# acproject/wsi-segmentation-pipeline

Measured on AMD Instinct MI355X. Metric: patches/sec (256×256×3) whole-slide inference, 1/2/4/8 MI355X + CPU ref, higher is better.
Workload: dtype fp16 + MX-fp6 cross terms (fp32 accumulate); 1 GPU; cfg3: ONE 40000x40000 synthetic slide, tile 256 stride 256 -> 24648 tiles sharded over 1 rank(s) (each holds only its own slide regions: 4.80 GB on rank 0), ResNet-18 trunk + Classifier, fused read+normalise+conv HIP path, 1 all-gather, float64 stitch + softmax; tiles_total=24648, batch=6200, mode=mx, parallelism=tile-shard x1 + 1 all-gather, batches_in_flight=2

## Files before the change

include/wsi_hip.h:

```cpp
#ifndef WSI_HIP_H
#define WSI_HIP_H
#include <stddef.h>
#include <stdint.h>

#ifdef __cplusplus
extern "C" {
#endif

#define WSI_HIP_ABI_VERSION 8
int wsi_hip_abi_version(void);

size_t wsi_pf_bytes(int n, int h, int w, int c, int planes);
long long wsi_pf_pixel_index(int n, int y, int x, int h, int w);

size_t wsi_prepack_conv_bytes(int cout, int cin, int k, int planes);
int wsi_prepack_conv(const float* w, const float* bn_weight, const float* bn_bias, const float* bn_mean,
                     const float* bn_var, float eps, int cout, int cin, int k, int planes, void* wpk_out,
                     float* bias_out);
size_t wsi_prepack_stem_bytes(int planes);
int wsi_prepack_stem(const float* w, const float* bn_weight, const float* bn_bias, const float* bn_mean,
                     const float* bn_var, float eps, int planes, void* wpk_out, float* bias_out);
int wsi_prepack_stem_u8(const float* w, const float* bn_weight, const float* bn_bias, const float* bn_mean,
                        const float* bn_var, float eps, const float mean[3], const float std_[3], int planes,
                        void* wpk_out, float* bias_out);
int wsi_normalize_u8_lut(const float mean[3], const float std_[3], float* lut_out );

int wsi_stem_conv7x7_bn_relu_maxpool(const float* in_f32, const uint8_t* slide, long long slide_pitch_bytes,
                                     int slide_h, int slide_w, const int* tile_xy, const float* lut,
                                     const void* stem_wpk, const float* stem_bias,
                                     const void* stem_wpk_u8 ,
                                     const float* stem_bias_u8, const float* norm_mean_std ,
                                     int n, int h, int w, float* scratch, void* out_pf, int planes, void* stream);

enum {
    WSI_STEM_MODE_UNFUSED = 0,
    WSI_STEM_MODE_FUSED = 1,
    WSI_STEM_MODE_FUSED_LUT = 2,
    WSI_STEM_MODE_FUSED_ONE_STRIP = 3
};
int wsi_stem_set_mode(int fused, int rows_per_seg);

int wsi_conv3x3_bn_act(const void* in_pf, void* out_pf, const void* resid_pf, const void* wpk, const float* bias,
                       int n, int h_in, int w_in, int cin, int cout, int stride, int relu, int planes,
                       void* stream);
int wsi_conv1x1_bn(const void* in_pf, void* out_pf, const void* wpk, const float* bias, int n, int h_in, int w_in,
                   int cin, int cout, int stride, int planes, void* stream);
int wsi_conv3x3_up_concat_bn_act(const void* up_pf, const void* skip_pf, void* out_pf, const void* wpk, const float* bias, int n, int h, int w,
                                 int c_up, int c_skip, int cout, int relu, int planes, void* stream);
int wsi_conv3x3s2_ds_fused(const void* in_pf, void* out_conv_pf, void* out_ds_pf, const void* wpk3, const float* bias3,
                           const void* wpk1, const float* bias1, int n, int h_in, int w_in, int cin, int cout, int planes,
                           void* stream);
int wsi_s2_slab_images(int n, int h_in, int w_in, int cin, int planes);
size_t wsi_pf_split_bytes(int n, int h, int w, int c, int planes);
int wsi_conv3x3_bn_act_split(const void* in_pf, void* out_split, const void* resid_pf, const void* wpk, const float* bias,
                             int n, int h, int w, int cin, int cout, int relu, int planes, void* stream);
int wsi_conv3x3s2_ds_fused_split(const void* in_split, void* out_conv_pf, void* out_ds_pf, const void* wpk3,
                                 const float* bias3, const void* wpk1, const float* bias1, int n, int h_in, int w_in,
                                 int cin, int cout, int planes, void* stream);
enum {
    WSI_CONV_MODE_S2_GATHER = 0,
    WSI_CONV_MODE_S2_SLAB = 1,
    WSI_CONV_MODE_S2_SLAB_128 = 3,
    WSI_CONV_MODE_XCD_ORDER = 8,
    WSI_CONV_MODE_WIDE_FROM_256 = 16,
    WSI_CONV_MODE_WIDE_NEVER = 32,
    WSI_CONV_MODE_S2_ABLATE = 64,
    WSI_CONV_MODE_NO_S2_SPLIT = 128,
    WSI_CONV_MODE_XCD_RANGES_OFF = 256,
    WSI_CONV_MODE_XCD_RANGES_L1 = 512,
    WSI_CONV_MODE_L1_SLAB3 = 1024,
    WSI_CONV_MODE_NO_DS_FOLD = 2048,
    WSI_CONV_MODE_NO_SLAB_PAIR = 4096,
    WSI_CONV_MODE_L1_LINES128 = 16384,
    WSI_CONV_MODE_S2_NT2 = 32768,
    WSI_CONV_MODE_UNET_CONCAT_PASS = 65536,
    WSI_CONV_MODE_WIDE_NO_D8 = 131072,
    WSI_CONV_MODE_L1_PERSISTENT = 1048576,
    WSI_CONV_MODE_UNET_NO_TAIL = 2097152,
    WSI_CONV_MODE_UNET_TAIL_FORM1 = 4194304,
    WSI_CONV_MODE_UNET_X0_UNFUSED = 8388608
};
int wsi_conv_set_mode(int mode);
int wsi_conv3x3_bn_act_cfg(const void* in_pf, void* out_pf, const void* resid_pf, const void* wpk, const float* bias,
                           int n, int h_in, int w_in, int cin, int cout, int stride, int relu, int planes, int cfg,
                           void* stream);

int wsi_avgpool_fc(const void* in_pf, int n, int h, int w, int c, const float* fc_w, const float* fc_b, int k,
                   float* feat_out, float* logits_out, int planes, void* stream);
int wsi_linear(const float* x, const float* w, const float* bias, float* y, int b, int k, int j, int relu,
               void* stream);

int wsi_pf_pack(const float* in_nchw, void* out_pf, int n, int c, int h, int w, int planes, void* stream);
int wsi_pf_unpack(const void* in_pf, float* out_nchw, int n, int c, int h, int w, int planes, void* stream);

typedef struct {
    const void* stem_w;   const float* stem_b;
    const void* stem_w_u8; const float* stem_b_u8;
    float norm[6];
    const void* conv_w[16]; const float* conv_b[16];
    const void* down_w[3];  const float* down_b[3];
    const float* head_w;  const float* head_b;  int head_k;
    int planes;
} wsi_trunk_weights;

size_t wsi_trunk_workspace_bytes(int n, int h, int w, int planes);
int wsi_trunk_workspace_init(void* workspace, int n, int h, int w, int planes, void* stream);
int wsi_trunk_workspace_release(void* workspace);
int wsi_trunk_forward(const wsi_trunk_weights* wt, const float* in_f32, const uint8_t* slide,
                      long long slide_pitch_bytes, int slide_h, int slide_w, const int* tile_xy, const float* lut,
                      int n, int h, int w, void* workspace, int workspace_n, float* feat_out ,
                      float* logits_out , float* fmap_out ,
                      void* stream);
int wsi_trunk_set_chunks(int stem_chunk, int layer1_chunk);
int wsi_trunk_forward_tap(const wsi_trunk_weights* wt, const float* in_f32, const uint8_t* slide,
                          long long slide_pitch_bytes, int slide_h, int slide_w, const int* tile_xy, const float* lut,
                          int n, int h, int w, void* workspace, int workspace_n, int stop_after, float* tap_out_nchw,
                          void* stream);

int wsi_prof_begin(int max_records);
int wsi_prof_end(float* ms_out, int* kind_out, double* flops_out, int cap);

int wsi_tile_gather(const uint8_t* slide, long long slide_pitch_bytes, int slide_h, int slide_w, const int* tile_xy,
                    const float* lut, float* out_nchw, int n, int ph, int pw, void* stream);
int wsi_stitch_add(const float* tile_logits, const int* map_xy, int t, int c, int dy, int dx, double* pred, int map_h,
                   int map_w, void* stream);
int wsi_stitch_add_dense(const float* tile_pred, const int* map_xy, int t, int c, int ph, int pw, double* pred, int map_h,
                         int map_w, void* stream);
int wsi_softmax_threshold_argmax(const double* pred, int c, long long hw, const double* class_thresh, double* probs,
                                 uint8_t* classes, const uint8_t* mask, int heat_mode, uint8_t* heat, void* stream);
typedef struct wsi_ring wsi_ring;
typedef struct wsi_resample_plan wsi_resample_plan;
int wsi_ring_create(wsi_ring** out, int slots, size_t slot_bytes);
void* wsi_ring_host_slot(wsi_ring* ring, int slot);
int wsi_ring_wait_slot(wsi_ring* ring, int slot);
int wsi_ring_submit(wsi_ring* ring, int slot, int rows, int width, int channels, long long src_pitch, uint8_t* level_rows, long long level_pitch);
int wsi_ring_acquire(wsi_ring* ring, void* compute_stream);
int wsi_ring_fence(wsi_ring* ring, void* compute_stream);
int wsi_ring_device(const wsi_ring* ring);
int wsi_ring_drain(wsi_ring* ring);
void wsi_ring_destroy(wsi_ring* ring);
int wsi_resample_plan_create(wsi_resample_plan** out, int in_h, int in_w, int out_h, int out_w);
void wsi_resample_plan_destroy(wsi_resample_plan* plan);
size_t wsi_resample_scratch_bytes(const wsi_resample_plan* plan, int n);
int wsi_resample_tiles(const wsi_resample_plan* plan, const uint8_t* slide, long long pitch, int sh, int sw, const int* tile_xy, int n,
                       uint8_t* out, void* scratch, void* stream);
int wsi_find_nuclei_hsv(const uint8_t* rgb, long long npix, int pixel_stride, double mu_percent, uint8_t* mask_out, void* stream);
size_t wsi_connected_components_scratch_bytes(int h, int w);
int wsi_connected_components(const uint8_t* mask, int h, int w, int* labels_out, int* count_out, void* scratch, void* stream);
int wsi_kmeans_points(const int* points_xy, int n, double* centres_xy, int k, int max_iters, int* labels_out, void* scratch, void* stream);
int wsi_kmeans_seed_farthest(const int* points_xy, int n, int k, double* centres_xy_out, void* scratch, void* stream);
int wsi_find_nuclei_lab(const uint8_t* rgb, long long npix, int pixel_stride, double mu_percent, uint8_t* mask_out, void* scratch, void* stream);
size_t wsi_fill_holes_scratch_bytes(int h, int w);
int wsi_fill_holes(const uint8_t* mask, int h, int w, uint8_t* out, void* scratch, void* stream);
size_t wsi_slic_scratch_bytes(int h, int w, int k);
int wsi_slic(const uint8_t* rgb, int h, int w, const double* gauss_weights, int radius, double* segments, int k, int step_y, int step_x,
             double step, double compactness, int iters, int* labels_out, void* scratch, void* stream);
long long wsi_tile_grid_candidates(int iw, int ih, int ph, int pw, int sh, int sw);
size_t wsi_tile_grid_scratch_bytes(long long candidates);
int wsi_tile_grid(int iw, int ih, int ph, int pw, int sh, int sw, const uint8_t* mask, int mask_h, int mask_w, double m, double thresh,
                  int* tile_xy_out, int* count_out, void* scratch, void* stream);
int wsi_exponent_span(const float* values, long long n, int* out2, void* stream);
int wsi_paint_regions(const long long* pixel_idx, const int* region_of, long long n, const uint8_t* region_class, int* winner_scratch,
                      long long* label, long long npix, void* stream);

int wsi_resize_bilinear_f64(const double* src, int c, int hs, int ws, double* dst, int hd, int wd, void* stream);
int wsi_argmax_classes(const double* pred, int c, long long hw, uint8_t* classes, void* stream);
int wsi_morph_rect(const uint8_t* src, uint8_t* dst, uint8_t* tmp, int h, int w, int k, int op, void* stream);
int wsi_bwperim(const uint8_t* src, uint8_t* dst, int h, int w, void* stream);
size_t wsi_tumor_bed_workspace_bytes(int h, int w);
int wsi_convex_hull_image(const uint8_t* src, uint8_t* dst, int h, int w, void* workspace, void* stream);
int wsi_tumor_bed(const uint8_t* codes, int h, int w, int min_code, int open_k, int dilate_k, uint8_t* opened_out,
                  uint8_t* tb_pred_out, uint8_t* outline_out, void* workspace, void* stream);
int wsi_hull_polygon(void* workspace, int h, int w, double* out_xy, int cap, int* count_out, void* stream);
int wsi_mask_iou_counts(const uint8_t* a, const uint8_t* b, long long n, unsigned long long* out2, void* stream);
int wsi_score_counts(const uint8_t* p, const uint8_t* gt, const uint8_t* mask, long long n, unsigned long long* out6,
                     void* stream);
int wsi_esp(const double* pts_xy, int n, int num_pts, double* out_xy, double* scratch, void* stream);

typedef struct {
    const void* conv_w[10]; const float* conv_b[10];
    int cin[10], cout[10];
    const float* head_w; const float* head_b;
    int head_cin, classes;
    const void* tail_w;
} wsi_unet_decoder_weights;
size_t wsi_unet_tail_prepack_bytes(void);
int wsi_unet_tail_prepack(const float* w1, const float* bn1_weight, const float* bn1_bias, const float* bn1_mean, const float* bn1_var,
                          const float* w2, const float* bn2_weight, const float* bn2_bias, const float* bn2_mean, const float* bn2_var,
                          float eps, const float* head_w, const float* head_b, int cin, int cmid, int classes, void* out);
int wsi_unet_tail_bands(int n, int h, int cus);
int wsi_unet_tail_timeouts(unsigned long long* out, int reset);
size_t wsi_unet_workspace_bytes(const wsi_unet_decoder_weights* dw, int n, int h, int w, int planes);
int wsi_unet_workspace_init(const wsi_unet_decoder_weights* dw, void* workspace, int n, int h, int w, int planes, void* stream);
int wsi_unet_forward(const wsi_trunk_weights* wt, const wsi_unet_decoder_weights* dw, const float* in_f32, const uint8_t* slide,
                     long long slide_pitch_bytes, int slide_h, int slide_w, const int* tile_xy, const float* lut, int n, int h,
                     int w, void* workspace, int workspace_n, float* logits_out, float* enc_out[5], void* stream);
int wsi_unet_decoder(const wsi_unet_decoder_weights* dw, const float* const enc_nchw[5], int n, int h, int w, int planes,
                     void* workspace, int workspace_n, float* logits_out, void* stream);
int wsi_resize_nearest_f32(const float* src, long long planes_n, int hs, int ws, float* dst, int hd, int wd, void* stream);

#ifdef __cplusplus
}
#endif
#endif
```

wsi_segmentation_pipeline_amd/csrc/capi.hip:

```cpp
#include "common.h"
#include <mutex>
#include <unordered_map>
#include <vector>
#include <cmath>
#include "../../include/wsi_hip.h"
#include <math.h>
#include <string.h>

int wsi_conv_dispatch(const ConvArgs& a, int planes, int cfg, hipStream_t st);
int wsi_s2_dispatch(const ConvArgs& a, int planes, hipStream_t st);
int wsi_stem_dispatch(const StemArgs& a, int planes, hipStream_t st);
int wsi_maxpool_dispatch(const float* in, void* out, int N, int Hc, int Wc, int planes, hipStream_t st);
int wsi_stem_pool_dispatch(const StemArgs& a, void* out_pf, int planes, int rows_per_seg, hipStream_t st, int out96 = 0, long long plane96 = 0, void* x0_pf = nullptr);
int wsi_avgpool_fc_dispatch(const void* in, const PFGeom& g, const float* w, const float* b, int K, float* feat,
                            float* logits, int planes, hipStream_t st);
int wsi_linear_dispatch(const float* x, const float* w, const float* bias, float* y, int B, int K, int J, int relu,
                        hipStream_t st);
int wsi_pf_pack_dispatch(const float* in, void* out, const PFGeom& g, int planes, hipStream_t st);
int wsi_pf_unpack_dispatch(const void* in, float* out, const PFGeom& g, int planes, hipStream_t st);
int wsi_tile_gather_dispatch(const uint8_t* slide, long long pitch, int SH, int SW, const int* origins, const float* lut,
                             float* out, int N, int ph, int pw, hipStream_t st);
int wsi_stitch_add_dispatch(const float* logits, const int* txy, int T, int C, int dy, int dx, double* pred, int MH, int MW,
                            hipStream_t st);
int wsi_stitch_add_dense_dispatch(const float* tiles, const int* txy, int T, int C, int ph, int pw, double* pred, int MH,
// ... 359 lines not shown
    const int DIG = 3;
    int8_t* o = (int8_t*)wpk_out;
    float* scale_out = (float*)((char*)wpk_out + 2 * 7 * 3 * 1024);
    memset(wpk_out, 0, (size_t)2 * 7 * 3 * 1024 + 64 * sizeof(float));
    const double qmax = DIG == 3 ? 127.0 * 65536.0 : 127.0 * 256.0;
    for (int co = 0; co < 64; ++co) {
        double sc, sh;
        bn_fold(bn_weight, bn_bias, bn_mean, bn_var, eps, co, sc, sh);
        bias_out[co] = (float)sh;
        double val[7][8][4];
        double amax = 0.0;
        for (int kh = 0; kh < 7; ++kh)
            for (int kw = 0; kw < 8; ++kw) {
                double kap = 0.0;
                for (int c = 0; c < 3; ++c) {
                    const double wd = kw < 7 ? (double)w[(((size_t)co * 3 + c) * 7 + kh) * 7 + kw] * sc / (255.0 * (double)std_[c]) : 0.0;
                    val[kh][kw][c] = wd;
                    kap += wd * (128.0 - 255.0 * (double)mean[c]);
                    amax = fmax(amax, fabs(wd));
                }
                val[kh][kw][3] = kap / 127.0;
                amax = fmax(amax, fabs(val[kh][kw][3]));
            }
        const double scale = amax > 0.0 ? amax / qmax : 1.0;
        scale_out[co] = (float)scale;
        const double fscale = (double)scale_out[co];
        const int nt = co >> 5, l31 = co & 31;
        for (int kh = 0; kh < 7; ++kh)
            for (int kw = 0; kw < 8; ++kw)
                for (int c = 0; c < 4; ++c) {
                    long long q = llround(val[kh][kw][c] / fscale);
                    const int h = kw >> 2, j = (kw & 3) * 4 + c, lane = h * 32 + l31;
                    for (int d = 0; d < DIG; ++d) {
                        const long long dig = ((q + 128) & 255) - 128;
                        q = (q - dig) / 256;
                        o[(((size_t)(nt * 7 + kh) * DIG + d) * 64 + lane) * 16 + j] = (int8_t)dig;
                    }
                }
    }
    return WSI_OK;
}

int wsi_normalize_u8_lut(const float mean[3], const float std_[3], float* lut_out) {
    if (!mean || !std_ || !lut_out) return WSI_EINVAL;
    for (int c = 0; c < 3; ++c)
        for (int v = 0; v < 256; ++v) {
            volatile float t = (float)v / 255.0f;
            volatile float d = t - mean[c];
            lut_out[c * 256 + v] = d / std_[c];
        }
    return WSI_OK;
}

int wsi_stem_set_mode(int fused, int rows_per_seg) {
    if (rows_per_seg <= 0) return WSI_EINVAL;
    g_routes.stem_fused = fused != WSI_STEM_MODE_UNFUSED; g_routes.stem_rows = rows_per_seg;
    g_routes.stem_u8x = fused != WSI_STEM_MODE_FUSED_LUT;
    g_routes.stem_shared_weights = fused != WSI_STEM_MODE_FUSED_ONE_STRIP;
    return WSI_OK;
}

struct TileSource {
    const float* in_f32;
    const uint8_t* slide;
    long long pitch; int SH, SW;
    const int* tile_xy;
    const float* lut;
    bool valid() const { return in_f32 || (slide && tile_xy && lut); }
    TileSource from_image(int n0, int h, int w) const {
        return {in_f32 ? in_f32 + (size_t)n0 * 3 * h * w : nullptr, slide, pitch, SH, SW, tile_xy ? tile_xy + 2 * n0 : nullptr, lut};
    }
};
static StemArgs stem_args(const TileSource& src, const void* wpk, const float* bias, float* scratch, int n, int h, int w) {
    StemArgs a;
    a.mode = src.in_f32 ? 0 : 1;
    a.in_f32 = src.in_f32; a.slide = src.slide; a.slide_pitch = src.pitch; a.SH = src.SH; a.SW = src.SW;
    a.origins = src.tile_xy; a.lut = src.lut; a.wpk = wpk; a.bias = bias; a.out = scratch;
    a.N = n; a.H = h; a.W = w; a.wpk_u8 = nullptr; a.bias_u8 = nullptr;
    return a;
}

static int stem_run(const TileSource& src, const void* stem_wpk, const float* stem_bias, const void* stem_wpk_u8,
                    const float* stem_bias_u8, const float* norm_mean_std, int n, int h, int w,
                    float* scratch, void* out_pf, int planes, void* stream, int out96, long long plane96 = 0, void* x0_pf = nullptr) {
    if (!stem_wpk || !stem_bias || !scratch || !out_pf || n <= 0 || h % 16 || w % 4) return WSI_EINVAL;
    if (!src.valid()) return WSI_EINVAL;
    StemArgs a = stem_args(src, stem_wpk, stem_bias, scratch, n, h, w);
    if (stem_wpk_u8 && stem_bias_u8 && norm_mean_std && !src.in_f32 && g_routes.stem_u8x) { a.wpk_u8 = stem_wpk_u8; a.bias_u8 = stem_bias_u8; }
    if (out96 && planes != 3) return WSI_EINVAL;
    if (x0_pf && !(a.wpk_u8 && g_routes.stem_fused && planes == 2)) return WSI_EINVAL;
    if (g_routes.stem_fused || planes == 3) return wsi_stem_pool_dispatch(a, out_pf, planes, g_routes.stem_rows, (hipStream_t)stream, out96, plane96, x0_pf);
    int rc = wsi_stem_dispatch(a, planes, (hipStream_t)stream);
    if (rc) return rc;
    return wsi_maxpool_dispatch(scratch, out_pf, n, h / 2, w / 2, planes, (hipStream_t)stream);
}

int wsi_stem_conv7x7_bn_relu_maxpool(const float* in_f32, const uint8_t* slide, long long slide_pitch_bytes,
                                     int slide_h, int slide_w, const int* tile_xy, const float* lut,
                                     const void* stem_wpk, const float* stem_bias, const void* stem_wpk_u8,
                                     const float* stem_bias_u8, const float* norm_mean_std, int n, int h, int w,
                                     float* scratch, void* out_pf, int planes, void* stream) {
    return stem_run({in_f32, slide, slide_pitch_bytes, slide_h, slide_w, tile_xy, lut}, stem_wpk, stem_bias, stem_wpk_u8, stem_bias_u8,
                    norm_mean_std, n, h, w, scratch, out_pf, planes, stream, 0);
}

#ifdef WSI_STUDY
static void* g_study_debug = nullptr;
extern "C" int wsi_study_set_debug(void* dev_buf) { g_study_debug = dev_buf; return WSI_OK; }
#endif

struct ConvCall {
    const void* in;
    void* out;
    const void* resid = nullptr;
    const void* wpk; const float* bias;
    int n, h, w, cin, cout, stride, ksize, relu, planes;
    void* stream;
    int cfg = -1;
    int split_out = 0; long long split_pixels = 0;
    const void* in2 = nullptr; int in2_c = 0; const void* wpk2 = nullptr; const float* bias2 = nullptr;
    int line_flags = 0;
    const void* in_up = nullptr; int up_c = 0;
    long long plane96 = 0;
};

static ConvArgs conv_args(const ConvCall& c) {
    ConvArgs a;
    a.in = c.in; a.out = c.out; a.resid = c.resid; a.wpk = c.wpk; a.bias = c.bias;
    a.gi = pf_geom_fd(c.n, c.h, c.w, c.cin);
    a.go = pf_geom_fd(c.n, c.h / c.stride, c.w / c.stride, c.cout);
    a.stride = c.stride; a.ksize = c.ksize; a.relu = c.relu & 1; a.flags = 0;
    a.out2 = nullptr; a.wpk2 = nullptr; a.bias2 = nullptr;
    a.in_split_pixels = 0; a.out_split_pixels = 0;
    return a;
}

static int conv_common(const ConvCall& c) {
    const hipStream_t st = (hipStream_t)c.stream;
    int cfg = c.cfg;
    if ((!c.in && !(c.in_up && c.up_c == c.cin)) || !c.out || !c.wpk || !c.bias || c.in == c.out || c.in_up == c.out || c.n <= 0) return WSI_EINVAL;
    if (c.line_flags && (c.planes != 3 || c.stride != 1 || c.ksize != 3 || c.cin != 64 || c.cout != 64 || (c.split_out && (c.line_flags & CONV_OUT96)) ||
                         (c.line_flags & ~(CONV_IN96 | CONV_OUT96 | CONV_RESID96)) || ((c.line_flags & CONV_RESID96) && !c.resid)))
        return WSI_EINVAL;
    if ((c.stride != 1 && c.stride != 2) || c.h % c.stride || c.w % c.stride) return WSI_EINVAL;
    ConvArgs a = conv_args(c);
    a.plane96 = c.line_flags ? (c.plane96 > 0 ? c.plane96 : (long long)pf_alloc_pixels(c.n, c.h, c.w) * 96) : 0;
#ifdef WSI_STUDY
    if (c.relu & 2) a.flags |= CONV_ABL_NO_STORE;
    if (c.relu & 64) a.flags |= CONV_ABL_DISPATCH_ONLY;
    if (c.relu & 128) a.flags |= CONV_ABL_NO_MAINLOOP;
    if (c.relu & 256) a.flags |= CONV_NONTEMPORAL;
    if (c.relu & 512) a.flags |= CONV_XCD_ORDER;
    if (c.relu & 16384) a.flags |= CONV_XCD_RANGES;
    if (c.relu & 65536) a.flags |= CONV_RESID_DIRECT;
    a.flags |= ((c.relu >> 10) & 15) << CONV_WCOPIES_SHIFT;
#else
    if (c.relu & ~1) return WSI_EINVAL;
#endif
    a.flags |= c.line_flags;
    if (c.in_up) {
        if (c.stride != 1 || c.ksize != 3 || c.h % 2 || c.w % 2 || c.up_c <= 0 || c.up_c > c.cin || c.resid || c.in2 || c.line_flags || c.split_out) return WSI_EINVAL;
        a.in_up = c.in_up; a.up_c = c.up_c; a.gup = pf_geom_fd(c.n, c.h / 2, c.w / 2, c.up_c);
    }
    if (c.in2) {
        if (c.planes != 3 || c.stride != 1 || c.ksize != 3 || c.resid || !c.wpk2 || !c.bias2 || c.in2_c <= 0 || c.in2_c % 32 || c.cout % 128 || cfg >= 0) return WSI_EINVAL;
        a.in2 = c.in2; a.in2_c = c.in2_c; a.wpk2 = c.wpk2; a.bias2 = c.bias2;
        cfg = 60;
    }
#ifdef WSI_STUDY
    if (cfg == 75 || cfg == 76) a.out2 = g_study_debug;
#endif
    a.out_split_pixels = c.split_out ? (c.split_pixels ? c.split_pixels : pf_alloc_pixels(c.n, c.h / 2, c.w / 2)) : 0;
    if (c.split_out && (c.stride != 1 || c.ksize != 3 || c.h % 2 || c.w % 2 || c.planes < 2)) return WSI_EINVAL;
    if (c.ksize == 3 && c.stride == 2 && c.cout % 128 == 0 && cfg != 0 && g_routes.s2_slab) {
        const int rc = wsi_s2_dispatch(a, c.planes, st);
        if (rc != WSI_EINVAL) return rc;
    }
    return wsi_conv_dispatch(a, c.planes, cfg, st);
}

int wsi_conv3x3_bn_act(const void* in_pf, void* out_pf, const void* resid_pf, const void* wpk, const float* bias,
                       int n, int h_in, int w_in, int cin, int cout, int stride, int relu, int planes,
                       void* stream) {
    return conv_common({.in = in_pf, .out = out_pf, .resid = resid_pf, .wpk = wpk, .bias = bias, .n = n, .h = h_in, .w = w_in, .cin = cin,
                        .cout = cout, .stride = stride, .ksize = 3, .relu = relu, .planes = planes, .stream = stream});
}

size_t wsi_pf_split_bytes(int n, int h, int w, int c, int planes) {
    if (h % 2 || w % 2) return 0;
    return 4 * wsi_pf_bytes(n, h / 2, w / 2, c, planes);
}

int wsi_conv3x3_bn_act_split(const void* in_pf, void* out_split, const void* resid_pf, const void* wpk, const float* bias,
                             int n, int h, int w, int cin, int cout, int relu, int planes, void* stream) {
    return conv_common({.in = in_pf, .out = out_split, .resid = resid_pf, .wpk = wpk, .bias = bias, .n = n, .h = h, .w = w, .cin = cin,
                        .cout = cout, .stride = 1, .ksize = 3, .relu = relu, .planes = planes, .stream = stream, .split_out = 1});
}

static ConvArgs s2_ds_args(const void* in, void* out_conv_pf, void* out_ds_pf, const void* wpk3, const float* bias3, const void* wpk1,
                           const float* bias1, int n, int h_in, int w_in, int cin, int cout) {
    ConvArgs a = conv_args({.in = in, .out = out_conv_pf, .wpk = wpk3, .bias = bias3, .n = n, .h = h_in, .w = w_in, .cin = cin, .cout = cout,
                            .stride = 2, .ksize = 3, .relu = 1});
    a.out2 = out_ds_pf; a.wpk2 = out_ds_pf ? wpk1 : nullptr; a.bias2 = out_ds_pf ? bias1 : nullptr;
    return a;
}

static int s2_split_common(const void* in_split, void* out_conv_pf, void* out_ds_pf, const void* wpk3,
                           const float* bias3, const void* wpk1, const float* bias1, int n, int h_in, int w_in,
                           int cin, int cout, int planes, void* stream, long long split_pixels) {
    if (!in_split || !out_conv_pf || !wpk3 || !bias3 || (out_ds_pf && (!wpk1 || !bias1)) || n <= 0 || h_in % 2 || w_in % 2)
        return WSI_EINVAL;
    if (in_split == out_conv_pf || in_split == out_ds_pf || out_conv_pf == out_ds_pf) return WSI_EINVAL;
    ConvArgs a = s2_ds_args(in_split, out_conv_pf, out_ds_pf, wpk3, bias3, wpk1, bias1, n, h_in, w_in, cin, cout);
    a.in_split_pixels = split_pixels ? split_pixels : pf_alloc_pixels(n, h_in / 2, w_in / 2);
    return wsi_s2_dispatch(a, planes, (hipStream_t)stream);
}

int wsi_conv3x3s2_ds_fused_split(const void* in_split, void* out_conv_pf, void* out_ds_pf, const void* wpk3,
                                 const float* bias3, const void* wpk1, const float* bias1, int n, int h_in, int w_in,
                                 int cin, int cout, int planes, void* stream) {
    return s2_split_common(in_split, out_conv_pf, out_ds_pf, wpk3, bias3, wpk1, bias1, n, h_in, w_in, cin, cout, planes, stream, 0);
}

int wsi_conv3x3_bn_act_cfg(const void* in_pf, void* out_pf, const void* resid_pf, const void* wpk, const float* bias,
                           int n, int h_in, int w_in, int cin, int cout, int stride, int relu, int planes, int cfg,
                           void* stream) {
    return conv_common({.in = in_pf, .out = out_pf, .resid = resid_pf, .wpk = wpk, .bias = bias, .n = n, .h = h_in, .w = w_in, .cin = cin,
                        .cout = cout, .stride = stride, .ksize = 3, .relu = relu, .planes = planes, .stream = stream, .cfg = cfg});
}

int wsi_conv3x3_up_concat_bn_act(const void* up_pf, const void* skip_pf, void* out_pf, const void* wpk, const float* bias, int n, int h, int w,
                                 int c_up, int c_skip, int cout, int relu, int planes, void* stream) {
    if (!up_pf || c_up <= 0 || c_skip < 0 || (c_skip > 0 && !skip_pf)) return WSI_EINVAL;
    return conv_common({.in = c_skip ? skip_pf : nullptr, .out = out_pf, .wpk = wpk, .bias = bias, .n = n, .h = h, .w = w, .cin = c_up + c_skip,
                        .cout = cout, .stride = 1, .ksize = 3, .relu = relu, .planes = planes, .stream = stream, .in_up = up_pf, .up_c = c_up});
}

int wsi_s2_slab_images(int n, int h_in, int w_in, int cin, int planes) {
    if (n <= 0 || h_in <= 0 || w_in <= 0 || cin <= 0 || planes < 1 || planes > 3) return WSI_EINVAL;
    const unsigned long long pix = (unsigned long long)cin * (planes == 1 ? PFmt<1>::BPC : PFmt<2>::BPC);
    auto fits = [&](int m) { return (unsigned long long)pf_alloc_pixels(m, h_in, w_in) * pix < 0xffffffffull; };
    if (fits(n)) return n;
    if (!fits(1)) return 0;
    int lo = 1, hi = n;
    while (hi - lo > 1) {
        const int mid = lo + (hi - lo) / 2;
        (fits(mid) ? lo : hi) = mid;
    }
    return lo;
}

int wsi_conv3x3s2_ds_fused(const void* in_pf, void* out_conv_pf, void* out_ds_pf, const void* wpk3, const float* bias3,
                           const void* wpk1, const float* bias1, int n, int h_in, int w_in, int cin, int cout, int planes,
                           void* stream) {
    if (!in_pf || !out_conv_pf || !out_ds_pf || !wpk3 || !bias3 || !wpk1 || !bias1 || n <= 0 || h_in % 2 || w_in % 2)
        return WSI_EINVAL;
    if (in_pf == out_conv_pf || in_pf == out_ds_pf || out_conv_pf == out_ds_pf) return WSI_EINVAL;
    ConvArgs a = s2_ds_args(in_pf, out_conv_pf, out_ds_pf, wpk3, bias3, wpk1, bias1, n, h_in, w_in, cin, cout);
    const int per = wsi_s2_slab_images(n, h_in, w_in, cin, planes);
    const size_t bpc = planes == 1 ? PFmt<1>::BPC : PFmt<2>::BPC;
    const size_t in_img = (size_t)(h_in + 1) * (w_in + 1) * cin * bpc, out_img = (size_t)(h_in / 2 + 1) * (w_in / 2 + 1) * cout * bpc;
    int rc = WSI_EINVAL;
    for (int n0 = 0; per > 0 && n0 < n; n0 += per) {
        const int nn = n - n0 < per ? n - n0 : per;
        a.in = (const char*)in_pf + n0 * in_img;
        a.out = (char*)out_conv_pf + n0 * out_img;
        a.out2 = (char*)out_ds_pf + n0 * out_img;
        a.gi = pf_geom_fd(nn, h_in, w_in, cin);
        a.go = pf_geom_fd(nn, h_in / 2, w_in / 2, cout);
        rc = wsi_s2_dispatch(a, planes, (hipStream_t)stream);
        if (rc) break;
    }
    if (rc == WSI_EINVAL) {
        ConvCall c = {.in = in_pf, .out = out_conv_pf, .wpk = wpk3, .bias = bias3, .n = n, .h = h_in, .w = w_in, .cin = cin, .cout = cout,
                      .stride = 2, .ksize = 3, .relu = 1, .planes = planes, .stream = stream, .cfg = 0};
        rc = conv_common(c);
        c.out = out_ds_pf; c.wpk = wpk1; c.bias = bias1; c.ksize = 1; c.relu = 0;
        if (!rc) rc = conv_common(c);
    }
    return rc;
}

int wsi_conv_set_mode(int mode) {
    ConvRoutes& r = g_routes;
    const int base = mode & 7;
    r.s2_slab = base != WSI_CONV_MODE_S2_GATHER;
    r.s2_small_tiles = base != WSI_CONV_MODE_S2_SLAB_128;
    r.xcd_order = (mode & WSI_CONV_MODE_XCD_ORDER) ? 1 : 0;
    r.wide_min_c = (mode & WSI_CONV_MODE_WIDE_FROM_256) ? 256 : (mode & WSI_CONV_MODE_WIDE_NEVER) ? (1 << 30) : 128;
    r.s2_ablate = (mode & WSI_CONV_MODE_S2_ABLATE) ? 1 : 0;
    r.s2_split = (mode & WSI_CONV_MODE_NO_S2_SPLIT) ? 0 : 1;
    r.xcd_ranges = (mode & WSI_CONV_MODE_XCD_RANGES_OFF) ? 0 : (mode & WSI_CONV_MODE_XCD_RANGES_L1) ? 1 : 2;
    r.l1_rows = (mode & WSI_CONV_MODE_L1_SLAB3) ? 0 : 1;
    r.ds_fold = (mode & WSI_CONV_MODE_NO_DS_FOLD) ? 0 : 1;
    r.slab_pair = (mode & WSI_CONV_MODE_NO_SLAB_PAIR) ? 0 : 1;
    r.l1_lines96 = (mode & WSI_CONV_MODE_L1_LINES128) ? 0 : 1;
    r.s2_nt4 = (mode & WSI_CONV_MODE_S2_NT2) ? 0 : 1;
    r.unet_fuse_up = (mode & WSI_CONV_MODE_UNET_CONCAT_PASS) ? 0 : 1;
    r.wide_d8 = (mode & WSI_CONV_MODE_WIDE_NO_D8) ? 0 : 1;
    r.l1p = (mode & WSI_CONV_MODE_L1_PERSISTENT) ? 1 : 0;
    r.unet_tail = (mode & WSI_CONV_MODE_UNET_NO_TAIL) ? 0 : 1;
    r.unet_tail_form = (mode & WSI_CONV_MODE_UNET_TAIL_FORM1) ? 1 : 2;
    r.unet_x0_fused = (mode & WSI_CONV_MODE_UNET_X0_UNFUSED) ? 0 : 1;
    return WSI_OK;
}

int wsi_conv1x1_bn(const void* in_pf, void* out_pf, const void* wpk, const float* bias, int n, int h_in, int w_in,
                   int cin, int cout, int stride, int planes, void* stream) {
    return conv_common({.in = in_pf, .out = out_pf, .wpk = wpk, .bias = bias, .n = n, .h = h_in, .w = w_in, .cin = cin, .cout = cout,
                        .stride = stride, .ksize = 1, .relu = 0, .planes = planes, .stream = stream});
}

int wsi_avgpool_fc(const void* in_pf, int n, int h, int w, int c, const float* fc_w, const float* fc_b, int k,
                   float* feat_out, float* logits_out, int planes, void* stream) {
    if (!in_pf || n <= 0 || (logits_out && (!fc_w || !fc_b || k <= 0))) return WSI_EINVAL;
    return wsi_avgpool_fc_dispatch(in_pf, pf_geom(n, h, w, c), fc_w, fc_b, k, feat_out, logits_out, planes,
                                   (hipStream_t)stream);
}

int wsi_linear(const float* x, const float* w, const float* bias, float* y, int b, int k, int j, int relu,
               void* stream) {
    if (!x || !w || !y) return WSI_EINVAL;
    return wsi_linear_dispatch(x, w, bias, y, b, k, j, relu, (hipStream_t)stream);
}

int wsi_pf_pack(const float* in_nchw, void* out_pf, int n, int c, int h, int w, int planes, void* stream) {
    if (!in_nchw || !out_pf || n <= 0 || planes < 1 || planes > 3 || c % (planes == 1 ? 64 : 32)) return WSI_EINVAL;
    return wsi_pf_pack_dispatch(in_nchw, out_pf, pf_geom(n, h, w, c), planes, (hipStream_t)stream);
}

int wsi_pf_unpack(const void* in_pf, float* out_nchw, int n, int c, int h, int w, int planes, void* stream) {
    if (!in_pf || !out_nchw || n <= 0 || planes < 1 || planes > 3 || c % (planes == 1 ? 64 : 32)) return WSI_EINVAL;
    return wsi_pf_unpack_dispatch(in_pf, out_nchw, pf_geom(n, h, w, c), planes, (hipStream_t)stream);
}

int wsi_tile_gather(const uint8_t* slide, long long slide_pitch_bytes, int slide_h, int slide_w, const int* tile_xy,
                    const float* lut, float* out_nchw, int n, int ph, int pw, void* stream) {
    if (!slide || !tile_xy || !lut || !out_nchw) return WSI_EINVAL;
    return wsi_tile_gather_dispatch(slide, slide_pitch_bytes, slide_h, slide_w, tile_xy, lut, out_nchw, n, ph, pw,
                                    (hipStream_t)stream);
}

int wsi_stitch_add(const float* tile_logits, const int* map_xy, int t, int c, int dy, int dx, double* pred, int map_h,
                   int map_w, void* stream) {
    if (!tile_logits || !map_xy || !pred || map_h <= 0 || map_w <= 0) return WSI_EINVAL;
    return wsi_stitch_add_dispatch(tile_logits, map_xy, t, c, dy, dx, pred, map_h, map_w, (hipStream_t)stream);
}

int wsi_stitch_add_dense(const float* tile_pred, const int* map_xy, int t, int c, int ph, int pw, double* pred, int map_h,
                         int map_w, void* stream) {
    if (!tile_pred || !map_xy || !pred || map_h <= 0 || map_w <= 0) return WSI_EINVAL;
    return wsi_stitch_add_dense_dispatch(tile_pred, map_xy, t, c, ph, pw, pred, map_h, map_w, (hipStream_t)stream);
}

int wsi_softmax_threshold_argmax(const double* pred, int c, long long hw, const double* class_thresh, double* probs,
                                 uint8_t* classes, const uint8_t* mask, int heat_mode, uint8_t* heat, void* stream) {
    if (!pred || !class_thresh) return WSI_EINVAL;
    return wsi_softmax_dispatch(pred, c, hw, class_thresh, probs, classes, mask, heat_mode, heat, (hipStream_t)stream);
}

int wsi_ring_create(wsi_ring** out, int slots, size_t slot_bytes) { return wsi_ring_create_impl(out, slots, slot_bytes); }
void* wsi_ring_host_slot(wsi_ring* r, int slot) { return wsi_ring_host_slot_impl(r, slot); }
int wsi_ring_wait_slot(wsi_ring* r, int slot) { return wsi_ring_wait_slot_impl(r, slot); }
int wsi_ring_submit(wsi_ring* r, int slot, int rows, int width, int channels, long long src_pitch, uint8_t* level_rows, long long level_pitch) {
    return wsi_ring_submit_impl(r, slot, rows, width, channels, src_pitch, level_rows, level_pitch);
}
int wsi_ring_fence(wsi_ring* r, void* compute_stream) { return wsi_ring_fence_impl(r, (hipStream_t)compute_stream); }
int wsi_ring_acquire(wsi_ring* r, void* compute_stream) { return wsi_ring_acquire_impl(r, (hipStream_t)compute_stream); }
int wsi_ring_device(const wsi_ring* r) { return wsi_ring_device_impl(r); }
int wsi_ring_drain(wsi_ring* r) { return wsi_ring_drain_impl(r); }
void wsi_ring_destroy(wsi_ring* r) { wsi_ring_destroy_impl(r); }
int wsi_resample_plan_create(wsi_resample_plan** out, int in_h, int in_w, int out_h, int out_w) {
    return wsi_resample_plan_create_impl(out, in_h, in_w, out_h, out_w);
}
void wsi_resample_plan_destroy(wsi_resample_plan* p) { wsi_resample_plan_destroy_impl(p); }
size_t wsi_resample_scratch_bytes(const wsi_resample_plan* p, int n) { return wsi_resample_scratch_bytes_impl(p, n); }
int wsi_resample_tiles(const wsi_resample_plan* p, const uint8_t* slide, long long pitch, int sh, int sw, const int* tile_xy, int n,
                       uint8_t* out, void* scratch, void* stream) {
    return wsi_resample_tiles_impl(p, slide, pitch, sh, sw, tile_xy, n, out, scratch, (hipStream_t)stream);
}

int wsi_find_nuclei_hsv(const uint8_t* rgb, long long npix, int pixel_stride, double mu_percent, uint8_t* mask_out, void* stream) {
    if (!rgb || !mask_out) return WSI_EINVAL;
    return wsi_hsv_mask_dispatch(rgb, npix, pixel_stride, mu_percent, mask_out, (hipStream_t)stream);
}
size_t wsi_connected_components_scratch_bytes(int h, int w) { return (h <= 0 || w <= 0) ? 0 : wsi_cc_scratch_bytes(h, w); }
int wsi_connected_components(const uint8_t* mask, int h, int w, int* labels_out, int* count_out, void* scratch, void* stream) {
    if (!mask || !labels_out || !scratch) return WSI_EINVAL;
    return wsi_cc_dispatch(mask, h, w, labels_out, count_out, scratch, (hipStream_t)stream);
}
int wsi_find_nuclei_lab(const uint8_t* rgb, long long npix, int pixel_stride, double mu_percent, uint8_t* mask_out, void* scratch, void* stream) {
    return wsi_lab_mask_dispatch(rgb, npix, pixel_stride, mu_percent, mask_out, scratch, (hipStream_t)stream);
}
size_t wsi_fill_holes_scratch_bytes(int h, int w) { return (h <= 0 || w <= 0) ? 0 : wsi_fill_holes_scratch_bytes_impl(h, w); }
int wsi_fill_holes(const uint8_t* mask, int h, int w, uint8_t* out, void* scratch, void* stream) {
    return wsi_fill_holes_dispatch(mask, h, w, out, scratch, (hipStream_t)stream);
}
size_t wsi_slic_scratch_bytes(int h, int w, int k) { return wsi_slic_scratch_bytes_impl(h, w, k); }
int wsi_slic(const uint8_t* rgb, int h, int w, const double* gauss_weights, int radius, double* segments, int k, int step_y, int step_x,
             double step, double compactness, int iters, int* labels_out, void* scratch, void* stream) {
    return wsi_slic_dispatch(rgb, h, w, gauss_weights, radius, segments, k, step_y, step_x, step, compactness, iters, labels_out, scratch,
                             (hipStream_t)stream);
}
int wsi_kmeans_points(const int* points_xy, int n, double* centres_xy, int k, int max_iters, int* labels_out, void* scratch, void* stream) {
    if (!points_xy || !centres_xy || !labels_out || !scratch) return WSI_EINVAL;
    return wsi_kmeans_dispatch(points_xy, n, centres_xy, k, max_iters, labels_out, scratch, (hipStream_t)stream);
}

int wsi_kmeans_seed_farthest(const int* points_xy, int n, int k, double* centres_xy_out, void* scratch, void* stream) {
    if (!points_xy || !centres_xy_out || !scratch) return WSI_EINVAL;
    return wsi_kmeans_seed_farthest_dispatch(points_xy, n, k, centres_xy_out, scratch, (hipStream_t)stream);
}

long long wsi_tile_grid_candidates(int iw, int ih, int ph, int pw, int sh, int sw) { return wsi_tile_grid_candidates_impl(iw, ih, ph, pw, sh, sw); }
size_t wsi_tile_grid_scratch_bytes(long long candidates) { return candidates < 0 ? 0 : wsi_tile_grid_scratch_bytes_impl(candidates); }
int wsi_tile_grid(int iw, int ih, int ph, int pw, int sh, int sw, const uint8_t* mask, int mask_h, int mask_w, double m, double thresh,
                  int* tile_xy_out, int* count_out, void* scratch, void* stream) {
    if (!tile_xy_out || !count_out || !scratch) return WSI_EINVAL;
    return wsi_tile_grid_dispatch(iw, ih, ph, pw, sh, sw, mask, mask_h, mask_w, m, thresh, tile_xy_out, count_out, scratch, (hipStream_t)stream);
}

int wsi_exponent_span(const float* values, long long n, int* out2, void* stream) {
    if (!values || !out2) return WSI_EINVAL;
    return wsi_exponent_span_dispatch(values, n, out2, (hipStream_t)stream);
}

int wsi_paint_regions(const long long* pixel_idx, const int* region_of, long long n, const uint8_t* region_class, int* winner_scratch,
                      long long* label, long long npix, void* stream) {
    if (!region_class || !winner_scratch || !label || (n && (!pixel_idx || !region_of))) return WSI_EINVAL;
    return wsi_paint_dispatch(pixel_idx, region_of, n, region_class, winner_scratch, label, npix, (hipStream_t)stream);
}

int wsi_resize_bilinear_f64(const double* src, int c, int hs, int ws, double* dst, int hd, int wd, void* stream) {
    if (!src || !dst || src == dst) return WSI_EINVAL;
    return wsi_resize_dispatch(src, c, hs, ws, dst, hd, wd, (hipStream_t)stream);
}
int wsi_argmax_classes(const double* pred, int c, long long hw, uint8_t* classes, void* stream) {
    if (!pred || !classes) return WSI_EINVAL;
    return wsi_argmax_dispatch(pred, c, hw, classes, (hipStream_t)stream);
}
int wsi_morph_rect(const uint8_t* src, uint8_t* dst, uint8_t* tmp, int h, int w, int k, int op, void* stream) {
    if (!src || !dst || !tmp) return WSI_EINVAL;
    return wsi_morph_dispatch(src, dst, tmp, h, w, k, op, (hipStream_t)stream);
}
int wsi_bwperim(const uint8_t* src, uint8_t* dst, int h, int w, void* stream) {
    if (!src || !dst) return WSI_EINVAL;
    return wsi_bwperim_dispatch(src, dst, h, w, (hipStream_t)stream);
}
size_t wsi_tumor_bed_workspace_bytes(int h, int w) {
    if (h <= 0 || w <= 0) return 0;
    return 3 * align_up((size_t)h * w, 256) + align_up(wsi_hull_ws_bytes(h), 256);
}
int wsi_convex_hull_image(const uint8_t* src, uint8_t* dst, int h, int w, void* workspace, void* stream) {
    if (!src || !dst || !workspace || src == dst) return WSI_EINVAL;
    return wsi_hull_dispatch(src, dst, h, w, (char*)workspace + 3 * align_up((size_t)h * w, 256), (hipStream_t)stream);
}
int wsi_tumor_bed(const uint8_t* codes, int h, int w, int min_code, int open_k, int dilate_k, uint8_t* opened_out,
                  uint8_t* tb_pred_out, uint8_t* outline_out, void* workspace, void* stream) {
    if (!codes || !tb_pred_out || !outline_out || !workspace || h <= 0 || w <= 0 || open_k <= 0 || dilate_k <= 0 ||
        tb_pred_out == outline_out)
        return WSI_EINVAL;
    hipStream_t st = (hipStream_t)stream;
    const size_t plane = align_up((size_t)h * w, 256);
    uint8_t *A = (uint8_t*)workspace, *B = A + plane, *Cc = B + plane;
    void* hws = Cc + plane;
    int rc = wsi_threshold_dispatch(codes, (long long)h * w, min_code, A, st);
    if (!rc) rc = wsi_morph_dispatch(A, B, Cc, h, w, open_k, 2, st);
    if (!rc && opened_out && hipMemcpyAsync(opened_out, B, (size_t)h * w, hipMemcpyDeviceToDevice, st) != hipSuccess) rc = WSI_EFAULT;
    if (!rc) rc = wsi_hull_dispatch(B, tb_pred_out, h, w, hws, st);
    if (!rc) rc = wsi_bwperim_dispatch(tb_pred_out, A, h, w, st);
    if (!rc) rc = wsi_morph_dispatch(A, outline_out, Cc, h, w, dilate_k, 1, st);
    return rc;
}
int wsi_hull_polygon(void* workspace, int h, int w, double* out_xy, int cap, int* count_out, void* stream) {
    if (!workspace || !out_xy || !count_out || h <= 0 || w <= 0 || cap <= 0) return WSI_EINVAL;
    char* hws = (char*)workspace + 3 * align_up((size_t)h * w, 256);
    int rc = wsi_hull_polygon_dispatch(hws, h, out_xy, cap, (hipStream_t)stream);
    if (rc) return rc;
    const int* counts = (const int*)hws + 2 * (2 * (size_t)h + 1);
    return hipMemcpyAsync(count_out, counts + 2, sizeof(int), hipMemcpyDeviceToDevice, (hipStream_t)stream) == hipSuccess ? WSI_OK : WSI_EFAULT;
}
int wsi_mask_iou_counts(const uint8_t* a, const uint8_t* b, long long n, unsigned long long* out2, void* stream) {
    if (!a || !b || !out2) return WSI_EINVAL;
    return wsi_iou_counts_dispatch(a, b, n, out2, (hipStream_t)stream);
}
int wsi_score_counts(const uint8_t* p, const uint8_t* gt, const uint8_t* mask, long long n, unsigned long long* out6, void* stream) {
    if (!p || !gt || !out6) return WSI_EINVAL;
    return wsi_score_counts_dispatch(p, gt, mask, n, out6, (hipStream_t)stream);
}
int wsi_esp(const double* pts_xy, int n, int num_pts, double* out_xy, double* scratch, void* stream) {
    if (!pts_xy || !out_xy || !scratch) return WSI_EINVAL;
    return wsi_esp_dispatch(pts_xy, n, num_pts, out_xy, scratch, (hipStream_t)stream);
}

#define WSI_PROF_MAX 16384
static struct {
    int enabled, count, cap;
    hipEvent_t ev[2 * WSI_PROF_MAX];
    int kind[WSI_PROF_MAX];
    double flops[WSI_PROF_MAX];
    int created;
} g_prof;

int wsi_prof_begin(int max_records) {
    if (max_records <= 0 || max_records > WSI_PROF_MAX) return WSI_EINVAL;
    for (; g_prof.created < 2 * max_records; ++g_prof.created)
        if (hipEventCreate(&g_prof.ev[g_prof.created]) != hipSuccess) return WSI_ENOMEM;
    g_prof.cap = max_records; g_prof.count = 0; g_prof.enabled = 1;
    return WSI_OK;
}

int wsi_prof_end(float* ms_out, int* kind_out, double* flops_out, int cap) {
    g_prof.enabled = 0;
    int n = g_prof.count < cap ? g_prof.count : cap;
    for (int i = 0; i < n; ++i) {
        if (hipEventSynchronize(g_prof.ev[2 * i + 1]) != hipSuccess) return WSI_EFAULT;
        float ms = 0.f;
        if (hipEventElapsedTime(&ms, g_prof.ev[2 * i], g_prof.ev[2 * i + 1]) != hipSuccess) return WSI_EFAULT;
        ms_out[i] = ms; kind_out[i] = g_prof.kind[i]; flops_out[i] = g_prof.flops[i];
    }
    g_prof.count = 0;
    return n;
}

struct ProfScope {
    const hipStream_t st;
    int i = -1;
    ProfScope(hipStream_t st, int kind, double flops) : st(st) {
        if (!g_prof.enabled || g_prof.count >= g_prof.cap) return;
        i = g_prof.count++;
        g_prof.kind[i] = kind; g_prof.flops[i] = flops;
        (void)hipEventRecord(g_prof.ev[2 * i], st);
    }
    ~ProfScope() { if (i >= 0) (void)hipEventRecord(g_prof.ev[2 * i + 1], st); }
    void relabel(int kind) { if (i >= 0) g_prof.kind[i] = kind; }
};
static inline double conv_flops(int n, int ho, int wo, int ci, int co, int taps) { return 2.0 * n * ho * wo * (double)co * ci * taps; }

static std::mutex g_ws_mutex;
struct WsTag { int layout; size_t bytes; };
static std::unordered_map<const void*, WsTag> g_ws_layout;
static int ws_layout_switch(const void* ws, int want, size_t need) {
    std::lock_guard<std::mutex> lk(g_ws_mutex);
    auto it = g_ws_layout.find(ws);
    const int have = it == g_ws_layout.end() ? -2 : it->second.layout;
    const size_t bytes = it == g_ws_layout.end() ? 0 : it->second.bytes;
    if (bytes && need > bytes) return -1;
    g_ws_layout[ws] = WsTag{want, bytes};
    if (have == want || have == -1) return 0;
    return (have >= 0 && have / 2 != want / 2) ? 2 : 1;
}
int wsi_trunk_workspace_release(void* workspace) {
    std::lock_guard<std::mutex> lk(g_ws_mutex);
    g_ws_layout.erase(workspace);
    return WSI_OK;
}

int wsi_trunk_set_chunks(int stem_chunk, int layer1_chunk) {
    if (stem_chunk < 0 || layer1_chunk < 0) return WSI_EINVAL;
    if (stem_chunk && layer1_chunk && layer1_chunk % stem_chunk) return WSI_EINVAL;
    g_routes.chunk_stem = stem_chunk; g_routes.chunk_l1 = layer1_chunk;
    return WSI_OK;
}
struct TrunkPlan {
    size_t stem_scratch;
    size_t buf[4][4];
    size_t total;
    int sh[4], sw[4], sc[4];
};

static int trunk_plan(int n, int h, int w, int planes, TrunkPlan& p) {
    if (n <= 0 || h <= 0 || w <= 0 || h % 32 || w % 32 || planes < 1 || planes > 3) return WSI_EINVAL;
    size_t off = 0;
    p.stem_scratch = off;
    off += align_up((size_t)n * (h / 2) * (w / 2) * 64 * sizeof(float), 256);
    for (int s = 0; s < 4; ++s) {
        p.sh[s] = h >> (2 + s); p.sw[s] = w >> (2 + s); p.sc[s] = 64 << s;
        for (int b = 0; b < 3; ++b) {
            p.buf[s][b] = off;
            off += align_up(wsi_pf_bytes(n, p.sh[s], p.sw[s], p.sc[s], planes), 256);
        }
        p.buf[s][3] = off;
        if (s < 3 && planes >= 2) off += align_up(wsi_pf_split_bytes(n, p.sh[s], p.sw[s], p.sc[s], planes), 256);
    }
    p.total = off;
    return WSI_OK;
}

size_t wsi_trunk_workspace_bytes(int n, int h, int w, int planes) {
    TrunkPlan p;
    return trunk_plan(n, h, w, planes, p) ? 0 : p.total;
}

int wsi_trunk_workspace_init(void* workspace, int n, int h, int w, int planes, void* stream) {
    TrunkPlan p;
    if (!workspace || trunk_plan(n, h, w, planes, p)) return WSI_EINVAL;
    {
        std::lock_guard<std::mutex> lk(g_ws_mutex);
        g_ws_layout[workspace] = WsTag{-1, p.total};
    }
    return hipMemsetAsync((char*)workspace + p.buf[0][0], 0, p.total - p.buf[0][0], (hipStream_t)stream) == hipSuccess
               ? WSI_OK
               : WSI_EFAULT;
}

static int trunk_run(const wsi_trunk_weights* wt, const TileSource& src, int n, int cap, int h, int w, void* workspace,
// ... 318 lines not shown
```

wsi_segmentation_pipeline_amd/csrc/common.h:

```cpp
#pragma once
#include <hip/hip_runtime.h>
#include <stdint.h>

typedef __attribute__((ext_vector_type(8))) __bf16 bf16x8;
typedef __attribute__((ext_vector_type(4))) __bf16 bf16x4;
typedef __attribute__((ext_vector_type(16))) float f32x16;
typedef __attribute__((ext_vector_type(4))) float f32x4;

#define WSI_OK 0
#define WSI_EINVAL (-22)
#define WSI_ENOMEM (-12)
#define WSI_EFAULT (-14)

struct FastDiv { unsigned m; int s; };
static inline FastDiv fastdiv_make(int d) {
    FastDiv f;
    if (d <= 1) { f.m = 0u; f.s = -1; return f; }
    int l = 0;
    while ((1ll << l) < d) ++l;
    f.m = (unsigned)(((1ull << (31 + l)) / (unsigned long long)d) + 1ull);
    f.s = l - 1;
    return f;
}
#ifdef __HIPCC__
static inline __device__ int fd_div(int i, const FastDiv& f) { return f.s < 0 ? i : (int)(__umulhi((unsigned)i, f.m) >> f.s); }
#endif

struct PFGeom {
    int N, H, W, C;
    int P, S, G;
    int NS;
    FastDiv dHW, dW, dS, dP;
};

static inline __host__ __device__ PFGeom pf_geom(int n, int h, int w, int c) {
    PFGeom g;
    g.N = n; g.H = h; g.W = w; g.C = c;
    g.P = w + 1; g.S = (h + 1) * (w + 1); g.G = w + 2; g.NS = n * g.S;
    g.dHW.m = g.dW.m = g.dS.m = g.dP.m = 0u; g.dHW.s = g.dW.s = g.dS.s = g.dP.s = 0;
    return g;
}
static inline PFGeom pf_geom_fd(int n, int h, int w, int c) {
    PFGeom g = pf_geom(n, h, w, c);
    g.dHW = fastdiv_make(h * w); g.dW = fastdiv_make(w); g.dS = fastdiv_make(g.S); g.dP = fastdiv_make(g.P);
    return g;
}
static inline __device__ int pf_pos_of_index(const PFGeom& g, int i) {
    const int n = fd_div(i, g.dHW), rem = i - n * (g.H * g.W);
    const int y = fd_div(rem, g.dW), x = rem - y * g.W;
    return g.G + n * g.S + y * g.P + x;
}

#define PF_TILE_ROUND 512

static inline __host__ __device__ long long pf_alloc_pixels(int n, int h, int w) {
    long long P = w + 1, S = (long long)(h + 1) * P, G = P + 1;
    long long body = ((long long)n * S + PF_TILE_ROUND - 1) / PF_TILE_ROUND * PF_TILE_ROUND;
    return 2 * G + body + PF_TILE_ROUND;
}

static inline __device__ bool pf_is_pixel(const PFGeom& g, int q) {
    int r = q - g.G;
    if (r < 0 || r >= g.NS) return false;
    int x = r % g.P;
    int y = (r / g.P) % (g.H + 1);
    return x != g.W && y != g.H;
}

template <int PLANES> struct PFmt {
    static constexpr int BPC = PLANES == 1 ? 2 : 4;
    static constexpr int CPL = PLANES == 1 ? 64 : 32;
};
typedef __attribute__((ext_vector_type(8))) _Float16 f16x8;
typedef __attribute__((ext_vector_type(4))) _Float16 f16x4;
typedef __attribute__((ext_vector_type(8))) int i32x8;
typedef __attribute__((ext_vector_type(4))) unsigned int u32x4;
typedef __attribute__((ext_vector_type(2))) float f32x2;
typedef __attribute__((ext_vector_type(2))) _Float16 f16x2;
typedef __attribute__((ext_vector_type(4))) int i32x4;

struct ConvArgs {
    const void* in;
    void* out;
    const void* resid;
    const void* wpk;
    const float* bias;
    PFGeom gi, go;
    int stride;
    int ksize;
    int relu;
    int flags;
    void* out2;
    const void* wpk2;
    const float* bias2;
    long long out_split_pixels, in_split_pixels;
    int mtiles = 0;
    const void* in2 = nullptr;
    int in2_c = 0;
    const void* in_up = nullptr;
    int up_c = 0;
    PFGeom gup = {};
    long long plane96 = 0;
};

enum : int {
    CONV_XCD_ORDER = 1,
    CONV_XCD_RANGES = 2,
    CONV_RESID_DIRECT = 4,
    CONV_IN96 = 16, CONV_OUT96 = 32, CONV_RESID96 = 64,
    CONV_ABL_NO_STORE = 1 << 8, CONV_ABL_DISPATCH_ONLY = 1 << 9, CONV_ABL_NO_MAINLOOP = 1 << 10, CONV_NONTEMPORAL = 1 << 11,
    CONV_WCOPIES_SHIFT = 16,
};
#ifdef WSI_STUDY
#define CONV_STUDY(a, bits) ((a).flags & (bits))
#else
#define CONV_STUDY(a, bits) 0
#endif

static inline __device__ size_t pf_out_offset(const PFGeom& g, long long split_pixels, int q, size_t pixstride) {
    if (!split_pixels) return (size_t)q * pixstride;
    int r = q - g.G;
    const int n = fd_div(r, g.dS);
    r -= n * g.S;
    const int y = fd_div(r, g.dP), x = r - y * g.P;
    const int P2 = g.W / 2 + 1, S2 = (g.H / 2 + 1) * P2;
    const long long q2 = (long long)(P2 + 1) + (long long)n * S2 + (y >> 1) * P2 + (x >> 1);
    return (size_t)(((y & 1) * 2 + (x & 1)) * split_pixels + q2) * pixstride;
}

static inline __device__ f32x16 mfma_bf16(bf16x8 a, bf16x8 b, f32x16 c) {
    return __builtin_amdgcn_mfma_f32_32x32x16_bf16(a, b, c, 0, 0, 0);
}
template <int PLANES> struct PairElem { typedef __bf16 T; };
template <> struct PairElem<2> { typedef _Float16 T; };
template <int PLANES>
static inline __device__ f32x16 mfma16(bf16x8 a, bf16x8 b, f32x16 c) {
    typedef __attribute__((ext_vector_type(8))) _Float16 h8;
    if constexpr (PLANES == 2) return __builtin_amdgcn_mfma_f32_32x32x16_f16(__builtin_bit_cast(h8, a), __builtin_bit_cast(h8, b), c, 0, 0, 0);
    else return __builtin_amdgcn_mfma_f32_32x32x16_bf16(a, b, c, 0, 0, 0);
}

typedef __attribute__((ext_vector_type(6))) unsigned u32x6;
typedef __attribute__((ext_vector_type(16))) unsigned u32x16;
typedef __attribute__((ext_vector_type(32))) float f32x32;
static inline __host__ __device__ int mx6_scale_byte(float amax) {
    union { float f; unsigned u; } c;
    c.f = amax;
    const unsigned u = c.u & 0x7fffffffu;
    if (u == 0u) return 0;
    const int e = (int)(u >> 23) - 2 + ((u & 0x7fffffu) > 0x780000u ? 1 : 0);
    return e < 1 ? 1 : (e > 254 ? 254 : e);
}
static inline __host__ __device__ float mx_scale_value(int s) {
    union { float f; unsigned u; } c;
    c.u = (unsigned)s << 23;
    return c.f;
}
static inline __host__ __device__ int mx_line_pos(int c) { return 16 * ((c >> 2) & 1) + 4 * (c >> 3) + (c & 3); }
static inline __host__ __device__ int mx_line_chan(int p) { return 8 * ((p & 15) >> 2) + 4 * (p >> 4) + (p & 3); }
static inline __host__ __device__ int mx6_field_of_pos(int p) { return 2 * (p & 15) + (p >> 4); }
static inline __host__ __device__ int mx6_field_chan(int f) { return mx_line_chan(16 * (f & 1) + (f >> 1)); }
#define MX6_PLANE_LO(q) (64 + 16 * (q))
#define MX6_PLANE_HI(q) (96 + 16 * (q))
#define MX6_SCALE(q) (104 + 16 * (q))

static inline __host__ __device__ float fp6_value(unsigned c) {
    const int e = (c >> 3) & 3, m = c & 7;
    const float v = e ? (float)(8 + m) * (e == 1 ? 0.125f : e == 2 ? 0.25f : 0.5f) : (float)m * 0.125f;
    return (c & 32) ? -v : v;
}
static inline __host__ __device__ unsigned fp6_encode(float y) {
    union { float f; unsigned u; } c;
    c.f = y;
    const unsigned sign = (c.u >> 31) ? 32u : 0u;
    c.u &= 0x7fffffffu;
    const float a = c.f;
    if (!(a < 7.5f)) return sign | 31u;
    const float step = a < 2.f ? 0.125f : a < 4.f ? 0.25f : 0.5f;
    const float t = a / step;
    float r = (float)(int)t;
    const float frac = t - r;
    if (frac > 0.5f || (frac == 0.5f && ((int)r & 1))) r += 1.f;
    const float q = r * step;
    unsigned code;
    if (q < 1.f) code = (unsigned)(q * 8.f);
    else if (q < 2.f) code = 8u + (unsigned)((q - 1.f) * 8.f);
    else if (q < 4.f) code = 16u + (unsigned)((q - 2.f) * 4.f);
    else code = 24u + (unsigned)((q - 4.f) * 2.f);
    return sign | code;
}
static inline __host__ __device__ unsigned mx6_get_field(const unsigned* w, int f) {
    const int bit = 6 * f, d = bit >> 5, s = bit & 31;
    unsigned v = w[d] >> s;
    if (s > 26) v |= w[d + 1] << (32 - s);
    return v & 63u;
}
static inline __host__ __device__ void mx6_set_field(unsigned* w, int f, unsigned code) {
    const int bit = 6 * f, d = bit >> 5, s = bit & 31;
    w[d] |= code << s;
    if (s > 26) w[d + 1] |= code >> (32 - s);
}

#ifdef __HIPCC__
static __device__ __forceinline__ u32x6 mx6_pack32(f32x16 a, f32x16 b, float scale) {
    u32x6 r;
    asm volatile("v_cvt_scalef32_2xpk16_fp6_f32 %0, %1, %2, %3" : "=&v"(r) : "v"(a), "v"(b), "v"(scale));
    return r;
}
static __device__ __forceinline__ f32x32 mx6_unpack32(u32x6 q, float scale) {
    f32x32 r;
    asm volatile("v_cvt_scalef32_pk32_f32_fp6 %0, %1, %2" : "=&v"(r) : "v"(q), "v"(scale));
    return r;
}
static __device__ __forceinline__ void swap32_halves(f32x16& a, f32x16& b) {
#pragma unroll
    for (int k = 0; k < 16; k += 8) {
        float a0 = a[k], a1 = a[k + 1], a2 = a[k + 2], a3 = a[k + 3], a4 = a[k + 4], a5 = a[k + 5], a6 = a[k + 6], a7 = a[k + 7];
        float b0 = b[k], b1 = b[k + 1], b2 = b[k + 2], b3 = b[k + 3], b4 = b[k + 4], b5 = b[k + 5], b6 = b[k + 6], b7 = b[k + 7];
        asm volatile("s_nop 1\n\tv_permlane32_swap_b32 %0, %8\n\tv_permlane32_swap_b32 %1, %9\n\tv_permlane32_swap_b32 %2, %10\n\t"
                     "v_permlane32_swap_b32 %3, %11\n\tv_permlane32_swap_b32 %4, %12\n\tv_permlane32_swap_b32 %5, %13\n\t"
                     "v_permlane32_swap_b32 %6, %14\n\tv_permlane32_swap_b32 %7, %15\n\ts_nop 1"
                     : "+v"(a0), "+v"(a1), "+v"(a2), "+v"(a3), "+v"(a4), "+v"(a5), "+v"(a6), "+v"(a7),
                       "+v"(b0), "+v"(b1), "+v"(b2), "+v"(b3), "+v"(b4), "+v"(b5), "+v"(b6), "+v"(b7));
        a[k] = a0; a[k + 1] = a1; a[k + 2] = a2; a[k + 3] = a3; a[k + 4] = a4; a[k + 5] = a5; a[k + 6] = a6; a[k + 7] = a7;
        b[k] = b0; b[k + 1] = b1; b[k + 2] = b2; b[k + 3] = b3; b[k + 4] = b4; b[k + 5] = b5; b[k + 6] = b6; b[k + 7] = b7;
    }
}
static __device__ __forceinline__ void pair_max2(float& x, float& y) {
    float x2 = x, y2 = y;
    asm volatile("s_nop 1\n\tv_permlane32_swap_b32 %0, %1\n\tv_permlane32_swap_b32 %2, %3\n\ts_nop 1" : "+v"(x), "+v"(x2), "+v"(y), "+v"(y2));
    x = fmaxf(x, x2);
    y = fmaxf(y, y2);
}

#endif

static inline __device__ void split_f16(float x, _Float16& hi, _Float16& lo) {
    x = __builtin_amdgcn_fmed3f(x, -65504.f, 65504.f);
    hi = (_Float16)x;
    lo = (_Float16)(x - (float)hi);
}
static inline __device__ void split_f16x4(const float* v, f16x4& hi, f16x4& lo) {
#pragma unroll
    for (int i = 0; i < 4; ++i) {
        _Float16 a, b;
        split_f16(v[i], a, b);
        hi[i] = a;
        lo[i] = b;
    }
}
static inline __device__ const float* conv_wscale_inv(const void* wpk, int cout, int cin, int ksize) {
    return (const float*)((const char*)wpk + (size_t)(cout / 32) * (cin / 32) * ksize * ksize * 4096);
}

struct StemArgs {
    int mode;
    const float* in_f32;
    const uint8_t* slide;
    long long slide_pitch;
    int SH, SW;
    const int* origins;
    const float* lut;
    const void* wpk;
    const float* bias;
    float* out;
    int N, H, W;
    const void* wpk_u8;
    const float* bias_u8;
    void* out_pf = nullptr;
    int out_planes = 0;
};

struct ConvRoutes {
    int stem_fused = 1;
    int stem_rows = 64;
    int stem_u8x = 1;
    int stem_shared_weights = 1;
    int chunk_stem = 0;
    int chunk_l1 = 0;
    int s2_slab = 1;
    int s2_small_tiles = 1;
    int xcd_order = 0;
    int wide_min_c = 128;
    int s2_ablate = 0;
    int s2_split = 1;
    int xcd_ranges = 2;
    int l1_rows = 1;
    int ds_fold = 1;
    int slab_pair = 1;
    int l1_lines96 = 1;
    int s2_nt4 = 1;
    int unet_fuse_up = 1;
    int wide_d8 = 1;
    int l1p = 0;
    int unet_tail = 1;
    int unet_tail_form = 2;
    int unet_x0_fused = 1;
};
extern ConvRoutes g_routes;
```

wsi_segmentation_pipeline_amd/csrc/conv.hip:

```cpp
#include "conv_dev.h"

template <int MT, int WM, int WN, int PLANES>
__global__ __launch_bounds__(WM* WN * 64) void conv_gather_kernel(ConvArgs a) {
    extern __shared__ __attribute__((aligned(16))) char smem[];
    constexpr int BM = WM * MT * 32;
    constexpr int NTHREADS = WM * WN * 64;
    constexpr int PPT = BM * 8 / NTHREADS;
    constexpr int PIX_STEP = NTHREADS / 8;
    const int tid = threadIdx.x, lane = tid & 63, wave = tid >> 6;
    const int wm = wave / WN, wn = wave % WN;
    const int l31 = lane & 31, h = lane >> 5;
    const int nblocks = a.go.C / (WN * 32);
    const int nb = blockIdx.x % nblocks;
    const int mtile = blockIdx.x / nblocks;
    const int q0 = a.go.G + mtile * BM;
    const int ntile = nb * WN + wn;
    const int NC = a.gi.C / PFmt<PLANES>::CPL;
    const int KS = a.ksize, NT = KS * KS, pad = KS / 2;
    const size_t in_pixstride = (size_t)a.gi.C * PFmt<PLANES>::BPC;
    const bf16x8* wbase = (const bf16x8*)a.wpk + (size_t)ntile * NC * NT * 4 * 64 + lane;

    int inq[PPT];
    const int sp = tid & 7;
#pragma unroll
// ... 16 lines not shown
#pragma unroll
    for (int mt = 0; mt < MT; ++mt)
#pragma unroll
        for (int r = 0; r < 16; ++r) acc[mt][r] = 0.f;
    int xbase[MT];
#pragma unroll
    for (int mt = 0; mt < MT; ++mt) xbase[mt] = lds_xbase(wm * MT * 32 + mt * 32 + l31, h);

    for (int c = 0; c < NC; ++c) {
        for (int t = 0; t < NT; ++t) {
            const int toff = (t / KS) * a.gi.P + (t % KS);
            __syncthreads();
#pragma unroll
            for (int k = 0; k < PPT; ++k) {
                const int m = (tid >> 3) + k * PIX_STEP;
                const int s = sp ^ ((m >> 1) & 7);
                const int src = inq[k] < 0 ? 0 : inq[k] + toff;
                *(uint4*)(smem + (size_t)(m * 8 + sp) * 16) =
                    *(const uint4*)((const char*)a.in + (size_t)src * in_pixstride + c * 128 + s * 16);
            }
            bf16x8 wf[4];
#pragma unroll
            for (int f = 0; f < 4; ++f) wf[f] = wbase[((size_t)(c * NT + t) * 4 + f) * 64];
            __syncthreads();
            mfma_line<MT, PLANES>(acc, wf, smem, xbase);
        }
    }
    conv_epilogue<MT, PLANES>(a, acc, q0 + wm * MT * 32, ntile, lane);
}

#ifdef WSI_STUDY
__device__ unsigned long long g_wide_stamps[8];
#define WSTAMP(...) __VA_ARGS__
extern "C" int wsi_study_wide_stamps(unsigned long long* out8, int reset) {
    if (out8 && hipMemcpyFromSymbol(out8, HIP_SYMBOL(g_wide_stamps), sizeof(g_wide_stamps)) != hipSuccess) return WSI_EFAULT;
    if (reset) {
        unsigned long long z[8] = {0};
        if (hipMemcpyToSymbol(HIP_SYMBOL(g_wide_stamps), z, sizeof(z)) != hipSuccess) return WSI_EFAULT;
    }
    return WSI_OK;
}
#else
#define WSTAMP(...)
#endif


template <int MT, int WM, int WN, int PLANES, int MINW, bool DENSE, int ABL = 0, bool PAIR = false>
__global__ __launch_bounds__(WM* WN * 64, MINW) void conv3x3s1_slab3_kernel(ConvArgs a) {
    extern __shared__ __attribute__((aligned(16))) char smem[];
    constexpr int BM = WM * MT * 32;
    constexpr int NTHREADS = WM * WN * 64;
    constexpr int RESID_NBUF = MT < 2 ? MT : 2;
    constexpr bool SCHED = MINW < 3;
    const int tid = threadIdx.x, lane = tid & 63;
    if (CONV_STUDY(a, CONV_ABL_DISPATCH_ONLY)) return;
    WSTAMP(const unsigned long long st_begin = __builtin_readcyclecounter(); unsigned long long st_pro = 0, st_line = 0, st_tap = 0, st_a = 0;)
    const int wave = __builtin_amdgcn_readfirstlane(tid >> 6);
    const int wm = wave / WN, wn = wave % WN;
    const int l31 = lane & 31, h = lane >> 5;
    const int nblocks = a.go.C / (WN * 32);
    int nb = blockIdx.x % nblocks, mtile = blockIdx.x / nblocks;
    if (a.flags & CONV_XCD_ORDER) {
        const int per = 8 * nblocks, r = blockIdx.x % per;
        nb = r >> 3;
        mtile = (blockIdx.x / per) * 8 + (r & 7);
        const int mtiles = DENSE ? (a.gi.N * a.gi.H * a.gi.W + BM - 1) / BM : (a.gi.NS + BM - 1) / BM;
        if (mtile >= mtiles) return;
    } else if (a.flags & CONV_XCD_RANGES) {
        const int chunk = gridDim.x >> 3, lin = (blockIdx.x & 7) * chunk + (blockIdx.x >> 3);
        nb = lin % nblocks;
        mtile = lin / nblocks;
        const int mtiles = DENSE ? (a.gi.N * a.gi.H * a.gi.W + BM - 1) / BM : (a.gi.NS + BM - 1) / BM;
        if (mtile >= mtiles) return;
    }
    const int P = a.gi.P;
    const int ntile = nb * WN + wn;
    const int NC = CONV_STUDY(a, CONV_ABL_NO_MAINLOOP) ? 0 : a.gi.C / PFmt<PLANES>::CPL;
    const bool in96 = PLANES == 3 && (a.flags & CONV_IN96);
    const int ncup = a.in_up ? a.up_c / PFmt<PLANES>::CPL : 0;
    const size_t in_pixstride = in96 ? (size_t)96 : (size_t)(a.gi.C - (a.in_up ? a.up_c : 0)) * PFmt<PLANES>::BPC;
    const int in_line = in96 ? 0 : 128;
    int xoff[MT], qs[MT];
    bool valid[MT];
    int slab0, npieces;
    if constexpr (DENSE) {
        const int HW = a.gi.H * a.gi.W, R = a.gi.N * HW;
        auto pos = [&](int i) { return pf_pos_of_index(a.gi, i); };
        const int i0 = mtile * BM, i1 = min(i0 + BM, R) - 1;
        slab0 = pos(i0) - P - 1;
        npieces = (pos(i1) + P + 1 - slab0 + 1) * 8;
#pragma unroll
        for (int mt = 0; mt < MT; ++mt) {
            const int i = i0 + wm * MT * 32 + mt * 32 + (a.gi.W < 32 ? dense_lane_pixel(l31) : l31);
            valid[mt] = i < R;
            qs[mt] = pos(valid[mt] ? i : i1);
            xoff[mt] = qs[mt] - slab0 - (P + 1);
        }
    } else {
        const int q0 = a.gi.G + mtile * BM;
        slab0 = q0 - P - 1;
        npieces = (BM + 2 * P + 2) * 8;
#pragma unroll
        for (int mt = 0; mt < MT; ++mt) {
            xoff[mt] = wm * MT * 32 + mt * 32 + l31;
            qs[mt] = q0 + xoff[mt];
            valid[mt] = pf_is_pixel(a.go, qs[mt]);
        }
    }
    static_assert((NTHREADS / 8) % 16 == 0, "whole swizzle periods per DMA round");
    const size_t slab_byte0 = (size_t)slab0 * in_pixstride;
    const size_t in_bytes = (size_t)pf_alloc_pixels(a.gi.N, a.gi.H, a.gi.W) * in_pixstride;
    const __amdgpu_buffer_rsrc_t xrs = __builtin_amdgcn_make_buffer_rsrc(
        (void*)((const char*)a.in + slab_byte0), 0, a.in ? (int)min(in_bytes - slab_byte0, (size_t)0x7fffffff) : 0, 0x00020000);
    int xvoff, upl, usl;
    bool xact = true;
    {
        const int i = wave * 64 + lane, Pl = i >> 3, sl = (i & 7) ^ ((Pl >> 1) & 7);
        xvoff = Pl * (int)in_pixstride + (in96 ? mx96_piece(sl) : sl) * 16;
        if (in96) xact = mx96_stored(sl);
        upl = Pl; usl = sl;
    }
    const int up_pixstride = a.up_c * PFmt<PLANES>::BPC;
    const __amdgpu_buffer_rsrc_t urs = __builtin_amdgcn_make_buffer_rsrc(
        (void*)a.in_up, 0, a.in_up ? (int)((size_t)pf_alloc_pixels(a.gup.N, a.gup.H, a.gup.W) * up_pixstride) : 0, 0x00020000);
    const size_t wcopy = (size_t)(mtile % ((CONV_STUDY(a, 15 << CONV_WCOPIES_SHIFT) >> CONV_WCOPIES_SHIFT) + 1)) * (size_t)(a.go.C / 32) * NC * 9 * 4096;
    const __amdgpu_buffer_rsrc_t wrs = __builtin_amdgcn_make_buffer_rsrc(
        (void*)((const char*)a.wpk + wcopy + (size_t)ntile * NC * 9 * 4096), 0, NC * 9 * 4096, 0x00020000);
    const int wvoff = lane * 16;

    f32x16 acc[1][MT];
    if constexpr (PLANES == 3) acc_init_bias<MT>(acc[0], a.bias, ntile, lane);
    else {
#pragma unroll
        for (int mt = 0; mt < MT; ++mt)
#pragma unroll
            for (int r = 0; r < 16; ++r) acc[0][mt][r] = 0.f;
    }
    auto wload = [&](bf16x8(&w)[4], int soff) {
#pragma unroll
        for (int f = 0; f < 4; ++f)
            w[f] = __builtin_bit_cast(bf16x8, __builtin_amdgcn_raw_buffer_load_b128(wrs, wvoff + f * 1024, soff, 0));
    };
    int xa[4];
    auto xload_m = [&](bf16x8(&x)[4], int Pl, int m) {
        if (PAIR && (m & 1)) {
#pragma unroll
            for (int f = 0; f < 4; ++f) x[f] = *(const bf16x8*)(smem + xa[f] + 4096);
            return;
        }
        const int base = lds_xbase(Pl, h);
#pragma unroll
        for (int f = 0; f < 4; ++f) {
            xa[f] = base ^ (f << 5);
            x[f] = *(const bf16x8*)(smem + xa[f]);
        }
    };

    WSTAMP(const unsigned long long st_setup = __builtin_readcyclecounter();)
    for (int c = 0; c < NC; ++c) {
        WSTAMP(st_a = __builtin_readcyclecounter();)
        const int sline = c * 9 * 4096;
        int Pc = P;
        asm volatile("" : "+s"(Pc));
        bf16x8 wbuf[3][4], xf[2][4];
        wload(wbuf[0], sline);
        if (c) __syncthreads();
        if (c < ncup) {
            for (int i0 = wave * 64, r = 0; i0 < npieces; i0 += NTHREADS, ++r) {
                const int rel = slab0 + upl + r * (NTHREADS / 8) - a.gi.G;
                int src = 0;
                if (rel >= 0 && rel < a.gi.NS) {
                    const int n = fd_div(rel, a.gi.dS), rem = rel - n * a.gi.S;
                    const int y = fd_div(rem, a.gi.dP), x = rem - y * P;
                    if (x != a.gi.W && y != a.gi.H) src = a.gup.G + n * a.gup.S + (y >> 1) * a.gup.P + (x >> 1);
                }
                dma16_buf(urs, smem + (size_t)i0 * 16, src * up_pixstride + usl * 16, c * 128);
            }
        } else {
            const __amdgpu_buffer_rsrc_t xr = in96 ? __builtin_amdgcn_make_buffer_rsrc((void*)((const char*)a.in + (size_t)c * (size_t)a.plane96 + slab_byte0), 0,
                                                                                        (int)min(in_bytes - slab_byte0, (size_t)0x7fffffff), 0x00020000)
                                                   : xrs;
            for (int i0 = wave * 64, r = 0; i0 < npieces; i0 += NTHREADS, ++r)
                if (xact) dma16_buf(xr, smem + (size_t)i0 * 16, xvoff, (c - ncup) * in_line + r * (NTHREADS / 8) * (int)in_pixstride);
        }
        asm volatile("s_waitcnt vmcnt(0)" ::: "memory");
        __syncthreads();
        WSTAMP(if (c) st_line += __builtin_readcyclecounter() - st_a; else st_pro = __builtin_readcyclecounter() - st_a; st_a = __builtin_readcyclecounter();)
        if (in96) {
            mx96_rebuild_hi6(smem, npieces >> 3, tid, NTHREADS);
            __syncthreads();
        }
        WSTAMP(st_tap += __builtin_readcyclecounter() - st_a;)
        xload_m(xf[0], xoff[0], 0);
#pragma unroll
        for (int t = 0; t < 9; ++t) {
            asm volatile("" ::: "memory");
            if (t < 8 && !(ABL & 16)) wload(wbuf[(t + 1) % 3], sline + (t + 1) * 4096);
            asm volatile("" ::: "memory");
            const int toff = (t / 3) * Pc + (t % 3);
            const int toff_next = ((t + 1) / 3) * Pc + ((t + 1) % 3);
#pragma unroll
            for (int mt = 0; mt < MT; ++mt) {
                const int k = t * MT + mt;
                if constexpr (!(ABL & 32)) {
                    if (mt + 1 < MT) xload_m(xf[(k + 1) & 1], xoff[mt + 1] + toff, mt + 1);
                    else if (t < 8) xload_m(xf[(k + 1) & 1], xoff[0] + toff_next, 0);
                }
                if constexpr (SCHED) __builtin_amdgcn_sched_barrier(0);
                const bf16x8(&w)[4] = wbuf[t % 3];
                const bf16x8(&x)[4] = xf[k & 1];
                if constexpr (ABL & 8) {
#pragma unroll
                    for (int f = 0; f < 4; ++f) acc[0][mt][f] += (float)w[f][0] * (float)x[f][0];
                } else if constexpr (PLANES == 3) {
                    acc[0][mt] = mfma_mx6(acc[0][mt], w, x);
                } else if constexpr (PLANES == 2) {
                    mfma_step<2>(acc[0][mt], w, x);
                } else {
#pragma unroll
                    for (int f = 0; f < 4; ++f) acc[0][mt] = mfma_bf16(w[f], x[f], acc[0][mt]);
                }
                if constexpr (SCHED) __builtin_amdgcn_sched_barrier(0);
            }
        }
    }
    WSTAMP(const unsigned long long st_loop_end = __builtin_readcyclecounter();)
    if constexpr (PLANES == 3) {
        if (a.resid) __syncthreads();
        conv_tail_mx<1, MT, RESID_NBUF>(a, acc, qs, valid, ntile, lane, smem + wave * (RESID_NBUF * 4096), slab0);
    } else {
        char* scratch = nullptr;
        if (PLANES == 2 && a.resid && !(a.flags & CONV_RESID_DIRECT)) {
            __syncthreads();
            scratch = smem + wave * 8192;
        }
        conv_epilogue_q<MT, PLANES>(a, acc[0], qs, valid, ntile, lane, scratch);
    }
#ifdef WSI_STUDY
    asm volatile("s_waitcnt vmcnt(0)" ::: "memory");
    if (lane == 0 && (blockIdx.x & 63) == 0) {
        const unsigned long long st_end = __builtin_readcyclecounter();
        atomicAdd(&g_wide_stamps[0], 1ull);
        atomicAdd(&g_wide_stamps[1], st_end - st_begin);
        atomicAdd(&g_wide_stamps[2], st_setup - st_begin);
        atomicAdd(&g_wide_stamps[3], st_pro);
        atomicAdd(&g_wide_stamps[4], st_line);
        atomicAdd(&g_wide_stamps[5], st_tap);
        atomicAdd(&g_wide_stamps[6], st_end - st_loop_end);
    }
#endif
}

long long dense_max_slab_pixels(const ConvArgs& a, int BM) {
    const long long R = (long long)a.gi.N * a.gi.H * a.gi.W;
    const int mtiles = (int)((R + BM - 1) / BM);
    const int HW = a.gi.H * a.gi.W;
    auto pos = [&](long long i) { const long long n = i / HW, rem = i - n * HW; return (long long)a.gi.G + n * a.gi.S + (rem / a.gi.W) * a.gi.P + rem % a.gi.W; };
    auto span = [&](int m) { const long long i0 = (long long)m * BM, i1 = (i0 + BM < R ? i0 + BM : R) - 1; return pos(i1) + a.gi.P + 1 - (pos(i0) - a.gi.P - 1) + 1; };
    long long maxpix = span(mtiles - 1);
    int g = BM, r = HW;
    while (r) { const int t = g % r; g = r; r = t; }
    const int period = HW / g + 1;
    const int scan = mtiles < period ? mtiles : period;
    for (int m = 0; m < scan; ++m) { const long long px = span(m); if (px > maxpix) maxpix = px; }
    return maxpix;
}

template <int MT, int WM, int WN, int PLANES, int MINW, bool DENSE, int ABL = 0, bool PAIR = false>
static int launch_slab3(const ConvArgs& a, hipStream_t st) {
    constexpr int BM = WM * MT * 32, NTHREADS = WM * WN * 64;
    if (a.go.C % (WN * 32)) return WSI_EINVAL;
    const int nblocks = a.go.C / (WN * 32);
    int mtiles, maxpix;
    if (DENSE) {
        const long long R = (long long)a.gi.N * a.gi.H * a.gi.W;
        mtiles = (int)((R + BM - 1) / BM);
        maxpix = (int)dense_max_slab_pixels(a, BM);
    } else {
        mtiles = (a.gi.NS + BM - 1) / BM;
        maxpix = BM + 2 * a.gi.P + 2;
    }
    size_t lds = (size_t)((maxpix * 8 + NTHREADS - 1) / NTHREADS * NTHREADS) * 16;
    if (lds < (size_t)WM * WN * 8192) lds = (size_t)WM * WN * 8192;
    if (lds > 160 * 1024) return WSI_EINVAL;
    if (PAIR && (!DENSE || MT % 2 || a.gi.W % 64 || ((long long)a.gi.N * a.gi.H * a.gi.W) % BM)) return WSI_EINVAL;
    if (a.in_up) {
        constexpr int CPL = PFmt<PLANES>::CPL;
        if (a.up_c <= 0 || a.up_c % CPL || a.up_c > a.gi.C || (a.up_c < a.gi.C && !a.in) || a.gup.H * 2 != a.gi.H || a.gup.W * 2 != a.gi.W ||
            a.gup.N != a.gi.N || (a.flags & (CONV_IN96 | CONV_RESID96)) || a.in2 ||
            (size_t)pf_alloc_pixels(a.gup.N, a.gup.H, a.gup.W) * a.up_c * PFmt<PLANES>::BPC > (size_t)0x7fffffff)
            return WSI_EINVAL;
    }
    auto k = conv3x3s1_slab3_kernel<MT, WM, WN, PLANES, MINW, DENSE, ABL, PAIR>;
    if (lds > 64 * 1024) {
        if (hipFuncSetAttribute((const void*)k, hipFuncAttributeMaxDynamicSharedMemorySize, (int)lds) != hipSuccess)
            return WSI_EINVAL;
    }
    const int grid = (a.flags & CONV_XCD_ORDER) ? (mtiles + 7) / 8 * 8 * nblocks : (a.flags & CONV_XCD_RANGES) ? (mtiles * nblocks + 7) / 8 * 8 : mtiles * nblocks;
    hipLaunchKernelGGL(k, dim3(grid), dim3(NTHREADS), lds, st, a);
    return hipGetLastError() == hipSuccess ? WSI_OK : WSI_EFAULT;
}


template <int MINW, int NCT = 0, bool IN96 = true>
__global__ __launch_bounds__(256, MINW) void conv3x3s1_rows_kernel(ConvArgs a) {
    extern __shared__ __attribute__((aligned(16))) char smem[];
    constexpr int MT = 4, WN = 2, BM = 256, NTHREADS = 256, RESID_NBUF = 2;
    const int tid = threadIdx.x, lane = tid & 63;
    WSTAMP(const unsigned long long st_begin = __builtin_readcyclecounter(); unsigned long long st_pro = 0, st_line = 0, st_tap = 0, st_a = 0;)
    const int wave = __builtin_amdgcn_readfirstlane(tid >> 6);
    const int wm = wave / WN, wn = wave % WN;
    const int l31 = lane & 31, h = lane >> 5;
    const int nblocks = a.go.C / (WN * 32);
    int nb = blockIdx.x % nblocks, mtile = blockIdx.x / nblocks;
    if (a.flags & CONV_XCD_RANGES) {
        const int chunk = gridDim.x >> 3, lin = (blockIdx.x & 7) * chunk + (blockIdx.x >> 3);
        nb = lin % nblocks;
        mtile = lin / nblocks;
        if (mtile >= (a.gi.N * a.gi.H * a.gi.W) / BM) return;
    }
    const int P = a.gi.P;
    const int ntile = nb * WN + wn;
    const int NC = NCT ? NCT : a.gi.C / 32;
    constexpr bool in96 = IN96;
    const size_t in_pixstride = in96 ? (size_t)96 : (size_t)a.gi.C * 4;
    const int in_line = in96 ? 0 : 128;
    const int p0 = pf_pos_of_index(a.gi, mtile * BM);
    const int slab0 = p0 - P - 1;
    const int npieces = (5 * P + 66) * 8;
    const int xoff0 = wm * 32 + l31;
    const size_t slab_byte0 = (size_t)slab0 * in_pixstride;
    const size_t in_bytes = (size_t)pf_alloc_pixels(a.gi.N, a.gi.H, a.gi.W) * in_pixstride;
    const __amdgpu_buffer_rsrc_t xrs = __builtin_amdgcn_make_buffer_rsrc(
        (void*)((const char*)a.in + slab_byte0), 0, (int)min(in_bytes - slab_byte0, (size_t)0x7fffffff), 0x00020000);
    int xvoff;
    bool xact = true;
    {
        const int i = wave * 64 + lane, Pl = i >> 3, sl = (i & 7) ^ ((Pl >> 1) & 7);
        xvoff = Pl * (int)in_pixstride + (in96 ? mx96_piece(sl) : sl) * 16;
        if (in96) xact = mx96_stored(sl);
    }
    const __amdgpu_buffer_rsrc_t wrs = __builtin_amdgcn_make_buffer_rsrc(
        (void*)((const char*)a.wpk + (size_t)ntile * NC * 9 * 4096), 0, NC * 9 * 4096, 0x00020000);
    const int wvoff = lane * 16;

    f32x16 acc[1][MT];
    auto wload = [&](bf16x8(&w)[4], int soff) {
#pragma unroll
        for (int f = 0; f < 4; ++f)
            w[f] = __builtin_bit_cast(bf16x8, __builtin_amdgcn_raw_buffer_load_b128(wrs, wvoff, soff + f * 1024, 0));
    };
    auto xload = [&](bf16x8(&x)[4], int Pl) {
        asm volatile("" : "+v"(Pl));
        const int base = lds_xbase(Pl, h);
#pragma unroll
        for (int f = 0; f < 4; ++f) x[f] = *(const bf16x8*)(smem + (base ^ (f << 5)));
    };

    bf16x8 wbuf[3][4], xf[2][4];
    constexpr bool XLINE = !IN96 && NCT > 0;
    if constexpr (XLINE) {
#pragma unroll
        for (int dy = 0; dy < 3; ++dy) wload(wbuf[dy], (dy * 3) * 4096);
    }
    WSTAMP(const unsigned long long st_setup = __builtin_readcyclecounter();)
#pragma unroll NCT ? NCT : 1
    for (int c = 0; c < (NCT ? NCT : NC); ++c) {
        WSTAMP(st_a = __builtin_readcyclecounter();)
        if (c) __syncthreads();
        {
            const __amdgpu_buffer_rsrc_t xr = in96 ? __builtin_amdgcn_make_buffer_rsrc((void*)((const char*)a.in + (size_t)c * (size_t)a.plane96 + slab_byte0), 0,
                                                                                        (int)min(in_bytes - slab_byte0, (size_t)0x7fffffff), 0x00020000)
                                                   : xrs;
            for (int i0 = wave * 64, r = 0; i0 < npieces; i0 += NTHREADS, ++r)
                if (xact) dma16_buf(xr, smem + (size_t)i0 * 16, xvoff, c * in_line + r * (NTHREADS / 8) * (int)in_pixstride);
        }
        asm volatile("s_waitcnt vmcnt(0)" ::: "memory");
        __syncthreads();
        WSTAMP(if (c) st_line += __builtin_readcyclecounter() - st_a; else st_pro = __builtin_readcyclecounter() - st_a; st_a = __builtin_readcyclecounter();)
        if (in96) {
            mx96_rebuild_hi6(smem, npieces >> 3, tid, NTHREADS);
            __syncthreads();
        }
        WSTAMP(st_tap += __builtin_readcyclecounter() - st_a;)
        int Pc = P;
        asm volatile("" : "+s"(Pc));
        const int sline = c * 9 * 4096;
        if constexpr (!XLINE) {
#pragma unroll
            for (int dy = 0; dy < 3; ++dy) wload(wbuf[dy], sline + (dy * 3) * 4096);
        }
        if (c == 0) acc_init_bias<MT>(acc[0], a.bias, ntile, lane);
        xload(xf[0], xoff0);
#pragma unroll
        for (int dx = 0; dx < 3; ++dx) {
#pragma unroll
            for (int j = 0; j < 6; ++j) {
                const int k = dx * 6 + j;
                if (j < 5) xload(xf[(k + 1) & 1], xoff0 + (j + 1) * Pc + dx);
                else if (dx < 2) xload(xf[(k + 1) & 1], xoff0 + dx + 1);
                __builtin_amdgcn_sched_barrier(0);
#pragma unroll
                for (int mt = 0; mt < MT; ++mt) {
                    const int dy = j - mt;
                    if (dy >= 0 && dy < 3) acc[0][mt] = mfma_mx6(acc[0][mt], wbuf[dy], xf[k & 1]);
                }
                __builtin_amdgcn_sched_barrier(0);
                if (j >= 3 && (dx < 2 || (XLINE && c + 1 < NC))) {
                    wload(wbuf[j - 3], dx < 2 ? sline + ((j - 3) * 3 + dx + 1) * 4096 : sline + (9 + (j - 3) * 3) * 4096);
                    __builtin_amdgcn_sched_barrier(0);
                }
            }
        }
    }
    WSTAMP(const unsigned long long st_loop_end = __builtin_readcyclecounter();)
    int qs[MT];
    bool valid[MT];
#pragma unroll
    for (int mt = 0; mt < MT; ++mt) {
        qs[mt] = p0 + mt * P + wm * 32 + l31;
        valid[mt] = true;
    }
    if (a.resid) __syncthreads();
    conv_tail_mx<1, MT, RESID_NBUF>(a, acc, qs, valid, ntile, lane, smem + wave * (RESID_NBUF * 4096), slab0);
#ifdef WSI_STUDY
    asm volatile("s_waitcnt vmcnt(0)" ::: "memory");
    if (lane == 0 && (blockIdx.x & 63) == 0) {
        const unsigned long long st_end = __builtin_readcyclecounter();
        atomicAdd(&g_wide_stamps[0], 1ull);
        atomicAdd(&g_wide_stamps[1], st_end - st_begin);
        atomicAdd(&g_wide_stamps[2], st_setup - st_begin);
        atomicAdd(&g_wide_stamps[3], st_pro);
        atomicAdd(&g_wide_stamps[4], st_line);
        atomicAdd(&g_wide_stamps[5], st_tap);
        atomicAdd(&g_wide_stamps[6], st_end - st_loop_end);
    }
#endif
}

template <int MINW>
static int launch_rows(const ConvArgs& a, hipStream_t st) {
    const bool nc2 = a.gi.C == 64;
    constexpr int BM = 256, NTHREADS = 256;
    if (a.go.C % 64 || a.gi.C % 32 || a.gi.W != 64 || a.gi.H % 4 || a.in2) return WSI_EINVAL;
    const int nblocks = a.go.C / 64;
    const long long R = (long long)a.gi.N * a.gi.H * a.gi.W;
    const int mtiles = (int)(R / BM);
    const int npix = 5 * a.gi.P + 66;
    size_t lds = (size_t)((npix * 8 + NTHREADS - 1) / NTHREADS * NTHREADS) * 16;
    if (lds < (size_t)4 * 8192) lds = (size_t)4 * 8192;
    const bool i96 = a.flags & CONV_IN96;
    auto k = nc2 ? (i96 ? conv3x3s1_rows_kernel<MINW, 2, true> : conv3x3s1_rows_kernel<MINW, 2, false>)
                 : (i96 ? conv3x3s1_rows_kernel<MINW, 0, true> : conv3x3s1_rows_kernel<MINW, 0, false>);
    if (lds > 64 * 1024 && hipFuncSetAttribute((const void*)k, hipFuncAttributeMaxDynamicSharedMemorySize, (int)lds) != hipSuccess)
        return WSI_EINVAL;
    const int grid = (a.flags & CONV_XCD_RANGES) ? (mtiles * nblocks + 7) / 8 * 8 : mtiles * nblocks;
    hipLaunchKernelGGL(k, dim3(grid), dim3(NTHREADS), lds, st, a);
    return hipGetLastError() == hipSuccess ? WSI_OK : WSI_EFAULT;
}


constexpr int L1P_SLAB_PIX = 392;
constexpr int L1P_SLAB = L1P_SLAB_PIX * 128;
constexpr int L1P_STAGE = 16 * 3072;
constexpr int L1P_LDS = 2 * L1P_SLAB + L1P_STAGE;
template <int NCT>
__global__ __launch_bounds__(320, 1) void conv3x3s1_l1p_kernel(ConvArgs a) {
    static_assert(NCT >= 2 && NCT % 2 == 0, "the slab buffer of a unit is its line's parity; the staging area needs two lines per tile");
    extern __shared__ __attribute__((aligned(16))) char smem[];
    constexpr int MT = 4, P = 65, NPIX = 391;
    char* const stage = smem + 2 * L1P_SLAB;
    const int tid = threadIdx.x, lane = tid & 63;
    const int wave = __builtin_amdgcn_readfirstlane(tid >> 6);
    const bool producer = wave == 4;
    const int wm = (wave >> 1) & 1, wn = wave & 1;
    const int l31 = lane & 31, h = lane >> 5;
    constexpr int NC = NCT;
    const int in_pixstride = 96;
    const int mtiles = (a.gi.N * a.gi.H * a.gi.W) >> 8;
    const int xcd = blockIdx.x & 7, slot = blockIdx.x >> 3, per = gridDim.x >> 3;
    const int chunk = (mtiles + 7) >> 3;
    const int t_lo = xcd * chunk, t_hi = min(t_lo + chunk, mtiles);
    const int ntl = t_hi - t_lo > slot ? (t_hi - t_lo - slot + per - 1) / per : 0;
    const int nunits = ntl * NC;
    if (nunits == 0) return;
    auto tile_p0 = [&](int k) { return pf_pos_of_index(a.gi, (t_lo + slot + k * per) << 8); };

    int sv[2];
    bool sact[2];
#pragma unroll
    for (int par = 0; par < 2; ++par) {
        const int Pl = 8 * par + (lane >> 3), sl = (lane & 7) ^ ((Pl >> 1) & 7);
        sv[par] = (lane >> 3) * in_pixstride + mx96_piece(sl) * 16;
        sact[par] = mx96_stored(sl);
    }
    const int r_pixstride = 96;
    int rv[3];
#pragma unroll
    for (int k = 0; k < 3; ++k) {
        const int g = 64 * k + lane;
        rv[k] = (g / 6) * r_pixstride + (g % 6) * 16;
    }
    auto dma_slab = [&](int u) {
        const int k = u / NC, c = u - k * NC;
        const size_t byte0 = (size_t)(tile_p0(k) - P - 1) * in_pixstride;
        const size_t in_bytes = (size_t)pf_alloc_pixels(a.gi.N, a.gi.H, a.gi.W) * in_pixstride;
        const __amdgpu_buffer_rsrc_t rs = __builtin_amdgcn_make_buffer_rsrc((void*)((const char*)a.in + (size_t)c * (size_t)a.plane96 + byte0), 0,
                                                                             (int)min(in_bytes - byte0, (size_t)0x7fffffff), 0x00020000);
        const unsigned dst = lds_addr_of(smem + (u & 1) * L1P_SLAB);
        for (int r = 0; r < (NPIX * 8 + 63) / 64; ++r) {
            const bool on = sact[r & 1] && (r * 64 + lane) < NPIX * 8;
            if (on) dma16_buf_asm(rs, dst + r * 1024, sv[r & 1], r * 8 * in_pixstride);
        }
    };
    auto dma_resid = [&](int k) {
        const int p0 = tile_p0(k);
        const size_t byte0 = (size_t)p0 * r_pixstride;
        const size_t r_bytes = (size_t)pf_alloc_pixels(a.go.N, a.go.H, a.go.W) * r_pixstride;
        for (int w = 0; w < 4; ++w) {
            const __amdgpu_buffer_rsrc_t rs = __builtin_amdgcn_make_buffer_rsrc((void*)((const char*)a.resid + (size_t)(w & 1) * (size_t)a.plane96 + byte0), 0,
                                                                                 (int)min(r_bytes - byte0, (size_t)0x7fffffff), 0x00020000);
            for (int mt = 0; mt < MT; ++mt) {
                const int soff = (mt * P + (w >> 1) * 32) * r_pixstride;
                const unsigned dst = lds_addr_of(stage + (w * MT + mt) * 3072);
#pragma unroll
                for (int k3 = 0; k3 < 3; ++k3) dma16_buf_asm(rs, dst + k3 * 1024, rv[k3], soff);
            }
        }
    };
    auto barrier = [&]() {
        asm volatile("s_waitcnt lgkmcnt(0)" ::: "memory");
        __builtin_amdgcn_s_barrier();
        asm volatile("" ::: "memory");
    };

    const int ntile = wn;
    const __amdgpu_buffer_rsrc_t wrs = __builtin_amdgcn_make_buffer_rsrc(
        (void*)((const char*)a.wpk + (size_t)ntile * NC * 9 * 4096), 0, NC * 9 * 4096, 0x00020000);
    const int wvoff = lane * 16;
    f32x16 acc[1][MT];
    bf16x8 wbuf[3][4], xf[2][4];
    auto wload = [&](bf16x8(&w)[4], int soff) {
#pragma unroll
        for (int f = 0; f < 4; ++f)
            w[f] = __builtin_bit_cast(bf16x8, __builtin_amdgcn_raw_buffer_load_b128(wrs, wvoff, soff + f * 1024, 0));
    };
    const int xoff0 = wm * 32 + l31;

    if (producer) {
        dma_slab(0);
        asm volatile("s_waitcnt vmcnt(0)" ::: "memory");
    }
    barrier();
    if (producer && nunits > 1) dma_slab(1);
    mx96_rebuild_hi6(smem, NPIX, tid, 320);
    barrier();

    for (int k = 0; k < ntl; ++k) {
#pragma unroll
    for (int c = 0; c < NC; ++c) {
        const int u = k * NC + c;
        const bool last_line = c == NC - 1;
        if (producer) {
            asm volatile("s_waitcnt vmcnt(0)" ::: "memory");
        } else {
            const char* const xl = smem + (c & 1) * L1P_SLAB;
            auto xload = [&](bf16x8(&x)[4], int Pl) {
                asm volatile("" : "+v"(Pl));
                const int base = lds_xbase(Pl, h);
#pragma unroll
                for (int f = 0; f < 4; ++f) x[f] = *(const bf16x8*)(xl + (base ^ (f << 5)));
            };
            if (c == 0) acc_init_bias<MT>(acc[0], a.bias, ntile, lane);
#pragma unroll
            for (int dy = 0; dy < 3; ++dy) wload(wbuf[dy], (c * 9 + dy * 3) * 4096);
            int Pc = P;
            asm volatile("" : "+s"(Pc));
            const int sline = c * 9 * 4096;
            xload(xf[0], xoff0);
#pragma unroll
            for (int dx = 0; dx < 3; ++dx) {
#pragma unroll
                for (int j = 0; j < 6; ++j) {
                    const int kk = dx * 6 + j;
                    if (j < 5) xload(xf[(kk + 1) & 1], xoff0 + (j + 1) * Pc + dx);
                    else if (dx < 2) xload(xf[(kk + 1) & 1], xoff0 + dx + 1);
                    __builtin_amdgcn_sched_barrier(0);
#pragma unroll
                    for (int mt = 0; mt < MT; ++mt) {
                        const int dy = j - mt;
                        if (dy >= 0 && dy < 3) acc[0][mt] = mfma_mx6(acc[0][mt], wbuf[dy], xf[kk & 1]);
                    }
                    __builtin_amdgcn_sched_barrier(0);
                    if (j >= 3 && dx < 2) {
                        wload(wbuf[j - 3], sline + ((j - 3) * 3 + dx + 1) * 4096);
                        __builtin_amdgcn_sched_barrier(0);
                    }
                }
            }
        }
        barrier();
        if (producer) {
            if (u + 2 < nunits) dma_slab(u + 2);
            if (a.resid && u + 1 < nunits && (u + 1) % NC == NC - 1) dma_resid((u + 1) / NC);
        }
        if (u + 1 < nunits) mx96_rebuild_hi6(smem + ((c + 1) & 1) * L1P_SLAB, NPIX, tid, 320);
        barrier();
        if (!producer && last_line) {
            const int p0 = tile_p0(k);
            int qs[MT];
            bool valid[MT];
#pragma unroll
            for (int mt = 0; mt < MT; ++mt) {
                qs[mt] = p0 + mt * P + wm * 32 + l31;
                valid[mt] = true;
            }
            if (a.resid) {
                bf16x8 iw[4];
                {
                    int lo = l31;
                    asm volatile("" : "+v"(lo));
                    const int pp = mx_line_pos(lo), f0 = mx6_field_of_pos(pp);
                    f16x8 k0, k1;
#pragma unroll
                    for (int jj = 0; jj < 8; ++jj) {
                        k0[jj] = (pp == 8 * h + jj) ? (_Float16)1.0f : (_Float16)0.0f;
                        k1[jj] = (pp == 16 + 8 * h + jj) ? (_Float16)1.0f : (_Float16)0.0f;
                    }
                    unsigned q[6];
#pragma unroll
                    for (int d = 0; d < 6; ++d) {
                        const int bit = 6 * f0 + 3 - 32 * d;
                        q[d] = (h == 0 && bit >= 0 && bit < 32) ? (1u << (bit & 31)) : 0u;
                    }
                    iw[0] = __builtin_bit_cast(bf16x8, k0);
                    iw[1] = __builtin_bit_cast(bf16x8, k1);
                    iw[2] = __builtin_bit_cast(bf16x8, u32x4{q[0], q[1], q[2], q[3]});
                    iw[3] = __builtin_bit_cast(bf16x8, u32x4{q[4], q[5], 127u, 0u});
                }
#pragma unroll
                for (int mt = 0; mt < MT; ++mt) {
                    const char* t = stage + (wave * MT + mt) * 3072 + l31 * 96;
                    bf16x8 x[4];
                    x[0] = *(const bf16x8*)(t + h * 16);
                    x[1] = *(const bf16x8*)(t + (2 + h) * 16);
                    if (h == 0) {
                        x[2] = *(const bf16x8*)(t + 4 * 16);
                        x[3] = *(const bf16x8*)(t + 5 * 16);
                    } else {
                        x[2] = __builtin_bit_cast(bf16x8, u32x4{0u, 0u, 0u, 0u});
                        x[3] = x[2];
                    }
                    acc[0][mt] = mfma_mx6(acc[0][mt], iw, x);
                }
            }
            conv_epilogue_mx<MT>(a, acc[0], qs, valid, ntile, lane);
        }
    }
    }
}

static int g_l1p_grid = 0;
static int launch_l1p(const ConvArgs& a, hipStream_t st) {
    if (a.go.C != 64 || a.gi.C % 32 || a.gi.C < 64 || a.gi.W != 64 || a.gi.H % 4 || a.in2 || a.in_up || !(a.flags & CONV_IN96) ||
        (a.resid && !(a.flags & CONV_RESID96)))
        return WSI_EINVAL;
    if (!g_l1p_grid) {
        int dev = 0, cus = 0;
        if (hipGetDevice(&dev) != hipSuccess || hipDeviceGetAttribute(&cus, hipDeviceAttributeMultiprocessorCount, dev) != hipSuccess || cus < 8)
            return WSI_EFAULT;
        g_l1p_grid = cus / 8 * 8;
    }
    const long long mtiles = (long long)a.gi.N * a.gi.H * a.gi.W / 256;
    int grid = g_l1p_grid;
    if (mtiles < grid) grid = (int)((mtiles + 7) / 8 * 8);
    if (a.gi.C != 64) return WSI_EINVAL;
    auto k = conv3x3s1_l1p_kernel<2>;
    if (hipFuncSetAttribute((const void*)k, hipFuncAttributeMaxDynamicSharedMemorySize, L1P_LDS) != hipSuccess) return WSI_EINVAL;
    hipLaunchKernelGGL(k, dim3(grid), dim3(320), L1P_LDS, st, a);
    return hipGetLastError() == hipSuccess ? WSI_OK : WSI_EFAULT;
}


template <int PLANES, int MINW, int ABL = 0, int WM = 2, int WN = 2, int NT = 2, bool D8 = false>
__global__ __launch_bounds__(WM* WN * 64, MINW) void conv3x3s1_wide_kernel(ConvArgs a) {
    extern __shared__ __attribute__((aligned(16))) char smem[];
    constexpr int MT = 4, BM = WM * 128, NTHREADS = WM * WN * 64, NTILES = WN * NT, WB = NTILES * 4096;
    constexpr int D8_ZB = 304;
    static_assert(!D8 || (BM == 256 && NTHREADS == 256), "D8: four whole 8 x 8 images per tile, 32 slab pixels per DMA round");
    constexpr int RESID_NBUF = 4;
    char* const wl = smem;
    char* const xl = smem + 2 * WB;
    const int tid = threadIdx.x, lane = tid & 63;
    WSTAMP(const unsigned long long st_begin = __builtin_readcyclecounter(); unsigned long long st_pro = 0, st_line = 0, st_tap = 0, st_a = 0;)
    const int wave = __builtin_amdgcn_readfirstlane(tid >> 6);
    const int wm = wave / WN, wn = wave % WN;
    const int l31 = lane & 31, h = lane >> 5;
    const int nblocks = a.go.C / (NTILES * 32);
    int nb = blockIdx.x % nblocks, mtile = blockIdx.x / nblocks;
    if (a.flags & CONV_XCD_RANGES) {
        const int chunk = gridDim.x >> 3, lin = (blockIdx.x & 7) * chunk + (blockIdx.x >> 3);
        nb = lin % nblocks;
        mtile = lin / nblocks;
        if (mtile >= (a.gi.N * a.gi.H * a.gi.W + BM - 1) / BM) return;
    }
    const int P = a.gi.P;
    const int NC = a.gi.C / PFmt<PLANES>::CPL;
    const size_t in_pixstride = (size_t)a.gi.C * PFmt<PLANES>::BPC;
    int xoff[MT];
    bool valid[MT];
    int slab0, npieces;
    const int lpix = a.gi.W < 32 ? dense_lane_pixel(l31) : l31;
    const int Rtot = a.gi.N * a.gi.H * a.gi.W;
    if constexpr (D8) {
        const int i0 = mtile * BM, i1 = min(i0 + BM, Rtot) - 1, n0 = i0 >> 6;
        slab0 = a.gi.G + n0 * a.gi.S - P;
        npieces = (1 + 9 * ((i1 >> 6) - n0 + 1)) * 64;
#pragma unroll
        for (int mt = 0; mt < MT; ++mt) {
            const int i = i0 + wm * MT * 32 + mt * 32 + lpix;
            valid[mt] = i < Rtot;
            const int ii = valid[mt] ? i : i1;
            xoff[mt] = 8 * (9 * ((ii >> 6) - n0) + ((ii >> 3) & 7)) + (ii & 7) - 1;
        }
    } else {
        auto pos = [&](int i) { return pf_pos_of_index(a.gi, i); };
        const int i0 = mtile * BM, i1 = min(i0 + BM, Rtot) - 1;
        slab0 = pos(i0) - P - 1;
        npieces = (pos(i1) + P + 1 - slab0 + 1) * 8;
#pragma unroll
        for (int mt = 0; mt < MT; ++mt) {
            const int i = i0 + wm * MT * 32 + mt * 32 + lpix;
            valid[mt] = i < Rtot;
            xoff[mt] = pos(valid[mt] ? i : i1) - slab0 - (P + 1);
        }
    }
    const bool d8_left = D8 && (lpix & 7) == 0, d8_right = D8 && (lpix & 7) == 7;
    constexpr int RPIX = D8 ? 36 : NTHREADS / 8;
    static_assert((NTHREADS / 8) % 16 == 0, "whole swizzle periods per DMA round");
    const size_t slab_byte0 = (size_t)slab0 * in_pixstride;
    const size_t in_bytes = (size_t)pf_alloc_pixels(a.gi.N, a.gi.H, a.gi.W) * in_pixstride;
    const __amdgpu_buffer_rsrc_t xrs = __builtin_amdgcn_make_buffer_rsrc(
        (void*)((const char*)a.in + slab_byte0), 0, (int)min(in_bytes - slab_byte0, (size_t)0x7fffffff), 0x00020000);
    int xvoff;
    {
        const int i = wave * 64 + lane, Pl = i >> 3, sl = (i & 7) ^ ((Pl >> 1) & 7);
        xvoff = (D8 ? (Pl >> 3) * 9 + (Pl & 7) : Pl) * (int)in_pixstride + sl * 16;
    }
    if constexpr (D8) {
        if (tid < 128) *(u32x4*)(xl + D8_ZB * 128 + tid * 16) = u32x4{0u, 0u, 0u, 0u};
    }
    const __amdgpu_buffer_rsrc_t wrs = __builtin_amdgcn_make_buffer_rsrc(
        (void*)((const char*)a.wpk + (size_t)(nb * NTILES) * NC * 9 * 4096), 0, NTILES * NC * 9 * 4096, 0x00020000);
    const int wvoff = (tid & 255) * 16;
    const unsigned wl_addr = lds_addr_of(wl), xl_addr = lds_addr_of(xl);
    auto wdma = [&](int c, int t, int wboff) {
#pragma unroll
        for (int p0 = 0; p0 < NTILES * 256; p0 += NTHREADS) {
            static_assert((NTILES * 256) % NTHREADS == 0, "whole DMA rounds");
            const int pw = p0 + wave * 64;
            dma16_buf_asm(wrs, wl_addr + wboff + pw * 16, wvoff, (((pw >> 8) * NC + c) * 9 + t) * 4096);
        }
    };

    f32x16 acc[NT][MT];
#pragma unroll
    for (int nt = 0; nt < NT; ++nt) {
        if constexpr (PLANES == 3) acc_init_bias<MT>(acc[nt], a.bias, nb * NTILES + wn * NT + nt, lane);
        else {
#pragma unroll
            for (int mt = 0; mt < MT; ++mt)
#pragma unroll
                for (int r = 0; r < 16; ++r) acc[nt][mt][r] = 0.f;
        }
    }

    auto xload = [&](bf16x8(&x)[4], int Pl, int tx = 1) {
        asm volatile("" : "+v"(Pl));
        if constexpr (D8) {
            if (tx == 0) Pl = d8_left ? D8_ZB + (Pl & 15) : Pl;
            if (tx == 2) Pl = d8_right ? D8_ZB + (Pl & 15) : Pl;
        }
        const int base = lds_xbase(Pl, h);
#pragma unroll
        for (int f = 0; f < 4; ++f) x[f] = *(const bf16x8*)(xl + (base ^ (f << 5)));
    };
    auto wread = [&](bf16x8(&w)[4], const char* wb, int nt) {
        const char* src = wb + (wn * NT + nt) * 4096 + lane * 16;
#pragma unroll
        for (int f = 0; f < 4; ++f) w[f] = *(const bf16x8*)(src + f * 1024);
    };

    int kpar = 0;
    WSTAMP(const unsigned long long st_setup = __builtin_readcyclecounter();)
    for (int c = 0; c < NC; ++c) {
        WSTAMP(st_a = __builtin_readcyclecounter();)
        if (c) __syncthreads();
        for (int i0 = wave * 64, r = 0; i0 < npieces; i0 += NTHREADS, ++r)
            dma16_buf_asm(xrs, xl_addr + i0 * 16, xvoff, c * 128 + r * RPIX * (int)in_pixstride);
        wdma(c, 0, kpar * WB);
        asm volatile("s_waitcnt vmcnt(0)" ::: "memory");
        __syncthreads();
        WSTAMP(if (c) st_line += __builtin_readcyclecounter() - st_a; else st_pro = __builtin_readcyclecounter() - st_a;)
        int Pc = D8 ? 8 : P;
        asm volatile("" : "+s"(Pc));
        bf16x8 xf[2][4], wf[NT][4];
        xload(xf[0], xoff[0], 0);
#pragma unroll
        for (int t = 0; t < 9; ++t) {
            const char* wb = wl + kpar * WB;
            if (t < 8) wdma(c, t + 1, (kpar ^ 1) * WB);
#pragma unroll
            for (int nt = 0; nt < NT; ++nt) wread(wf[nt], wb, nt);
            const int toff = (t / 3) * Pc + (t % 3);
            const int toff_next = ((t + 1) / 3) * Pc + ((t + 1) % 3);
#pragma unroll
            for (int mt = 0; mt < MT; ++mt) {
                const int k = t * MT + mt;
                if constexpr (!(ABL & 32)) {
                    if (mt + 1 < MT) xload(xf[(k + 1) & 1], xoff[mt + 1] + toff, t % 3);
                    else if (t < 8) xload(xf[(k + 1) & 1], xoff[0] + toff_next, (t + 1) % 3);
                }
                __builtin_amdgcn_sched_barrier(0);
                const bf16x8(&x)[4] = xf[k & 1];
#pragma unroll
                for (int nt = 0; nt < NT; ++nt) {
                    mfma_step<PLANES>(acc[nt][mt], wf[nt], x);
                }
            }
            if (t < 8) {
                WSTAMP(st_a = __builtin_readcyclecounter();)
                asm volatile("s_waitcnt vmcnt(0)" ::: "memory");
                __syncthreads();
                WSTAMP(st_tap += __builtin_readcyclecounter() - st_a;)
            }
            kpar ^= 1;
        }
    }
    WSTAMP(const unsigned long long st_loop_end = __builtin_readcyclecounter();)
    int qs[MT];
#pragma unroll
    for (int mt = 0; mt < MT; ++mt) {
        if constexpr (D8) {
            const int i = mtile * BM + wm * MT * 32 + mt * 32 + lpix;
            qs[mt] = pf_pos_of_index(a.gi, valid[mt] ? i : min(mtile * BM + BM, Rtot) - 1);
        } else {
            qs[mt] = xoff[mt] + slab0 + (P + 1);
        }
    }
    if constexpr (PLANES == 3) {
        if (a.in2) {
            const int NC2 = a.in2_c / 32;
            const size_t ps2 = (size_t)a.in2_c * 4, sb2 = (size_t)slab0 * ps2;
            const size_t bytes2 = (size_t)pf_alloc_pixels(a.gi.N, a.gi.H, a.gi.W) * ps2;
            const __amdgpu_buffer_rsrc_t xrs2 = __builtin_amdgcn_make_buffer_rsrc(
                (void*)((const char*)a.in2 + sb2), 0, (int)min(bytes2 - sb2, (size_t)0x7fffffff), 0x00020000);
            int xvoff2;
            {
                const int i = wave * 64 + lane, Pl = i >> 3, sl = (i & 7) ^ ((Pl >> 1) & 7);
                xvoff2 = (D8 ? (Pl >> 3) * 9 + (Pl & 7) : Pl) * (int)ps2 + sl * 16;
            }
            const char* wsrc2 = (const char*)a.wpk2 + (size_t)(nb * NTILES) * NC2 * 4096 + (size_t)(tid & 255) * 16;
#pragma unroll
            for (int nt = 0; nt < NT; ++nt) {
                f32x16 b2[1];
                acc_init_bias<1>(b2, a.bias2, nb * NTILES + wn * NT + nt, lane);
#pragma unroll
                for (int mt = 0; mt < MT; ++mt)
#pragma unroll
                    for (int r = 0; r < 16; ++r) acc[nt][mt][r] += b2[0][r];
            }
            for (int c = 0; c < NC2; ++c) {
                __syncthreads();
                for (int i0 = wave * 64, r = 0; i0 < npieces; i0 += NTHREADS, ++r)
                    dma16_buf(xrs2, xl + (size_t)i0 * 16, xvoff2, c * 128 + r * RPIX * (int)ps2);
#pragma unroll
                for (int p0 = 0; p0 < NTILES * 256; p0 += NTHREADS) {
                    const int pw = p0 + wave * 64;
                    dma16(wsrc2 + (size_t)((pw >> 8) * NC2 + c) * 4096, wl + pw * 16);
                }
                asm volatile("s_waitcnt vmcnt(0)" ::: "memory");
                __syncthreads();
                bf16x8 wf2[NT][4];
#pragma unroll
                for (int nt = 0; nt < NT; ++nt) wread(wf2[nt], wl, nt);
#pragma unroll
                for (int mt = 0; mt < MT; ++mt) {
                    bf16x8 x2[4];
                    xload(x2, xoff[mt] + (D8 ? 8 : P) + 1);
#pragma unroll
                    for (int nt = 0; nt < NT; ++nt) mfma_step<PLANES>(acc[nt][mt], wf2[nt], x2);
                }
            }
        }
        if (a.resid) __syncthreads();
        conv_tail_mx<NT, MT, RESID_NBUF>(a, acc, qs, valid, nb * NTILES + wn * NT, lane, smem + wave * (RESID_NBUF * 4096), slab0);
    } else {
        char* scratch = nullptr;
        if (PLANES == 2 && a.resid && !(a.flags & CONV_RESID_DIRECT)) {
            __syncthreads();
            scratch = xl + wave * 8192;
        }
#pragma unroll
        for (int nt = 0; nt < NT; ++nt) conv_epilogue_q<MT, PLANES>(a, acc[nt], qs, valid, nb * NTILES + wn * NT + nt, lane, scratch);
    }
#ifdef WSI_STUDY
    asm volatile("s_waitcnt vmcnt(0)" ::: "memory");
    if (lane == 0 && (blockIdx.x & 63) == 0) {
        const unsigned long long st_end = __builtin_readcyclecounter();
        atomicAdd(&g_wide_stamps[0], 1ull);
        atomicAdd(&g_wide_stamps[1], st_end - st_begin);
        atomicAdd(&g_wide_stamps[2], st_setup - st_begin);
        atomicAdd(&g_wide_stamps[3], st_pro);
        atomicAdd(&g_wide_stamps[4], st_line);
        atomicAdd(&g_wide_stamps[5], st_tap);
        atomicAdd(&g_wide_stamps[6], st_end - st_loop_end);
    }
#endif
}


template <int PLANES, int MINW, int ABL = 0, int WM = 2, int WN = 2, int NT = 2, bool D8 = false>
static int launch_wide(const ConvArgs& a, hipStream_t st) {
    constexpr int BM = WM * 128, NTHREADS = WM * WN * 64, BN = WN * NT * 32;
    if (a.go.C % BN) return WSI_EINVAL;
    if constexpr (!D8 && ABL == 0 && WM == 2 && WN == 2 && NT == 2) {
        if (g_routes.wide_d8 && a.gi.W == 8 && a.gi.H == 8) return launch_wide<PLANES, MINW, 0, 2, 2, 2, true>(a, st);
    }
    const int nblocks = a.go.C / BN;
    const long long R = (long long)a.gi.N * a.gi.H * a.gi.W;
    const int mtiles = (int)((R + BM - 1) / BM);
    size_t xbytes = D8 ? (size_t)(304 + 16) * 128
                       : (size_t)((dense_max_slab_pixels(a, BM) * 8 + NTHREADS - 1) / NTHREADS * NTHREADS) * 16;
    if (xbytes < (size_t)WM * WN * 8192) xbytes = (size_t)WM * WN * 8192;
    size_t lds = 2 * (BN / 32) * 4096 + xbytes;
    if (PLANES == 3 && lds < (size_t)WM * WN * 4 * 4096) lds = (size_t)WM * WN * 4 * 4096;
    if (lds > 160 * 1024) return WSI_EINVAL;
    auto k = conv3x3s1_wide_kernel<PLANES, MINW, ABL, WM, WN, NT, D8>;
    if (lds > 64 * 1024 && hipFuncSetAttribute((const void*)k, hipFuncAttributeMaxDynamicSharedMemorySize, (int)lds) != hipSuccess)
        return WSI_EINVAL;
    const int grid = (a.flags & CONV_XCD_RANGES) ? (mtiles * nblocks + 7) / 8 * 8 : mtiles * nblocks;
    hipLaunchKernelGGL(k, dim3(grid), dim3(NTHREADS), lds, st, a);
    return hipGetLastError() == hipSuccess ? WSI_OK : WSI_EFAULT;
}


template <int MT, int WM, int WN, int PLANES, int MINW, bool FUSE, int PMAX = 34, int ABL = 0>
__global__ __launch_bounds__(WM* WN * 64, MINW) void conv3x3s2_slab_kernel(ConvArgs a) {
    extern __shared__ __attribute__((aligned(16))) char smem[];
    constexpr int BM = WM * MT * 32;
    constexpr int NTHREADS = WM * WN * 64;
    constexpr int KMAX = ((4 * BM + 2 * PMAX + 2) * 8 + NTHREADS - 1) / NTHREADS;
    constexpr int NT = FUSE ? 10 : 9;
    constexpr int RING = FUSE ? 2 : 3;
    const int tid = threadIdx.x, lane = tid & 63;
    const int wave = __builtin_amdgcn_readfirstlane(tid >> 6);
    const int wm = wave / WN, wn = wave % WN;
    const int l31 = lane & 31, h = lane >> 5;
    const int nblocks = a.go.C / (WN * 32);
    int nb = blockIdx.x % nblocks, mtile = blockIdx.x / nblocks;
    if (a.flags & CONV_XCD_ORDER) {
        const int per = 8 * nblocks, r = blockIdx.x % per;
        nb = r >> 3;
        mtile = (blockIdx.x / per) * 8 + (r & 7);
        if (mtile >= (a.go.NS + BM - 1) / BM) return;
    }
    const int P = a.go.P;
    const int q0 = a.go.G + mtile * BM;
    const int R01 = BM, R10 = 2 * BM + 1, R11 = 3 * BM + 1 + P;
    const int npix = 4 * BM + 2 * P + 2;
    const int npieces = npix * 8;
    const int ntile = nb * WN + wn;
    const int NC = a.gi.C / PFmt<PLANES>::CPL;
    const size_t in_pixstride = (size_t)a.gi.C * PFmt<PLANES>::BPC;
    const __amdgpu_buffer_rsrc_t wrs = __builtin_amdgcn_make_buffer_rsrc(
        (void*)((const char*)a.wpk + (size_t)ntile * NC * 9 * 4096), 0, NC * 9 * 4096, 0x00020000);
    const __amdgpu_buffer_rsrc_t wrd = __builtin_amdgcn_make_buffer_rsrc(
        (void*)((const char*)(FUSE ? a.wpk2 : a.wpk) + (size_t)ntile * NC * 4096), 0, NC * 4096, 0x00020000);
    const int wvoff = lane * 16;

    int srcpix[KMAX];
#pragma unroll
    for (int k = 0; k < KMAX; ++k) {
        const int i = wave * 64 + k * NTHREADS + lane;
        const int Pl = i >> 3;
        int reg = 0, j = Pl;
        if (Pl >= R11) { reg = 3; j = Pl - R11; }
        else if (Pl >= R10) { reg = 2; j = Pl - R10; }
        else if (Pl >= R01) { reg = 1; j = Pl - R01; }
        const int py = reg >> 1, px = reg & 1;
        const int v = q0 - (py ? P : 0) - px + j;
        int src = 0;
        int r = v - a.go.G;
        if (Pl < npix && r >= 0 && r < a.go.NS) {
            const int n = r / a.go.S;
            r -= n * a.go.S;
            const int y = r / P, x = r - y * P;
            if (x != a.go.W && y != a.go.H) src = a.gi.G + n * a.gi.S + (2 * y + py) * a.gi.P + 2 * x + px;
        }
        const int sl = (i & 7) ^ ((Pl >> 1) & 7);
        srcpix[k] = (int)((unsigned)src * (unsigned)in_pixstride + (unsigned)sl * 16u);
    }
    const __amdgpu_buffer_rsrc_t irs = __builtin_amdgcn_make_buffer_rsrc((void*)a.in, 0, 0xffffffff, 0x00020000);

    f32x16 acc[MT], accd[FUSE ? MT : 1];
    if constexpr (PLANES == 3) {
        acc_init_bias<MT>(acc, a.bias, ntile, lane);
        if constexpr (FUSE) acc_init_bias<MT>(accd, a.bias2, ntile, lane);
    } else {
#pragma unroll
        for (int mt = 0; mt < MT; ++mt)
#pragma unroll
            for (int r = 0; r < 16; ++r) acc[mt][r] = 0.f;
        if constexpr (FUSE) {
#pragma unroll
            for (int mt = 0; mt < MT; ++mt)
#pragma unroll
                for (int r = 0; r < 16; ++r) accd[mt][r] = 0.f;
        }
    }
    int xoff[MT];
#pragma unroll
    for (int mt = 0; mt < MT; ++mt) xoff[mt] = wm * MT * 32 + mt * 32 + l31;

    auto wload = [&](bf16x8(&w)[4], int c, int t) {
#pragma unroll
        for (int f = 0; f < 4; ++f) {
            const u32x4 v = (t < 9) ? __builtin_amdgcn_raw_buffer_load_b128(wrs, wvoff + f * 1024, (c * 9 + t) * 4096, 0)
                                    : __builtin_amdgcn_raw_buffer_load_b128(wrd, wvoff + f * 1024, c * 4096, 0);
            w[f] = __builtin_bit_cast(bf16x8, v);
        }
    };
    auto xload = [&](bf16x8(&x)[4], int Pl) {
        const int base = lds_xbase(Pl, h);
#pragma unroll
        for (int f = 0; f < 4; ++f) x[f] = *(const bf16x8*)(smem + (base ^ (f << 5)));
    };
    auto tap_off = [&](int t, int Pc) {
        if (t == 9) return 0;
        const int kh = t / 3, kw = t % 3;
        const int py = kh != 1, px = kw != 1;
        const int base = py ? (px ? 3 * BM + 1 + Pc : 2 * BM + 1) : (px ? BM : 0);
        const int back = (py ? Pc : 0) + px;
        return base + back + (kh == 0 ? -Pc : 0) + (kw == 0 ? -1 : 0);
    };

    bf16x8 wbuf[RING][4], xf[2][4];
    wload(wbuf[0], 0, 0);
    for (int c = 0; c < NC; ++c) {
        int Pc = P;
        asm volatile("" : "+s"(Pc));
        if (c) __syncthreads();
#pragma unroll
        for (int k = 0; k < KMAX; ++k) {
            const int i0 = wave * 64 + k * NTHREADS;
            if (i0 < npieces)
                dma16_buf(irs, smem + (size_t)i0 * 16, srcpix[k], c * 128);
        }
        asm volatile("s_waitcnt vmcnt(0)" ::: "memory");
        __syncthreads();
        xload(xf[0], xoff[0] + tap_off(0, Pc));
#pragma unroll
        for (int t = 0; t < NT; ++t) {
            asm volatile("" ::: "memory");
            if constexpr (!(ABL & 16)) {
                if (t + 1 < NT) wload(wbuf[(t + 1) % RING], c, t + 1);
                else if (c + 1 < NC) wload(wbuf[0], c + 1, 0);
            }
            asm volatile("" ::: "memory");
            const int toff = tap_off(t, Pc);
            const int toff_next = t + 1 < NT ? tap_off(t + 1, Pc) : 0;
#pragma unroll
            for (int mt = 0; mt < MT; ++mt) {
                const int k = t * MT + mt;
                if (mt + 1 < MT) xload(xf[(k + 1) & 1], xoff[mt + 1] + toff);
                else if (t + 1 < NT) xload(xf[(k + 1) & 1], xoff[0] + toff_next);
                const bf16x8(&w)[4] = wbuf[t % RING];
                const bf16x8(&x)[4] = xf[k & 1];
                f32x16& d = (FUSE && t == 9) ? accd[FUSE ? mt : 0] : acc[mt];
                if constexpr (PLANES == 3) {
                    d = mfma_mx6(d, w, x);
                } else if constexpr (PLANES == 2) {
                    mfma_step<2>(d, w, x);
                } else {
#pragma unroll
                    for (int f = 0; f < 4; ++f) d = mfma_bf16(w[f], x[f], d);
                }
            }
        }
    }
    conv_epilogue_any<MT, PLANES>(a, acc, q0 + wm * MT * 32, ntile, lane);
    if constexpr (FUSE) {
        ConvArgs a2 = a;
        a2.out = a.out2; a2.bias = a.bias2; a2.resid = nullptr; a2.relu = 0;
        a2.wpk = a.wpk2; a2.ksize = 1;
        conv_epilogue_any<MT, PLANES>(a2, accd, q0 + wm * MT * 32, ntile, lane);
    }
}

template <int MT, int WM, int WN, int PLANES, int MINW, bool FUSE, int PMAX = 34, int ABL = 0>
static int launch_s2slab(const ConvArgs& a, hipStream_t st) {
    constexpr int BM = WM * MT * 32, NTHREADS = WM * WN * 64;
    if (a.go.C % (WN * 32) || a.go.P > PMAX) return WSI_EINVAL;
    if ((unsigned long long)pf_alloc_pixels(a.gi.N, a.gi.H, a.gi.W) * a.gi.C * PFmt<PLANES>::BPC >= 0xffffffffull) return WSI_EINVAL;
    const int mtiles = (a.go.NS + BM - 1) / BM;
    const int nblocks = a.go.C / (WN * 32);
    const int npieces = (4 * BM + 2 * a.go.P + 2) * 8;
    const size_t lds = (size_t)((npieces + NTHREADS - 1) / NTHREADS * NTHREADS) * 16;
    if (lds > 160 * 1024) return WSI_EINVAL;
    auto k = conv3x3s2_slab_kernel<MT, WM, WN, PLANES, MINW, FUSE, PMAX, ABL>;
    if (lds > 64 * 1024) {
        if (hipFuncSetAttribute((const void*)k, hipFuncAttributeMaxDynamicSharedMemorySize, (int)lds) != hipSuccess)
            return WSI_EINVAL;
    }
    const int grid = (a.flags & CONV_XCD_ORDER) ? (mtiles + 7) / 8 * 8 * nblocks : mtiles * nblocks;
    hipLaunchKernelGGL(k, dim3(grid), dim3(NTHREADS), lds, st, a);
    return hipGetLastError() == hipSuccess ? WSI_OK : WSI_EFAULT;
}

template <int PLANES, bool DENSE, bool DS, int NT = 2>
__global__ __launch_bounds__(512, 1) void conv3x3s2_wide_kernel(ConvArgs a) {
    extern __shared__ __attribute__((aligned(16))) char smem[];
    static_assert(NT == 2 || (NT == 4 && !DS), "four channel tiles per wave: no second accumulator set");
    constexpr int MT = 2, BM = 256, NTILES = 2 * NT, ULEN = NT == 2 ? 2 : 1;
    constexpr int WBUF = NTILES * 4096, XB = 45056;
    constexpr int NWB = 2 * ULEN;
    char* const wl = smem;
    char* const xl0 = smem + NWB * WBUF;
    const int tid = threadIdx.x, lane = tid & 63;
    const int wave = __builtin_amdgcn_readfirstlane(tid >> 6);
    const int wm = wave >> 1, wn = wave & 1;
    const int l31 = lane & 31, h = lane >> 5;
    const int nblocks = a.go.C / (NTILES * 32);
    const int chunk = gridDim.x >> 3, lin = (blockIdx.x & 7) * chunk + (blockIdx.x >> 3);
    const int nb = lin % nblocks, mtile = lin / nblocks;
    if (mtile >= a.mtiles) return;
    const int P = a.go.P;
    int q0, qlast, qs[MT];
    bool valid[MT];
    if constexpr (!DENSE) {
        q0 = a.go.G + mtile * BM;
        qlast = q0 + BM - 1;
#pragma unroll
        for (int mt = 0; mt < MT; ++mt) {
            qs[mt] = q0 + wm * MT * 32 + mt * 32 + l31;
            valid[mt] = pf_is_pixel(a.go, qs[mt]);
        }
    } else {
        const int HW = a.go.H * a.go.W, R = a.go.N * HW;
        auto pos = [&](int i) { return pf_pos_of_index(a.go, i); };
        const int i0 = mtile * BM, i1 = min(i0 + BM, R) - 1;
        q0 = pos(i0);
        qlast = pos(i1);
#pragma unroll
        for (int mt = 0; mt < MT; ++mt) {
            const int i = i0 + wm * MT * 32 + mt * 32 + (a.go.W < 32 ? dense_lane_pixel(l31) : l31);
            valid[mt] = i < R;
            qs[mt] = pos(valid[mt] ? i : i1);
        }
    }
    const int NC = a.gi.C / PFmt<PLANES>::CPL;
    const size_t in_pixstride = (size_t)a.gi.C * PFmt<PLANES>::BPC;
    const __amdgpu_buffer_rsrc_t wrs = __builtin_amdgcn_make_buffer_rsrc(
        (void*)((const char*)a.wpk + (size_t)(nb * NTILES) * NC * 9 * 4096), 0, NTILES * NC * 9 * 4096, 0x00020000);
    const __amdgpu_buffer_rsrc_t wrd = __builtin_amdgcn_make_buffer_rsrc(
        (void*)((const char*)(DS ? a.wpk2 : a.wpk) + (size_t)(nb * NTILES) * NC * 4096), 0, NTILES * NC * 4096, 0x00020000);
    const int wvoff = lane * 16;
    auto wdma = [&](int c, int t, char* wb) {
#pragma unroll
        for (int j = 0; j < NTILES; ++j) {
            if (t < 9) dma16_buf_asm(wrs, lds_addr_of(wb) + j * 4096 + (wave - 4) * 1024, wvoff, ((j * NC + c) * 9 + t) * 4096 + (wave - 4) * 1024);
            else dma16_buf_asm(wrd, lds_addr_of(wb) + j * 4096 + (wave - 4) * 1024, wvoff, (j * NC + c) * 4096 + (wave - 4) * 1024);
        }
    };
    auto xdma = [&](int c, int ph, char* xb) {
        const int back = ((ph & 2) ? P : 0) + (ph & 1);
        const char* src = (const char*)a.in + ((size_t)ph * a.in_split_pixels + (size_t)(q0 - back)) * in_pixstride + c * 128;
        const int npieces = (qlast - q0 + 1 + back) * 8;
        for (int i0 = wave * 64; i0 < npieces; i0 += 256) {
            const int i = i0 + lane;
            const int Pl = i >> 3, sl = (i & 7) ^ ((Pl >> 1) & 7);
            dma16_asm(src + (size_t)Pl * in_pixstride + sl * 16, lds_addr_of(xb) + i0 * 16);
        }
    };
    auto wread = [&](bf16x8(&w)[NT][4], const char* wb) {
        const char* src = wb + (wn * NT) * 4096 + lane * 16;
#pragma unroll
        for (int nt = 0; nt < NT; ++nt) {
#pragma unroll
            for (int f = 0; f < 4; ++f) w[nt][f] = *(const bf16x8*)(src + nt * 4096 + f * 1024);
        }
    };

    f32x16 acc[NT][MT], accd[DS ? NT : 1][DS ? MT : 1];
#pragma unroll
    for (int nt = 0; nt < NT; ++nt) {
        if constexpr (PLANES == 3) {
            acc_init_bias<MT>(acc[nt], a.bias, nb * NTILES + wn * NT + nt, lane);
            if constexpr (DS) acc_init_bias<MT>(accd[nt], a.bias2, nb * NTILES + wn * NT + nt, lane);
        } else {
#pragma unroll
            for (int mt = 0; mt < MT; ++mt)
#pragma unroll
                for (int r = 0; r < 16; ++r) {
                    acc[nt][mt][r] = 0.f;
                    if constexpr (DS) accd[nt][mt][r] = 0.f;
                }
        }
    }

    constexpr int SPL = DS ? 10 : 9;
    constexpr int STEP_TAP[10] = {4, DS ? 9 : 3, DS ? 3 : 5, DS ? 5 : 1, DS ? 1 : 7, DS ? 7 : 0, DS ? 0 : 2, DS ? 2 : 6, DS ? 6 : 8, 8};
    constexpr int UNIT0[4] = {0, DS ? 2 : 1, DS ? 4 : 3, DS ? 6 : 5};
    constexpr int NSTEP[4] = {DS ? 2 : 1, 2, 2, 4};
    const int NG = NC * SPL;
    auto wdma_step = [&](int c, int j) {
        const int cc = c + j / SPL, g = cc * SPL + j % SPL;
        if (g < NG) wdma(cc, STEP_TAP[j % SPL], wl + (g & (NWB - 1)) * WBUF);
    };
    if (wave < 4) xdma(0, 0, xl0);
    else { wdma_step(0, 0); if (NSTEP[0] == 2 && ULEN == 2) wdma_step(0, 1); }
    asm volatile("s_waitcnt vmcnt(0)" ::: "memory");
    __syncthreads();
    for (int c = 0; c < NC; ++c) {
#pragma unroll
        for (int ph = 0; ph < 4; ++ph) {
            const char* xl = xl0 + (size_t)(ph & 1) * XB;
            if (wave < 4) {
                if (ph < 3) xdma(c, ph + 1, xl0 + (size_t)((ph + 1) & 1) * XB);
                else if (c + 1 < NC) xdma(c + 1, 0, xl0);
            }
#pragma unroll
            for (int kp = 0; kp < NSTEP[ph]; kp += ULEN) {
                const int j0 = UNIT0[ph] + kp;
                const int ulen = NSTEP[ph] - kp >= ULEN ? ULEN : 1;
                const int jn = j0 + ulen;
                const int nlen = ULEN == 1 ? 1 : (kp + 2 < NSTEP[ph]) ? 2 : (ph < 3 ? (NSTEP[ph + 1] >= 2 ? 2 : 1) : (NSTEP[0] >= 2 ? 2 : 1));
                if (wave >= 4) { wdma_step(c, jn); if (nlen == 2) wdma_step(c, jn + 1); }
#pragma unroll
                for (int k = 0; k < ulen; ++k) {
                    const int g = c * SPL + j0 + k;
// ... 223 lines not shown
```

wsi_segmentation_pipeline_amd/csrc/conv_dev.h:

```cpp
#pragma once
#include "common.h"

static __device__ __forceinline__ void dma16(const void* gsrc, char* lds_wave_base) {
    __builtin_amdgcn_global_load_lds((const __attribute__((address_space(1))) void*)gsrc,
                                     (__attribute__((address_space(3))) void*)lds_wave_base, 16, 0, 0);
}

static __device__ __forceinline__ void dma16_buf(__amdgpu_buffer_rsrc_t rs, char* lds_wave_base, int voff, int soff) {
    __builtin_amdgcn_raw_ptr_buffer_load_lds(rs, (__attribute__((address_space(3))) void*)lds_wave_base, 16, voff, soff, 0, 0);
}

static __device__ __forceinline__ unsigned lds_addr_of(const char* p) {
    return (unsigned)(size_t)(const __attribute__((address_space(3))) char*)p;
}
static __device__ __forceinline__ void dma16_asm(const void* gsrc, unsigned lds) {
    unsigned keep;
    asm volatile("s_mov_b32 %0, m0\n\ts_mov_b32 m0, %1\n\ts_nop 0\n\tglobal_load_lds_dwordx4 %2, off\n\ts_mov_b32 m0, %0"
                 : "=&s"(keep) : "s"(lds), "v"(gsrc) : "memory");
}
static __device__ __forceinline__ void dma16_buf_asm(__amdgpu_buffer_rsrc_t rs, unsigned lds, int voff, int soff) {
    unsigned keep;
    asm volatile("s_mov_b32 %0, m0\n\ts_mov_b32 m0, %1\n\ts_nop 0\n\tbuffer_load_dwordx4 %2, %3, %4 offen lds\n\ts_mov_b32 m0, %0"
                 : "=&s"(keep) : "s"(lds), "v"(voff), "s"(rs), "s"(soff) : "memory");
}

static __device__ __forceinline__ void resid_tile_dma(const void* resid, int q_own, size_t pixstride, size_t line_off, int lane, char* dst) {
#pragma unroll
    for (int j = 0; j < 4; ++j) {
        const int pp = 8 * j + (lane >> 3);
        const int q = __shfl(q_own, pp);
        const int sl = (lane & 7) ^ ((pp >> 1) & 7);
        dma16((const char*)resid + (size_t)q * pixstride + line_off + sl * 16, dst + j * 1024);
    }
}

static __device__ __forceinline__ void resid_tile_dma_buf(__amdgpu_buffer_rsrc_t rs, int q_rel, int pixstride, int line_off, int lane, char* dst) {
#pragma unroll
    for (int j = 0; j < 4; ++j) {
        const int pp = 8 * j + (lane >> 3);
        const int q = __shfl(q_rel, pp);
        const int sl = (lane & 7) ^ ((pp >> 1) & 7);
        dma16_buf(rs, dst + j * 1024, q * pixstride + sl * 16, line_off);
    }
}

static __device__ __forceinline__ bool mx96_stored(int s) { return s != 5 && s != 7; }
static __device__ __forceinline__ int mx96_piece(int s) { return s == 6 ? 5 : s; }

static __device__ __forceinline__ void mx96_rebuild_hi6(char* slab, int npix, int tid, int nthreads) {
    for (int Pl = tid; Pl < npix; Pl += nthreads) {
        const int key = (Pl >> 1) & 7;
        char* line = slab + Pl * 128;
        unsigned D[16];
#pragma unroll
        for (int s4 = 0; s4 < 4; ++s4) {
            const u32x4 d = *(const u32x4*)(line + ((s4 ^ key) << 4));
            D[4 * s4] = d[0]; D[4 * s4 + 1] = d[1]; D[4 * s4 + 2] = d[2]; D[4 * s4 + 3] = d[3];
        }
        const int sh = (int)(*(const unsigned*)(line + ((6 ^ key) << 4) + 12) & 255u);
        u32x16 e;
#pragma unroll
        for (int k = 0; k < 16; ++k)
            e[k] = __builtin_amdgcn_perm(D[8 + (k >> 1)], D[k >> 1], (k & 1) ? 0x07060302u : 0x05040100u);
        u32x6 q;
        const float scale = sh ? mx_scale_value(sh) : 1.f;
        asm volatile("v_cvt_scalef32_pk32_fp6_f16 %0, %1, %2" : "=&v"(q) : "v"(e), "v"(scale));
        *(u32x4*)(line + ((5 ^ key) << 4)) = u32x4{q[0], q[1], q[2], q[3]};
        *(u32x4*)(line + ((7 ^ key) << 4)) = u32x4{q[4], q[5], (unsigned)sh, 0u};
    }
}

static __device__ __forceinline__ void resid_tile_dma_buf96(__amdgpu_buffer_rsrc_t rs, int q_rel, int pixstride, int line_off, int lane, char* dst) {
#pragma unroll
    for (int j = 0; j < 4; ++j) {
        const int pp = 8 * j + (lane >> 3);
        const int q = __shfl(q_rel, pp);
        const int sl = (lane & 7) ^ ((pp >> 1) & 7);
        if (mx96_stored(sl)) dma16_buf(rs, dst + j * 1024, q * pixstride + mx96_piece(sl) * 16, line_off);
    }
}

template <int MT, int PLANES>
static __device__ __forceinline__ void conv_epilogue_q(const ConvArgs& a, f32x16 (&acc)[MT], const int (&qs)[MT],
                                                       const bool (&valid)[MT], int ntile, int lane, char* scratch = nullptr) {
    typedef typename PairElem<PLANES>::T E;
    typedef __attribute__((ext_vector_type(4))) E Ex4;
    const int h = lane >> 5, l31 = lane & 31;
    const size_t pixstride = (size_t)a.go.C * PFmt<PLANES>::BPC;
    const size_t chan_off = (size_t)ntile * (32 * PFmt<PLANES>::BPC) + (size_t)(4 * h) * 2;
    size_t poff[MT], ooff[MT];
#pragma unroll
    for (int mt = 0; mt < MT; ++mt) {
        poff[mt] = (size_t)(valid[mt] ? qs[mt] : a.go.G) * pixstride + chan_off;
        ooff[mt] = a.out_split_pixels ? pf_out_offset(a.go, a.out_split_pixels, valid[mt] ? qs[mt] : a.go.G, pixstride) + chan_off : poff[mt];
    }

    const bool via_lds = PLANES == 2 && a.resid && scratch;
    Ex4 rh[MT][4], rl[MT][4];
    if (via_lds) {
        resid_tile_dma(a.resid, valid[0] ? qs[0] : a.go.G, pixstride, (size_t)ntile * 128, lane, scratch);
    } else if (a.resid) {
#pragma unroll
        for (int mt = 0; mt < MT; ++mt)
#pragma unroll
            for (int g = 0; g < 4; ++g) {
                const char* rp = (const char*)a.resid + poff[mt] + 16 * g;
                if (CONV_STUDY(a, CONV_NONTEMPORAL)) {
                    rh[mt][g] = __builtin_nontemporal_load((const Ex4*)rp);
                    if constexpr (PLANES == 2) rl[mt][g] = __builtin_nontemporal_load((const Ex4*)(rp + 64));
                } else {
                    rh[mt][g] = *(const Ex4*)rp;
                    if constexpr (PLANES == 2) rl[mt][g] = *(const Ex4*)(rp + 64);
                }
            }
    }
    float bias[16], wsi[16];
#pragma unroll
    for (int g = 0; g < 4; ++g)
#pragma unroll
        for (int i = 0; i < 4; ++i) bias[g * 4 + i] = a.bias[ntile * 32 + 8 * g + 4 * h + i];
    if constexpr (PLANES == 2) {
        const float* ws = conv_wscale_inv(a.wpk, a.go.C, a.gi.C, a.ksize) + ntile * 32 + 4 * h;
#pragma unroll
        for (int g = 0; g < 4; ++g) {
            const f32x4 v = *(const f32x4*)(ws + 8 * g);
#pragma unroll
            for (int i = 0; i < 4; ++i) wsi[g * 4 + i] = v[i];
        }
    }
#pragma unroll
    for (int mt = 0; mt < MT; ++mt) {
        if (via_lds) {
            asm volatile("s_waitcnt vmcnt(0)" ::: "memory");
            if (mt + 1 < MT)
                resid_tile_dma(a.resid, valid[mt + 1] ? qs[mt + 1] : a.go.G, pixstride, (size_t)ntile * 128, lane, scratch + ((mt + 1) & 1) * 4096);
            const char* t = scratch + (mt & 1) * 4096 + l31 * 128 + 8 * h;
            const int sw = (l31 >> 1) & 7;
#pragma unroll
            for (int g = 0; g < 4; ++g) {
                rh[mt][g] = *(const Ex4*)(t + ((g ^ sw) << 4));
                rl[mt][g] = *(const Ex4*)(t + (((4 + g) ^ sw) << 4));
            }
        }
#pragma unroll
        for (int g = 0; g < 4; ++g) {
            float v[4];
#pragma unroll
            for (int i = 0; i < 4; ++i) {
                if constexpr (PLANES == 2) v[i] = acc[mt][4 * g + i] * wsi[4 * g + i] + bias[4 * g + i];
                else v[i] = acc[mt][4 * g + i] + bias[4 * g + i];
            }
            if (a.resid) {
#pragma unroll
                for (int i = 0; i < 4; ++i) v[i] += (float)rh[mt][g][i];
                if constexpr (PLANES == 2) {
#pragma unroll
                    for (int i = 0; i < 4; ++i) v[i] += (float)rl[mt][g][i];
                }
            }
            Ex4 hi, lo;
            if constexpr (PLANES == 2) {
                const float lo_clamp = a.relu ? 0.f : -65504.f;
#pragma unroll
                for (int i = 0; i < 4; ++i) {
                    v[i] = __builtin_amdgcn_fmed3f(v[i], lo_clamp, 65504.f);
                    hi[i] = (E)v[i];
                    lo[i] = (E)(v[i] - (float)hi[i]);
                }
            } else {
                if (a.relu) {
#pragma unroll
                    for (int i = 0; i < 4; ++i) v[i] = fmaxf(v[i], 0.f);
                }
#pragma unroll
                for (int i = 0; i < 4; ++i) {
                    hi[i] = (E)v[i];
                    lo[i] = (E)(v[i] - (float)hi[i]);
                }
            }
            if (valid[mt] && !CONV_STUDY(a, CONV_ABL_NO_STORE)) {
                char* op = (char*)a.out + ooff[mt] + 16 * g;
                if (CONV_STUDY(a, CONV_NONTEMPORAL)) {
                    __builtin_nontemporal_store(hi, (Ex4*)op);
                    if constexpr (PLANES == 2) __builtin_nontemporal_store(lo, (Ex4*)(op + 64));
                } else {
                    *(Ex4*)op = hi;
                    if constexpr (PLANES == 2) *(Ex4*)(op + 64) = lo;
                }
            }
        }
    }
}

static __device__ __forceinline__ f32x16 mfma_mx6(f32x16 d, const bf16x8 (&w)[4], const bf16x8 (&x)[4]) {
    d = __builtin_amdgcn_mfma_f32_32x32x16_f16(__builtin_bit_cast(f16x8, w[0]), __builtin_bit_cast(f16x8, x[0]), d, 0, 0, 0);
    d = __builtin_amdgcn_mfma_f32_32x32x16_f16(__builtin_bit_cast(f16x8, w[1]), __builtin_bit_cast(f16x8, x[1]), d, 0, 0, 0);
    const i32x4 wq = __builtin_bit_cast(i32x4, w[2]), wr = __builtin_bit_cast(i32x4, w[3]);
    const i32x4 xq = __builtin_bit_cast(i32x4, x[2]), xr = __builtin_bit_cast(i32x4, x[3]);
    const i32x8 wa = {wq[0], wq[1], wq[2], wq[3], wr[0], wr[1], wr[2], wr[3]}, xa = {xq[0], xq[1], xq[2], xq[3], xr[0], xr[1], xr[2], xr[3]};
    return __builtin_amdgcn_mfma_scale_f32_32x32x64_f8f6f4(wa, xa, d, 2, 2, 0, wr[2], 0, xr[2]);
}

template <int MT>
static __device__ __forceinline__ void acc_init_bias(f32x16 (&acc)[MT], const float* bias, int ntile, int lane) {
    const int h = lane >> 5;
    float b[16];
#pragma unroll
    for (int g = 0; g < 4; ++g) {
        const f32x4 v = *(const f32x4*)(bias + ntile * 32 + 8 * g + 4 * h);
#pragma unroll
        for (int i = 0; i < 4; ++i) b[4 * g + i] = v[i];
    }
#pragma unroll
    for (int mt = 0; mt < MT; ++mt)
#pragma unroll
        for (int r = 0; r < 16; ++r) acc[mt][r] = b[r];
}

template <int MT, int MTN = MT>
static __device__ __forceinline__ void conv_epilogue_mx(const ConvArgs& a, f32x16 (&acc)[MT], const int (&qs)[MT],
                                                        const bool (&valid)[MT], int ntile, int lane, int mt0 = 0) {
    const int h = lane >> 5;
    const bool o96 = a.flags & CONV_OUT96;
    const size_t pixstride = o96 ? (size_t)96 : (size_t)a.go.C * 4;
    const float lo_clamp = a.relu ? 0.f : -65504.f;
#pragma unroll
    for (int mt = mt0; mt < mt0 + MTN; ++mt) {
        const size_t loff = (size_t)(valid[mt] ? qs[mt] : a.go.G) * pixstride + (o96 ? (size_t)ntile * (size_t)a.plane96 : (size_t)ntile * 128);
        f32x16 v = acc[mt];
        f32x16 hi, lo;
        f16x8 hv[2];
        float mv = 0.f, ml = 0.f;
#pragma unroll
        for (int r = 0; r < 16; r += 2) {
            const float v0 = __builtin_amdgcn_fmed3f(v[r], lo_clamp, 65504.f);
            const float v1 = __builtin_amdgcn_fmed3f(v[r + 1], lo_clamp, 65504.f);
            const f16x2 hh = __builtin_convertvector(f32x2{v0, v1}, f16x2);
            hv[r >> 3][r & 7] = hh[0];
            hv[r >> 3][(r & 7) + 1] = hh[1];
            hi[r] = (float)hh[0];
            hi[r + 1] = (float)hh[1];
            lo[r] = v0 - hi[r];
            lo[r + 1] = v1 - hi[r + 1];
            mv = fmaxf(mv, fmaxf(fabsf(hi[r]), fabsf(hi[r + 1])));
            ml = fmaxf(ml, fmaxf(fabsf(lo[r]), fabsf(lo[r + 1])));
        }
        pair_max2(mv, ml);
        const int sh = mx6_scale_byte(mv), sl = mx6_scale_byte(ml);
        const int sb = h ? sh : sl;
        swap32_halves(lo, hi);
        const u32x6 q = mx6_pack32(lo, hi, sb ? mx_scale_value(sb) : 1.f);
        if (valid[mt] && !CONV_STUDY(a, CONV_ABL_NO_STORE)) {
            char* ol = (char*)a.out + (a.out_split_pixels ? pf_out_offset(a.go, a.out_split_pixels, qs[mt], pixstride) + (size_t)ntile * 128 : loff);
            *(f16x8*)(ol + 32 * h) = hv[0];
            *(f16x8*)(ol + 32 * h + 16) = hv[1];
            if (!o96) {
                *(u32x4*)(ol + MX6_PLANE_LO(0) + 16 * h) = u32x4{q[0], q[1], q[2], q[3]};
                *(u32x4*)(ol + MX6_PLANE_HI(0) + 16 * h) = u32x4{q[4], q[5], (unsigned)sb, 0u};
            } else if (h == 0) {
                *(u32x4*)(ol + 64) = u32x4{q[0], q[1], q[2], q[3]};
                *(u32x4*)(ol + 80) = u32x4{q[4], q[5], (unsigned)sl, (unsigned)sh};
            }
        }
    }
}

template <int NT, int MT, int NBUF>
static __device__ __forceinline__ void conv_tail_mx(const ConvArgs& a, f32x16 (&acc)[NT][MT], const int (&qs)[MT], const bool (&valid)[MT],
                                                    int ntile0, int lane, char* scratch, int slab0) {
    constexpr int T = NT * MT;
    static_assert(MT % NBUF == 0 || NBUF % MT == 0, "a batch is part of one channel tile or whole channel tiles");
    static_assert(NBUF <= T && T % NBUF == 0, "whole batches");
    if (!a.resid) {
#pragma unroll
        for (int nt = 0; nt < NT; ++nt) conv_epilogue_mx<MT>(a, acc[nt], qs, valid, ntile0 + nt, lane);
        return;
    }
    const int h = lane >> 5, l31 = lane & 31;
    const bool r96 = a.flags & CONV_RESID96;
    const int pixstride = r96 ? 96 : a.go.C * 4;
    const size_t rbase = (size_t)slab0 * pixstride, rbytes = (size_t)pf_alloc_pixels(a.go.N, a.go.H, a.go.W) * pixstride;
    const __amdgpu_buffer_rsrc_t rrs = __builtin_amdgcn_make_buffer_rsrc((void*)((const char*)a.resid + rbase), 0,
                                                                          (int)min(rbytes - rbase, (size_t)0x7fffffff), 0x00020000);
    bf16x8 iw[4];
    {
        const int p = mx_line_pos(l31), f0 = mx6_field_of_pos(p);
        f16x8 k0, k1;
#pragma unroll
        for (int j = 0; j < 8; ++j) {
            k0[j] = (p == 8 * h + j) ? (_Float16)1.0f : (_Float16)0.0f;
            k1[j] = (p == 16 + 8 * h + j) ? (_Float16)1.0f : (_Float16)0.0f;
        }
        unsigned q[6];
#pragma unroll
        for (int d = 0; d < 6; ++d) {
            const int bit = 6 * f0 + 3 - 32 * d;
            q[d] = (h == 0 && bit >= 0 && bit < 32) ? (1u << (bit & 31)) : 0u;
        }
        iw[0] = __builtin_bit_cast(bf16x8, k0);
        iw[1] = __builtin_bit_cast(bf16x8, k1);
        iw[2] = __builtin_bit_cast(bf16x8, u32x4{q[0], q[1], q[2], q[3]});
        iw[3] = __builtin_bit_cast(bf16x8, u32x4{q[4], q[5], 127u, 0u});
    }
    auto rdma = [&](int k) {
        const int nt = k / MT, mt = k % MT;
        int qr = qs[mt] - slab0;
        asm volatile("" : "+v"(qr));
        if (r96) {
            const __amdgpu_buffer_rsrc_t prs = __builtin_amdgcn_make_buffer_rsrc(
                (void*)((const char*)a.resid + (size_t)(ntile0 + nt) * (size_t)a.plane96 + rbase), 0, (int)min(rbytes - rbase, (size_t)0x7fffffff), 0x00020000);
            resid_tile_dma_buf96(prs, qr, pixstride, 0, lane, scratch + (k % NBUF) * 4096);
        }
        else resid_tile_dma_buf(rrs, qr, pixstride, (ntile0 + nt) * 128, lane, scratch + (k % NBUF) * 4096);
    };
    const int xb = l31 * 128 + ((h ^ ((l31 >> 1) & 7)) << 4);
#pragma unroll
    for (int k = 0; k < NBUF; ++k) rdma(k);
#pragma unroll
    for (int b0 = 0; b0 < T; b0 += NBUF) {
        asm volatile("s_waitcnt vmcnt(0)" ::: "memory");
#pragma unroll
        for (int k = b0; k < b0 + NBUF; ++k) {
            const char* t = scratch + (k % NBUF) * 4096;
            bf16x8 x[4];
#pragma unroll
            for (int f = 0; f < 4; ++f) x[f] = *(const bf16x8*)(t + (xb ^ (f << 5)));
            if (r96 && h) {
                x[2] = __builtin_bit_cast(bf16x8, u32x4{0u, 0u, 0u, 0u});
                x[3] = x[2];
            }
            acc[k / MT][k % MT] = mfma_mx6(acc[k / MT][k % MT], iw, x);
        }
        if (b0 + NBUF < T) {
            asm volatile("s_waitcnt lgkmcnt(0)" ::: "memory");
#pragma unroll
            for (int k = b0 + NBUF; k < b0 + 2 * NBUF; ++k) rdma(k);
        }
        if constexpr (NBUF >= MT) {
#pragma unroll
            for (int nt = b0 / MT; nt < (b0 + NBUF) / MT; ++nt) conv_epilogue_mx<MT>(a, acc[nt], qs, valid, ntile0 + nt, lane);
        } else {
            conv_epilogue_mx<MT, NBUF>(a, acc[b0 / MT], qs, valid, ntile0 + b0 / MT, lane, b0 % MT);
        }
    }
}

template <int MT, int PLANES>
static __device__ __forceinline__ void conv_epilogue(const ConvArgs& a, f32x16 (&acc)[MT], int q_base, int ntile,
                                                     int lane) {
    int qs[MT];
    bool valid[MT];
#pragma unroll
    for (int mt = 0; mt < MT; ++mt) {
        qs[mt] = q_base + mt * 32 + (lane & 31);
        valid[mt] = pf_is_pixel(a.go, qs[mt]);
    }
    conv_epilogue_q<MT, PLANES>(a, acc, qs, valid, ntile, lane);
}

template <int MT, int PLANES>
static __device__ __forceinline__ void conv_epilogue_any(const ConvArgs& a, f32x16 (&acc)[MT], int q_base, int ntile, int lane) {
    if constexpr (PLANES == 3) {
        int qs[MT];
        bool valid[MT];
#pragma unroll
        for (int mt = 0; mt < MT; ++mt) {
            qs[mt] = q_base + mt * 32 + (lane & 31);
            valid[mt] = pf_is_pixel(a.go, qs[mt]);
        }
        conv_epilogue_mx<MT>(a, acc, qs, valid, ntile, lane);
    } else {
        conv_epilogue<MT, PLANES>(a, acc, q_base, ntile, lane);
    }
}

template <int MT, int PLANES>
static __device__ __forceinline__ void mfma_line(f32x16 (&acc)[MT], const bf16x8 (&wf)[4], const char* smem,
                                                 const int (&xbase)[MT]) {
    bf16x8 xf[2][4];
#pragma unroll
    for (int f = 0; f < 4; ++f) xf[0][f] = *(const bf16x8*)(smem + (xbase[0] ^ (f << 5)));
#pragma unroll
    for (int mt = 0; mt < MT; ++mt) {
        const bf16x8(&x)[4] = xf[mt & 1];
        if (mt + 1 < MT) {
#pragma unroll
            for (int f = 0; f < 4; ++f) xf[(mt + 1) & 1][f] = *(const bf16x8*)(smem + (xbase[mt + 1] ^ (f << 5)));
        }
        if constexpr (PLANES == 2) {
            acc[mt] = mfma16<2>(wf[2], x[0], acc[mt]);
            acc[mt] = mfma16<2>(wf[3], x[1], acc[mt]);
            acc[mt] = mfma16<2>(wf[0], x[2], acc[mt]);
            acc[mt] = mfma16<2>(wf[1], x[3], acc[mt]);
            acc[mt] = mfma16<2>(wf[0], x[0], acc[mt]);
            acc[mt] = mfma16<2>(wf[1], x[1], acc[mt]);
        } else {
#pragma unroll
            for (int f = 0; f < 4; ++f) acc[mt] = mfma_bf16(wf[f], x[f], acc[mt]);
        }
    }
}

static __device__ __forceinline__ int dense_lane_pixel(int l31) {
    return l31 < 4 ? l31 : l31 < 12 ? l31 + 12 : l31 < 16 ? l31 - 8 : l31 < 20 ? l31 + 8 : l31 < 28 ? l31 - 12 : l31;
}

static __device__ __forceinline__ int lds_xbase(int Pl, int h) { return Pl * 128 + ((h ^ ((Pl >> 1) & 7)) << 4); }
template <int PLANES>
static __device__ __forceinline__ void mfma_step(f32x16& d, const bf16x8 (&w)[4], const bf16x8 (&x)[4]) {
    if constexpr (PLANES == 3) {
        d = mfma_mx6(d, w, x);
    } else if constexpr (PLANES == 2) {
        d = mfma16<2>(w[2], x[0], d);
        d = mfma16<2>(w[3], x[1], d);
        d = mfma16<2>(w[0], x[2], d);
        d = mfma16<2>(w[1], x[3], d);
        d = mfma16<2>(w[0], x[0], d);
        d = mfma16<2>(w[1], x[1], d);
    } else {
#pragma unroll
        for (int f = 0; f < 4; ++f) d = mfma_bf16(w[f], x[f], d);
    }
}
```

wsi_segmentation_pipeline_amd/native.py:

```python
import contextlib
import ctypes as C
import enum
import os
import subprocess

_HERE = os.path.dirname(os.path.abspath(__file__))
LIB_PATH = os.path.join(_HERE, 'lib', 'libwsi_hip.so')
CSRC = os.path.join(_HERE, 'csrc')

_lib = None


class NativeLibraryMissing(RuntimeError):
    pass


class WsiTrunkWeights(C.Structure):
    _fields_ = [
        ('stem_w', C.c_void_p), ('stem_b', C.c_void_p),
        ('stem_w_u8', C.c_void_p), ('stem_b_u8', C.c_void_p), ('norm', C.c_float * 6),
        ('conv_w', C.c_void_p * 16), ('conv_b', C.c_void_p * 16),
        ('down_w', C.c_void_p * 3), ('down_b', C.c_void_p * 3),
        ('head_w', C.c_void_p), ('head_b', C.c_void_p), ('head_k', C.c_int),
        ('planes', C.c_int),
    ]


class WsiUnetDecoderWeights(C.Structure):
    _fields_ = [
        ('conv_w', C.c_void_p * 10), ('conv_b', C.c_void_p * 10), ('cin', C.c_int * 10), ('cout', C.c_int * 10),
        ('head_w', C.c_void_p), ('head_b', C.c_void_p), ('head_cin', C.c_int), ('classes', C.c_int), ('tail_w', C.c_void_p),
    ]


_vp, _i, _ll, _sz, _f, _d = C.c_void_p, C.c_int, C.c_longlong, C.c_size_t, C.c_float, C.c_double
SIGNATURES = {
    'wsi_hip_abi_version': (_i, []),
    'wsi_pf_bytes': (_sz, [_i, _i, _i, _i, _i]),
    'wsi_pf_pixel_index': (_ll, [_i, _i, _i, _i, _i]),
    'wsi_prepack_conv_bytes': (_sz, [_i, _i, _i, _i]),
    'wsi_prepack_conv': (_i, [_vp, _vp, _vp, _vp, _vp, _f, _i, _i, _i, _i, _vp, _vp]),
    'wsi_unet_tail_prepack_bytes': (_sz, []),
    'wsi_unet_tail_prepack': (_i, [_vp] * 10 + [_f, _vp, _vp, _i, _i, _i, _vp]),
    'wsi_unet_tail_bands': (_i, [_i, _i, _i]),
    'wsi_unet_tail_timeouts': (_i, [C.POINTER(C.c_ulonglong), _i]),
    'wsi_prepack_stem_bytes': (_sz, [_i]),
    'wsi_prepack_stem': (_i, [_vp, _vp, _vp, _vp, _vp, _f, _i, _vp, _vp]),
    'wsi_prepack_stem_u8': (_i, [_vp, _vp, _vp, _vp, _vp, _f, _vp, _vp, _i, _vp, _vp]),
    'wsi_normalize_u8_lut': (_i, [_vp, _vp, _vp]),
    'wsi_stem_conv7x7_bn_relu_maxpool': (_i, [_vp, _vp, _ll, _i, _i, _vp, _vp, _vp, _vp, _vp, _vp, _vp, _i, _i, _i, _vp, _vp, _i, _vp]),
    'wsi_stem_set_mode': (_i, [_i, _i]),
    'wsi_conv3x3_bn_act': (_i, [_vp, _vp, _vp, _vp, _vp, _i, _i, _i, _i, _i, _i, _i, _i, _vp]),
    'wsi_conv3x3_bn_act_cfg': (_i, [_vp, _vp, _vp, _vp, _vp, _i, _i, _i, _i, _i, _i, _i, _i, _i, _vp]),
    'wsi_conv3x3s2_ds_fused': (_i, [_vp, _vp, _vp, _vp, _vp, _vp, _vp, _i, _i, _i, _i, _i, _i, _vp]),
    'wsi_s2_slab_images': (_i, [_i, _i, _i, _i, _i]),
    'wsi_pf_split_bytes': (_sz, [_i, _i, _i, _i, _i]),
    'wsi_conv3x3_bn_act_split': (_i, [_vp] * 5 + [_i] * 7 + [_vp]),
    'wsi_conv3x3_up_concat_bn_act': (_i, [_vp] * 5 + [_i] * 8 + [_vp]),
    'wsi_conv3x3s2_ds_fused_split': (_i, [_vp] * 7 + [_i] * 6 + [_vp]),
    'wsi_conv_set_mode': (_i, [_i]),
    'wsi_conv1x1_bn': (_i, [_vp, _vp, _vp, _vp, _i, _i, _i, _i, _i, _i, _i, _vp]),
    'wsi_avgpool_fc': (_i, [_vp, _i, _i, _i, _i, _vp, _vp, _i, _vp, _vp, _i, _vp]),
    'wsi_linear': (_i, [_vp, _vp, _vp, _vp, _i, _i, _i, _i, _vp]),
    'wsi_pf_pack': (_i, [_vp, _vp, _i, _i, _i, _i, _i, _vp]),
    'wsi_pf_unpack': (_i, [_vp, _vp, _i, _i, _i, _i, _i, _vp]),
    'wsi_trunk_workspace_bytes': (_sz, [_i, _i, _i, _i]),
    'wsi_trunk_workspace_init': (_i, [_vp, _i, _i, _i, _i, _vp]),
    'wsi_trunk_workspace_release': (_i, [_vp]),
    'wsi_trunk_forward': (_i, [C.POINTER(WsiTrunkWeights), _vp, _vp, _ll, _i, _i, _vp, _vp, _i, _i, _i, _vp, _i, _vp, _vp, _vp, _vp]),
    'wsi_trunk_forward_tap': (_i, [C.POINTER(WsiTrunkWeights), _vp, _vp, _ll, _i, _i, _vp, _vp, _i, _i, _i, _vp, _i, _i, _vp, _vp]),
    'wsi_trunk_set_chunks': (_i, [_i, _i]),
    'wsi_prof_begin': (_i, [_i]),
    'wsi_prof_end': (_i, [_vp, _vp, _vp, _i]),
    'wsi_tile_gather': (_i, [_vp, _ll, _i, _i, _vp, _vp, _vp, _i, _i, _i, _vp]),
    'wsi_stitch_add': (_i, [_vp, _vp, _i, _i, _i, _i, _vp, _i, _i, _vp]),
    'wsi_stitch_add_dense': (_i, [_vp, _vp, _i, _i, _i, _i, _vp, _i, _i, _vp]),
    'wsi_softmax_threshold_argmax': (_i, [_vp, _i, _ll, _vp, _vp, _vp, _vp, _i, _vp, _vp]),
    'wsi_ring_create': (_i, [_vp, _i, _sz]),
    'wsi_ring_host_slot': (_vp, [_vp, _i]),
    'wsi_ring_wait_slot': (_i, [_vp, _i]),
    'wsi_ring_submit': (_i, [_vp, _i, _i, _i, _i, _ll, _vp, _ll]),
    'wsi_ring_fence': (_i, [_vp, _vp]),
    'wsi_ring_acquire': (_i, [_vp, _vp]),
    'wsi_ring_device': (_i, [_vp]),
    'wsi_ring_drain': (_i, [_vp]),
    'wsi_ring_destroy': (None, [_vp]),
    'wsi_resample_plan_create': (_i, [_vp, _i, _i, _i, _i]),
    'wsi_resample_plan_destroy': (None, [_vp]),
    'wsi_resample_scratch_bytes': (_sz, [_vp, _i]),
    'wsi_resample_tiles': (_i, [_vp, _vp, _ll, _i, _i, _vp, _i, _vp, _vp, _vp]),
    'wsi_find_nuclei_hsv': (_i, [_vp, _ll, _i, C.c_double, _vp, _vp]),
    'wsi_connected_components_scratch_bytes': (_sz, [_i, _i]),
    'wsi_connected_components': (_i, [_vp, _i, _i, _vp, _vp, _vp, _vp]),
    'wsi_kmeans_points': (_i, [_vp, _i, _vp, _i, _i, _vp, _vp, _vp]),
    'wsi_kmeans_seed_farthest': (_i, [_vp, _i, _i, _vp, _vp, _vp]),
    'wsi_find_nuclei_lab': (_i, [_vp, _ll, _i, _d, _vp, _vp, _vp]),
    'wsi_fill_holes_scratch_bytes': (_sz, [_i, _i]),
    'wsi_fill_holes': (_i, [_vp, _i, _i, _vp, _vp, _vp]),
    'wsi_slic_scratch_bytes': (_sz, [_i, _i, _i]),
    'wsi_slic': (_i, [_vp, _i, _i, _vp, _i, _vp, _i, _i, _i, _d, _d, _i, _vp, _vp, _vp]),
    'wsi_tile_grid_candidates': (_ll, [_i, _i, _i, _i, _i, _i]),
    'wsi_tile_grid_scratch_bytes': (_sz, [_ll]),
    'wsi_tile_grid': (_i, [_i, _i, _i, _i, _i, _i, _vp, _i, _i, C.c_double, C.c_double, _vp, _vp, _vp, _vp]),
    'wsi_exponent_span': (_i, [_vp, _ll, _vp, _vp]),
    'wsi_paint_regions': (_i, [_vp, _vp, _ll, _vp, _vp, _vp, _ll, _vp]),
    'wsi_resize_bilinear_f64': (_i, [_vp, _i, _i, _i, _vp, _i, _i, _vp]),
    'wsi_argmax_classes': (_i, [_vp, _i, _ll, _vp, _vp]),
    'wsi_morph_rect': (_i, [_vp, _vp, _vp, _i, _i, _i, _i, _vp]),
    'wsi_bwperim': (_i, [_vp, _vp, _i, _i, _vp]),
    'wsi_tumor_bed_workspace_bytes': (_sz, [_i, _i]),
    'wsi_convex_hull_image': (_i, [_vp, _vp, _i, _i, _vp, _vp]),
    'wsi_tumor_bed': (_i, [_vp, _i, _i, _i, _i, _i, _vp, _vp, _vp, _vp, _vp]),
    'wsi_hull_polygon': (_i, [_vp, _i, _i, _vp, _i, _vp, _vp]),
    'wsi_mask_iou_counts': (_i, [_vp, _vp, _ll, _vp, _vp]),
    'wsi_score_counts': (_i, [_vp, _vp, _vp, _ll, _vp, _vp]),
    'wsi_esp': (_i, [_vp, _i, _i, _vp, _vp, _vp]),
    'wsi_unet_workspace_bytes': (_sz, [C.POINTER(WsiUnetDecoderWeights), _i, _i, _i, _i]),
    'wsi_unet_workspace_init': (_i, [C.POINTER(WsiUnetDecoderWeights), _vp, _i, _i, _i, _i, _vp]),
    'wsi_unet_forward': (_i, [C.POINTER(WsiTrunkWeights), C.POINTER(WsiUnetDecoderWeights), _vp, _vp, _ll, _i, _i, _vp, _vp, _i, _i, _i,
                              _vp, _i, _vp, C.POINTER(C.c_void_p * 5), _vp]),
    'wsi_resize_nearest_f32': (_i, [_vp, _ll, _i, _i, _vp, _i, _i, _vp]),
    'wsi_unet_decoder': (_i, [C.POINTER(WsiUnetDecoderWeights), C.POINTER(C.c_void_p * 5), _i, _i, _i, _i, _vp, _i, _vp, _vp]),
}


def build(verbose=False):
    res = subprocess.run(['make', '-C', CSRC, '-j8'], stdout=subprocess.PIPE, stderr=subprocess.STDOUT, text=True)
    if verbose or res.returncode:
        print(res.stdout)
    if res.returncode:
        raise RuntimeError('hipcc build of libwsi_hip.so failed')
    global _lib
    _lib = None
    return LIB_PATH


ABI_VERSION = 8


def load():
    global _lib
    if _lib is not None:
        return _lib
    if not os.path.exists(LIB_PATH):
        raise NativeLibraryMissing(
            '%s not found: the WSI inference path has no CPU fallback - build it first '
            '(python -c "import __graft_entry__ as g; g.build()" or make -C %s)' % (LIB_PATH, CSRC))
    lib = C.CDLL(LIB_PATH)
    for name, (res, args) in SIGNATURES.items():
        fn = getattr(lib, name)
        fn.restype = res
        fn.argtypes = args
    if lib.wsi_hip_abi_version() != ABI_VERSION:
        raise RuntimeError('libwsi_hip.so ABI version mismatch')
    _lib = lib
    return lib


class ConvMode(enum.IntFlag):
    S2_GATHER = 0
    S2_SLAB = 1
    S2_SLAB_128 = 3
    XCD_ORDER = 8
    WIDE_FROM_256 = 16
    WIDE_NEVER = 32
    S2_ABLATE = 64
    NO_S2_SPLIT = 128
    XCD_RANGES_OFF = 256
    XCD_RANGES_L1 = 512
    L1_SLAB3 = 1024
    NO_DS_FOLD = 2048
    NO_SLAB_PAIR = 4096
    L1_LINES128 = 16384
    S2_NT2 = 32768
    UNET_CONCAT_PASS = 65536
    WIDE_NO_D8 = 131072
    L1_PERSISTENT = 1048576
    UNET_NO_TAIL = 2097152
    UNET_TAIL_FORM1 = 4194304
    UNET_X0_UNFUSED = 8388608


class StemMode(enum.IntEnum):
    UNFUSED = 0
    FUSED = 1
    FUSED_LUT = 2
    FUSED_ONE_STRIP = 3


@contextlib.contextmanager
def conv_mode(flags=0, base=ConvMode.S2_SLAB):
    lib = load()
    check(lib.wsi_conv_set_mode(int(base) | int(flags)), 'wsi_conv_set_mode')
    try:
        yield
    finally:
        lib.wsi_conv_set_mode(int(ConvMode.S2_SLAB))


@contextlib.contextmanager
def stem_mode(fused, rows=64):
    lib = load()
    check(lib.wsi_stem_set_mode(int(fused), rows), 'wsi_stem_set_mode')
    try:
        yield
    finally:
        lib.wsi_stem_set_mode(int(StemMode.FUSED), 64)


def check(rc, what):
    if rc != 0:
        raise RuntimeError('%s failed with code %d (see include/wsi_hip.h error conventions)' % (what, rc))
```

Measured before the change: 119,200 patches/s.

## Pipeline residual-add tail with prefetch into weight buffers and deferred epilogue

Adds a pipelined MX residual tail that interleaves residual-tile DMA, identity-MFMA adds and the encode/store epilogue, deferring one line's store so it overlaps the next group's loads. In the wide 3-plane kernel, the first residual tile (or the second-input weights) is prefetched during the last main-loop tap, and the freed weight and slab LDS buffers are reused as extra ring slots. The second-input pass is restructured to double-buffer weights. The old batched tail stays reachable through a new mode flag, at the cost of more template variants and tighter LDS aliasing assumptions.

```diff
diff --git a/include/wsi_hip.h b/include/wsi_hip.h
--- a/include/wsi_hip.h
+++ b/include/wsi_hip.h
@@ -75,6 +75,7 @@
     WSI_CONV_MODE_S2_NT2 = 32768,
     WSI_CONV_MODE_UNET_CONCAT_PASS = 65536,
     WSI_CONV_MODE_WIDE_NO_D8 = 131072,
+    WSI_CONV_MODE_TAIL_BATCHED = 262144,
     WSI_CONV_MODE_L1_PERSISTENT = 1048576,
     WSI_CONV_MODE_UNET_NO_TAIL = 2097152,
     WSI_CONV_MODE_UNET_TAIL_FORM1 = 4194304,
diff --git a/wsi_segmentation_pipeline_amd/csrc/capi.hip b/wsi_segmentation_pipeline_amd/csrc/capi.hip
--- a/wsi_segmentation_pipeline_amd/csrc/capi.hip
+++ b/wsi_segmentation_pipeline_amd/csrc/capi.hip
@@ -685,6 +685,7 @@
     r.unet_tail = (mode & WSI_CONV_MODE_UNET_NO_TAIL) ? 0 : 1;
     r.unet_tail_form = (mode & WSI_CONV_MODE_UNET_TAIL_FORM1) ? 1 : 2;
     r.unet_x0_fused = (mode & WSI_CONV_MODE_UNET_X0_UNFUSED) ? 0 : 1;
+    r.tail_pipe = (mode & WSI_CONV_MODE_TAIL_BATCHED) ? 0 : 1;
     return WSI_OK;
 }
 
diff --git a/wsi_segmentation_pipeline_amd/csrc/common.h b/wsi_segmentation_pipeline_amd/csrc/common.h
--- a/wsi_segmentation_pipeline_amd/csrc/common.h
+++ b/wsi_segmentation_pipeline_amd/csrc/common.h
@@ -296,5 +296,6 @@
     int unet_tail = 1;
     int unet_tail_form = 2;
     int unet_x0_fused = 1;
+    int tail_pipe = 1;
 };
 extern ConvRoutes g_routes;
diff --git a/wsi_segmentation_pipeline_amd/csrc/conv.hip b/wsi_segmentation_pipeline_amd/csrc/conv.hip
--- a/wsi_segmentation_pipeline_amd/csrc/conv.hip
+++ b/wsi_segmentation_pipeline_amd/csrc/conv.hip
@@ -342,7 +342,7 @@
 }
 
 
-template <int MINW, int NCT = 0, bool IN96 = true>
+template <int MINW, int NCT = 0, bool IN96 = true, bool OLDTAIL = false>
 __global__ __launch_bounds__(256, MINW) void conv3x3s1_rows_kernel(ConvArgs a) {
     extern __shared__ __attribute__((aligned(16))) char smem[];
     constexpr int MT = 4, WN = 2, BM = 256, NTHREADS = 256, RESID_NBUF = 2;
@@ -462,7 +462,9 @@
         valid[mt] = true;
     }
     if (a.resid) __syncthreads();
-    conv_tail_mx<1, MT, RESID_NBUF>(a, acc, qs, valid, ntile, lane, smem + wave * (RESID_NBUF * 4096), slab0);
+    char* const scratch = smem + wave * (RESID_NBUF * 4096);
+    if constexpr (OLDTAIL) conv_tail_mx<1, MT, RESID_NBUF>(a, acc, qs, valid, ntile, lane, scratch, slab0);
+    else conv_tail_mx_pipe<1, MT, RESID_NBUF, false, false>(a, acc, qs, valid, ntile, lane, [&](int s) { return scratch + s * 4096; }, slab0);
 #ifdef WSI_STUDY
     asm volatile("s_waitcnt vmcnt(0)" ::: "memory");
     if (lane == 0 && (blockIdx.x & 63) == 0) {
@@ -492,6 +494,9 @@
     const bool i96 = a.flags & CONV_IN96;
     auto k = nc2 ? (i96 ? conv3x3s1_rows_kernel<MINW, 2, true> : conv3x3s1_rows_kernel<MINW, 2, false>)
                  : (i96 ? conv3x3s1_rows_kernel<MINW, 0, true> : conv3x3s1_rows_kernel<MINW, 0, false>);
+    if (!g_routes.tail_pipe)
+        k = nc2 ? (i96 ? conv3x3s1_rows_kernel<MINW, 2, true, true> : conv3x3s1_rows_kernel<MINW, 2, false, true>)
+                : (i96 ? conv3x3s1_rows_kernel<MINW, 0, true, true> : conv3x3s1_rows_kernel<MINW, 0, false, true>);
     if (lds > 64 * 1024 && hipFuncSetAttribute((const void*)k, hipFuncAttributeMaxDynamicSharedMemorySize, (int)lds) != hipSuccess)
         return WSI_EINVAL;
     const int grid = (a.flags & CONV_XCD_RANGES) ? (mtiles * nblocks + 7) / 8 * 8 : mtiles * nblocks;
@@ -722,10 +727,11 @@
 }
 
 
-template <int PLANES, int MINW, int ABL = 0, int WM = 2, int WN = 2, int NT = 2, bool D8 = false>
+template <int PLANES, int MINW, int ABL = 0, int WM = 2, int WN = 2, int NT = 2, bool D8 = false, bool OLDTAIL = false>
 __global__ __launch_bounds__(WM* WN * 64, MINW) void conv3x3s1_wide_kernel(ConvArgs a) {
     extern __shared__ __attribute__((aligned(16))) char smem[];
     constexpr int MT = 4, BM = WM * 128, NTHREADS = WM * WN * 64, NTILES = WN * NT, WB = NTILES * 4096;
+    constexpr bool PRE = PLANES == 3 && !OLDTAIL && NTILES >= WM * WN;
     constexpr int D8_ZB = 304;
     static_assert(!D8 || (BM == 256 && NTHREADS == 256), "D8: four whole 8 x 8 images per tile, 32 slab pixels per DMA round");
     constexpr int RESID_NBUF = 4;
@@ -803,6 +809,30 @@
         }
     };
 
+    auto qpos = [&](int mt) {
+        if constexpr (D8) {
+            const int i = mtile * BM + wm * MT * 32 + mt * 32 + lpix;
+            return pf_pos_of_index(a.gi, valid[mt] ? i : min(mtile * BM + BM, Rtot) - 1);
+        } else {
+            return xoff[mt] + slab0 + (P + 1);
+        }
+    };
+    auto resid_pre = [&](int wbuf) {
+        int qr = qpos(0) - slab0, ln = lane;
+        asm volatile("" : "+v"(qr), "+v"(ln));
+        resid_tile_request<true>(a, nb * NTILES + wn * NT, qr, slab0, ln, wl_addr + wbuf * WB + wave * 4096);
+    };
+    auto wdma2 = [&](int c, int wbuf) {
+        const int NC2 = a.in2_c / 32;
+        const __amdgpu_buffer_rsrc_t wrs2 = __builtin_amdgcn_make_buffer_rsrc(
+            (void*)((const char*)a.wpk2 + (size_t)(nb * NTILES) * NC2 * 4096), 0, NTILES * NC2 * 4096, 0x00020000);
+#pragma unroll
+        for (int p0 = 0; p0 < NTILES * 256; p0 += NTHREADS) {
+            const int pw = p0 + wave * 64;
+            dma16_buf_asm(wrs2, wl_addr + wbuf * WB + pw * 16, wvoff, ((pw >> 8) * NC2 + c) * 4096);
+        }
+    };
+
     f32x16 acc[NT][MT];
 #pragma unroll
     for (int nt = 0; nt < NT; ++nt) {
@@ -850,6 +880,12 @@
         for (int t = 0; t < 9; ++t) {
             const char* wb = wl + kpar * WB;
             if (t < 8) wdma(c, t + 1, (kpar ^ 1) * WB);
+            if constexpr (PLANES == 3 && !OLDTAIL) {
+                if (t == 8 && c == NC - 1) {
+                    if (a.in2) wdma2(0, kpar ^ 1);
+                    else if (PRE && a.resid) resid_pre(kpar ^ 1);
+                }
+            }
 #pragma unroll
             for (int nt = 0; nt < NT; ++nt) wread(wf[nt], wb, nt);
             const int toff = (t / 3) * Pc + (t % 3);
@@ -881,15 +917,10 @@
     int qs[MT];
 #pragma unroll
     for (int mt = 0; mt < MT; ++mt) {
-        if constexpr (D8) {
-            const int i = mtile * BM + wm * MT * 32 + mt * 32 + lpix;
-            qs[mt] = pf_pos_of_index(a.gi, valid[mt] ? i : min(mtile * BM + BM, Rtot) - 1);
-        } else {
-            qs[mt] = xoff[mt] + slab0 + (P + 1);
-        }
+        qs[mt] = qpos(mt);
     }
     if constexpr (PLANES == 3) {
-        if (a.in2) {
+        if (!OLDTAIL && a.in2) {
             const int NC2 = a.in2_c / 32;
             const size_t ps2 = (size_t)a.in2_c * 4, sb2 = (size_t)slab0 * ps2;
             const size_t bytes2 = (size_t)pf_alloc_pixels(a.gi.N, a.gi.H, a.gi.W) * ps2;
@@ -900,6 +931,50 @@
                 const int i = wave * 64 + lane, Pl = i >> 3, sl = (i & 7) ^ ((Pl >> 1) & 7);
                 xvoff2 = (D8 ? (Pl >> 3) * 9 + (Pl & 7) : Pl) * (int)ps2 + sl * 16;
             }
+#pragma unroll
+            for (int nt = 0; nt < NT; ++nt) {
+                f32x16 b2[1];
+                acc_init_bias<1>(b2, a.bias2, nb * NTILES + wn * NT + nt, lane);
+#pragma unroll
+                for (int mt = 0; mt < MT; ++mt)
+#pragma unroll
+                    for (int r = 0; r < 16; ++r) acc[nt][mt][r] += b2[0][r];
+            }
+            for (int c = 0; c < NC2; ++c) {
+                __syncthreads();
+                for (int i0 = wave * 64, r = 0; i0 < npieces; i0 += NTHREADS, ++r)
+                    dma16_buf_asm(xrs2, xl_addr + i0 * 16, xvoff2, c * 128 + r * RPIX * (int)ps2);
+                asm volatile("s_waitcnt vmcnt(0)" ::: "memory");
+                __syncthreads();
+                if (c + 1 < NC2) wdma2(c + 1, kpar ^ 1);
+                else if (PRE && a.resid) resid_pre(kpar ^ 1);
+                const char* wb = wl + kpar * WB;
+                bf16x8 wf2[NT][4], x2[2][4];
+#pragma unroll
+                for (int nt = 0; nt < NT; ++nt) wread(wf2[nt], wb, nt);
+                const int ctr = (D8 ? 8 : P) + 1;
+                xload(x2[0], xoff[0] + ctr);
+#pragma unroll
+                for (int mt = 0; mt < MT; ++mt) {
+                    if (mt + 1 < MT) xload(x2[(mt + 1) & 1], xoff[mt + 1] + ctr);
+                    __builtin_amdgcn_sched_barrier(0);
+#pragma unroll
+                    for (int nt = 0; nt < NT; ++nt) mfma_step<PLANES>(acc[nt][mt], wf2[nt], x2[mt & 1]);
+                }
+                kpar ^= 1;
+            }
+        }
+        if (OLDTAIL && a.in2) {
+            const int NC2 = a.in2_c / 32;
+            const size_t ps2 = (size_t)a.in2_c * 4, sb2 = (size_t)slab0 * ps2;
+            const size_t bytes2 = (size_t)pf_alloc_pixels(a.gi.N, a.gi.H, a.gi.W) * ps2;
+            const __amdgpu_buffer_rsrc_t xrs2 = __builtin_amdgcn_make_buffer_rsrc(
+                (void*)((const char*)a.in2 + sb2), 0, (int)min(bytes2 - sb2, (size_t)0x7fffffff), 0x00020000);
+            int xvoff2;
+            {
+                const int i = wave * 64 + lane, Pl = i >> 3, sl = (i & 7) ^ ((Pl >> 1) & 7);
+                xvoff2 = (D8 ? (Pl >> 3) * 9 + (Pl & 7) : Pl) * (int)ps2 + sl * 16;
+            }
             const char* wsrc2 = (const char*)a.wpk2 + (size_t)(nb * NTILES) * NC2 * 4096 + (size_t)(tid & 255) * 16;
 #pragma unroll
             for (int nt = 0; nt < NT; ++nt) {
@@ -933,8 +1008,24 @@
                 }
             }
         }
-        if (a.resid) __syncthreads();
-        conv_tail_mx<NT, MT, RESID_NBUF>(a, acc, qs, valid, nb * NTILES + wn * NT, lane, smem + wave * (RESID_NBUF * 4096), slab0);
+        if (a.resid) {
+            if constexpr (PRE) asm volatile("s_waitcnt vmcnt(0)" ::: "memory");
+            __syncthreads();
+        }
+        if constexpr (OLDTAIL) {
+            conv_tail_mx<NT, MT, RESID_NBUF>(a, acc, qs, valid, nb * NTILES + wn * NT, lane, smem + wave * (RESID_NBUF * 4096), slab0);
+        } else if constexpr (PRE) {
+            auto slot = [&](int s) -> char* {
+                if (s == 0) return wl + kpar * WB + wave * 4096;
+                const int j = wave * (RESID_NBUF - 1) + s - 1;
+                return j < NTILES ? wl + (kpar ^ 1) * WB + j * 4096 : xl + (j - NTILES) * 4096;
+            };
+            static_assert((WM * WN * (RESID_NBUF - 1) - NTILES) * 4096 <= WM * WN * 8192, "ring slots past the weight buffer fit the slab's minimum size");
+            conv_tail_mx_pipe<NT, MT, RESID_NBUF, true, true>(a, acc, qs, valid, nb * NTILES + wn * NT, lane, slot, slab0);
+        } else {
+            char* const scratch = smem + wave * (RESID_NBUF * 4096);
+            conv_tail_mx_pipe<NT, MT, RESID_NBUF, false, true>(a, acc, qs, valid, nb * NTILES + wn * NT, lane, [&](int s) { return scratch + s * 4096; }, slab0);
+        }
     } else {
         char* scratch = nullptr;
         if (PLANES == 2 && a.resid && !(a.flags & CONV_RESID_DIRECT)) {
@@ -960,12 +1051,17 @@
 }
 
 
-template <int PLANES, int MINW, int ABL = 0, int WM = 2, int WN = 2, int NT = 2, bool D8 = false>
+template <int PLANES, int MINW, int ABL = 0, int WM = 2, int WN = 2, int NT = 2, bool D8 = false, bool OLDTAIL = false>
 static int launch_wide(const ConvArgs& a, hipStream_t st) {
     constexpr int BM = WM * 128, NTHREADS = WM * WN * 64, BN = WN * NT * 32;
     if (a.go.C % BN) return WSI_EINVAL;
-    if constexpr (!D8 && ABL == 0 && WM == 2 && WN == 2 && NT == 2) {
+    if (a.flags & (CONV_IN96 | CONV_OUT96 | CONV_RESID96)) return WSI_EINVAL;
+    if (a.in2 && (a.in2_c < 32 || a.in2_c % 32)) return WSI_EINVAL;
+    if constexpr (!D8 && ABL == 0 && WM == 2 && WN == 2 && NT == 2 && !OLDTAIL) {
         if (g_routes.wide_d8 && a.gi.W == 8 && a.gi.H == 8) return launch_wide<PLANES, MINW, 0, 2, 2, 2, true>(a, st);
+    }
+    if constexpr (PLANES == 3 && ABL == 0 && WM == 2 && WN == 2 && NT == 2 && !OLDTAIL) {
+        if (!g_routes.tail_pipe) return launch_wide<PLANES, MINW, 0, 2, 2, 2, D8, true>(a, st);
     }
     const int nblocks = a.go.C / BN;
     const long long R = (long long)a.gi.N * a.gi.H * a.gi.W;
@@ -976,7 +1072,7 @@
     size_t lds = 2 * (BN / 32) * 4096 + xbytes;
     if (PLANES == 3 && lds < (size_t)WM * WN * 4 * 4096) lds = (size_t)WM * WN * 4 * 4096;
     if (lds > 160 * 1024) return WSI_EINVAL;
-    auto k = conv3x3s1_wide_kernel<PLANES, MINW, ABL, WM, WN, NT, D8>;
+    auto k = conv3x3s1_wide_kernel<PLANES, MINW, ABL, WM, WN, NT, D8, OLDTAIL>;
     if (lds > 64 * 1024 && hipFuncSetAttribute((const void*)k, hipFuncAttributeMaxDynamicSharedMemorySize, (int)lds) != hipSuccess)
         return WSI_EINVAL;
     const int grid = (a.flags & CONV_XCD_RANGES) ? (mtiles * nblocks + 7) / 8 * 8 : mtiles * nblocks;
diff --git a/wsi_segmentation_pipeline_amd/csrc/conv_dev.h b/wsi_segmentation_pipeline_amd/csrc/conv_dev.h
--- a/wsi_segmentation_pipeline_amd/csrc/conv_dev.h
+++ b/wsi_segmentation_pipeline_amd/csrc/conv_dev.h
@@ -42,6 +42,30 @@
         const int sl = (lane & 7) ^ ((pp >> 1) & 7);
         dma16_buf(rs, dst + j * 1024, q * pixstride + sl * 16, line_off);
     }
+}
+
+template <bool R96>
+static __device__ __forceinline__ void resid_tile_dma_asm(__amdgpu_buffer_rsrc_t rs, int q_rel, int pixstride, int line_off, int lane, unsigned lds) {
+#pragma unroll
+    for (int j = 0; j < 4; ++j) {
+        const int pp = 8 * j + (lane >> 3);
+        const int q = __shfl(q_rel, pp);
+        const int sl = (lane & 7) ^ ((pp >> 1) & 7);
+        if (!R96) dma16_buf_asm(rs, lds + j * 1024, q * pixstride + sl * 16, line_off);
+        else if (sl != 5 && sl != 7) dma16_buf_asm(rs, lds + j * 1024, q * pixstride + (sl == 6 ? 5 : sl) * 16, line_off);
+    }
+}
+
+template <bool NO96 = false>
+static __device__ __forceinline__ void resid_tile_request(const ConvArgs& a, int ntile, int q_rel, int slab0, int lane, unsigned lds) {
+    const bool r96 = !NO96 && (a.flags & CONV_RESID96);
+    const int pixstride = r96 ? 96 : a.go.C * 4;
+    const size_t rbase = (size_t)slab0 * pixstride, rbytes = (size_t)pf_alloc_pixels(a.go.N, a.go.H, a.go.W) * pixstride;
+    const __amdgpu_buffer_rsrc_t rs = __builtin_amdgcn_make_buffer_rsrc(
+        (void*)((const char*)a.resid + (r96 ? (size_t)ntile * (size_t)a.plane96 : (size_t)0) + rbase), 0,
+        (int)min(rbytes - rbase, (size_t)0x7fffffff), 0x00020000);
+    if (r96) resid_tile_dma_asm<true>(rs, q_rel, pixstride, 0, lane, lds);
+    else resid_tile_dma_asm<false>(rs, q_rel, pixstride, ntile * 128, lane, lds);
 }
 
 static __device__ __forceinline__ bool mx96_stored(int s) { return s != 5 && s != 7; }
@@ -217,52 +241,87 @@
         for (int r = 0; r < 16; ++r) acc[mt][r] = b[r];
 }
 
+struct MxLine {
+    f16x8 hv[2];
+    u32x6 q;
+    int sl, sh;
+};
+static __device__ __forceinline__ MxLine mx_line_encode(const f32x16& v, float lo_clamp, int h) {
+    MxLine L;
+    f32x16 hi, lo;
+    float mv = 0.f, ml = 0.f;
+#pragma unroll
+    for (int r = 0; r < 16; r += 2) {
+        const float v0 = __builtin_amdgcn_fmed3f(v[r], lo_clamp, 65504.f);
+        const float v1 = __builtin_amdgcn_fmed3f(v[r + 1], lo_clamp, 65504.f);
+        const f16x2 hh = __builtin_convertvector(f32x2{v0, v1}, f16x2);
+        L.hv[r >> 3][r & 7] = hh[0];
+        L.hv[r >> 3][(r & 7) + 1] = hh[1];
+        hi[r] = (float)hh[0];
+        hi[r + 1] = (float)hh[1];
+        lo[r] = v0 - hi[r];
+        lo[r + 1] = v1 - hi[r + 1];
+        mv = fmaxf(mv, fmaxf(fabsf(hi[r]), fabsf(hi[r + 1])));
+        ml = fmaxf(ml, fmaxf(fabsf(lo[r]), fabsf(lo[r + 1])));
+    }
+    pair_max2(mv, ml);
+    L.sh = mx6_scale_byte(mv);
+    L.sl = mx6_scale_byte(ml);
+    const int sb = h ? L.sh : L.sl;
+    swap32_halves(lo, hi);
+    L.q = mx6_pack32(lo, hi, sb ? mx_scale_value(sb) : 1.f);
+    return L;
+}
+template <bool NO96 = false>
+static __device__ __forceinline__ void mx_line_store(const ConvArgs& a, const MxLine& L, int q, bool valid, int ntile, int lane) {
+    const int h = lane >> 5;
+    const bool o96 = !NO96 && (a.flags & CONV_OUT96);
+    const size_t pixstride = o96 ? (size_t)96 : (size_t)a.go.C * 4;
+    if (valid && !CONV_STUDY(a, CONV_ABL_NO_STORE)) {
+        const size_t loff = (size_t)q * pixstride + (o96 ? (size_t)ntile * (size_t)a.plane96 : (size_t)ntile * 128);
+        char* ol = (char*)a.out + (a.out_split_pixels ? pf_out_offset(a.go, a.out_split_pixels, q, pixstride) + (size_t)ntile * 128 : loff);
+        *(f16x8*)(ol + 32 * h) = L.hv[0];
+        *(f16x8*)(ol + 32 * h + 16) = L.hv[1];
+        if (!o96) {
+            const int sb = h ? L.sh : L.sl;
+            *(u32x4*)(ol + MX6_PLANE_LO(0) + 16 * h) = u32x4{L.q[0], L.q[1], L.q[2], L.q[3]};
+            *(u32x4*)(ol + MX6_PLANE_HI(0) + 16 * h) = u32x4{L.q[4], L.q[5], (unsigned)sb, 0u};
+        } else if (h == 0) {
+            *(u32x4*)(ol + 64) = u32x4{L.q[0], L.q[1], L.q[2], L.q[3]};
+            *(u32x4*)(ol + 80) = u32x4{L.q[4], L.q[5], (unsigned)L.sl, (unsigned)L.sh};
+        }
+    }
+}
 template <int MT, int MTN = MT>
 static __device__ __forceinline__ void conv_epilogue_mx(const ConvArgs& a, f32x16 (&acc)[MT], const int (&qs)[MT],
                                                         const bool (&valid)[MT], int ntile, int lane, int mt0 = 0) {
-    const int h = lane >> 5;
-    const bool o96 = a.flags & CONV_OUT96;
-    const size_t pixstride = o96 ? (size_t)96 : (size_t)a.go.C * 4;
     const float lo_clamp = a.relu ? 0.f : -65504.f;
 #pragma unroll
     for (int mt = mt0; mt < mt0 + MTN; ++mt) {
-        const size_t loff = (size_t)(valid[mt] ? qs[mt] : a.go.G) * pixstride + (o96 ? (size_t)ntile * (size_t)a.plane96 : (size_t)ntile * 128);
-        f32x16 v = acc[mt];
-        f32x16 hi, lo;
-        f16x8 hv[2];
-        float mv = 0.f, ml = 0.f;
-#pragma unroll
-        for (int r = 0; r < 16; r += 2) {
-            const float v0 = __builtin_amdgcn_fmed3f(v[r], lo_clamp, 65504.f);
-            const float v1 = __builtin_amdgcn_fmed3f(v[r + 1], lo_clamp, 65504.f);
-            const f16x2 hh = __builtin_convertvector(f32x2{v0, v1}, f16x2);
-            hv[r >> 3][r & 7] = hh[0];
-            hv[r >> 3][(r & 7) + 1] = hh[1];
-            hi[r] = (float)hh[0];
-            hi[r + 1] = (float)hh[1];
-            lo[r] = v0 - hi[r];
-            lo[r + 1] = v1 - hi[r + 1];
-            mv = fmaxf(mv, fmaxf(fabsf(hi[r]), fabsf(hi[r + 1])));
-            ml = fmaxf(ml, fmaxf(fabsf(lo[r]), fabsf(lo[r + 1])));
-        }
-        pair_max2(mv, ml);
-        const int sh = mx6_scale_byte(mv), sl = mx6_scale_byte(ml);
-        const int sb = h ? sh : sl;
-        swap32_halves(lo, hi);
-        const u32x6 q = mx6_pack32(lo, hi, sb ? mx_scale_value(sb) : 1.f);
-        if (valid[mt] && !CONV_STUDY(a, CONV_ABL_NO_STORE)) {
-            char* ol = (char*)a.out + (a.out_split_pixels ? pf_out_offset(a.go, a.out_split_pixels, qs[mt], pixstride) + (size_t)ntile * 128 : loff);
-            *(f16x8*)(ol + 32 * h) = hv[0];
-            *(f16x8*)(ol + 32 * h + 16) = hv[1];
-            if (!o96) {
-                *(u32x4*)(ol + MX6_PLANE_LO(0) + 16 * h) = u32x4{q[0], q[1], q[2], q[3]};
-                *(u32x4*)(ol + MX6_PLANE_HI(0) + 16 * h) = u32x4{q[4], q[5], (unsigned)sb, 0u};
-            } else if (h == 0) {
-                *(u32x4*)(ol + 64) = u32x4{q[0], q[1], q[2], q[3]};
-                *(u32x4*)(ol + 80) = u32x4{q[4], q[5], (unsigned)sl, (unsigned)sh};
-            }
-        }
-    }
+        const MxLine L = mx_line_encode(acc[mt], lo_clamp, lane >> 5);
+        mx_line_store(a, L, qs[mt], valid[mt], ntile, lane);
+    }
+}
+
+static __device__ __forceinline__ void mx_identity_operand(bf16x8 (&iw)[4], int lane) {
+    const int h = lane >> 5, l31 = lane & 31;
+            const int p = mx_line_pos(l31), f0 = mx6_field_of_pos(p);
+            f16x8 k0, k1;
+    #pragma unroll
+            for (int j = 0; j < 8; ++j) {
+                k0[j] = (p == 8 * h + j) ? (_Float16)1.0f : (_Float16)0.0f;
+                k1[j] = (p == 16 + 8 * h + j) ? (_Float16)1.0f : (_Float16)0.0f;
+            }
+            unsigned q[6];
+    #pragma unroll
+            for (int d = 0; d < 6; ++d) {
+                const int bit = 6 * f0 + 3 - 32 * d;
+                q[d] = (h == 0 && bit >= 0 && bit < 32) ? (1u << (bit & 31)) : 0u;
+            }
+            iw[0] = __builtin_bit_cast(bf16x8, k0);
+            iw[1] = __builtin_bit_cast(bf16x8, k1);
+            iw[2] = __builtin_bit_cast(bf16x8, u32x4{q[0], q[1], q[2], q[3]});
+            iw[3] = __builtin_bit_cast(bf16x8, u32x4{q[4], q[5], 127u, 0u});
 }
 
 template <int NT, int MT, int NBUF>
@@ -283,25 +342,7 @@
     const __amdgpu_buffer_rsrc_t rrs = __builtin_amdgcn_make_buffer_rsrc((void*)((const char*)a.resid + rbase), 0,
                                                                           (int)min(rbytes - rbase, (size_t)0x7fffffff), 0x00020000);
     bf16x8 iw[4];
-    {
-        const int p = mx_line_pos(l31), f0 = mx6_field_of_pos(p);
-        f16x8 k0, k1;
-#pragma unroll
-        for (int j = 0; j < 8; ++j) {
-            k0[j] = (p == 8 * h + j) ? (_Float16)1.0f : (_Float16)0.0f;
-            k1[j] = (p == 16 + 8 * h + j) ? (_Float16)1.0f : (_Float16)0.0f;
-        }
-        unsigned q[6];
-#pragma unroll
-        for (int d = 0; d < 6; ++d) {
-            const int bit = 6 * f0 + 3 - 32 * d;
-            q[d] = (h == 0 && bit >= 0 && bit < 32) ? (1u << (bit & 31)) : 0u;
-        }
-        iw[0] = __builtin_bit_cast(bf16x8, k0);
-        iw[1] = __builtin_bit_cast(bf16x8, k1);
-        iw[2] = __builtin_bit_cast(bf16x8, u32x4{q[0], q[1], q[2], q[3]});
-        iw[3] = __builtin_bit_cast(bf16x8, u32x4{q[4], q[5], 127u, 0u});
-    }
+    mx_identity_operand(iw, lane);
     auto rdma = [&](int k) {
         const int nt = k / MT, mt = k % MT;
         int qr = qs[mt] - slab0;
@@ -342,6 +383,77 @@
         } else {
             conv_epilogue_mx<MT, NBUF>(a, acc[b0 / MT], qs, valid, ntile0 + b0 / MT, lane, b0 % MT);
         }
+    }
+}
+
+template <int NBUF, bool PRE>
+static constexpr int tail_group_begin(int g) { return PRE && NBUF > 1 ? (g == 0 ? 0 : g == 1 ? 1 : (g - 1) * NBUF) : g * NBUF; }
+
+template <int NT, int MT, int NBUF, bool PRE, bool NO96, class Slot>
+static __device__ __forceinline__ void conv_tail_mx_pipe(const ConvArgs& a, f32x16 (&acc)[NT][MT], const int (&qs)[MT], const bool (&valid)[MT],
+                                                         int ntile0, int lane, Slot slot, int slab0) {
+    constexpr int T = NT * MT, NG = T / NBUF + (PRE && NBUF > 1 ? 1 : 0);
+    static_assert(NBUF <= T && T % NBUF == 0, "whole groups");
+    if (!a.resid) {
+#pragma unroll
+        for (int nt = 0; nt < NT; ++nt) conv_epilogue_mx<MT>(a, acc[nt], qs, valid, ntile0 + nt, lane);
+        return;
+    }
+    const int h = lane >> 5, l31 = lane & 31;
+    const bool r96 = !NO96 && (a.flags & CONV_RESID96);
+    auto rdma = [&](int k) {
+        int qr = qs[k % MT] - slab0, ln = lane;
+        asm volatile("" : "+v"(qr), "+v"(ln));
+        resid_tile_request<NO96>(a, ntile0 + k / MT, qr, slab0, ln, lds_addr_of(slot(k % NBUF)));
+    };
+    const float lo_clamp = a.relu ? 0.f : -65504.f;
+    const int xb = l31 * 128 + ((h ^ ((l31 >> 1) & 7)) << 4);
+    int late_k = -1;
+    auto finish = [&](int k) {
+        __builtin_amdgcn_sched_barrier(0);
+        const MxLine L = mx_line_encode(acc[k / MT][k % MT], lo_clamp, h);
+        int q = qs[k % MT], ln = lane;
+        asm volatile("" : "+v"(q), "+v"(ln));
+        mx_line_store<NO96>(a, L, q, valid[k % MT], ntile0 + k / MT, ln);
+    };
+#pragma unroll
+    for (int k = (PRE ? 1 : 0); k < tail_group_begin<NBUF, PRE>(PRE && NBUF > 1 ? 2 : 1); ++k) rdma(k);
+#pragma unroll
+    for (int g = 0; g < NG; ++g) {
+        const int b = tail_group_begin<NBUF, PRE>(g), e = tail_group_begin<NBUF, PRE>(g + 1);
+        if (!(PRE && g == 0)) asm volatile("s_waitcnt vmcnt(0)" ::: "memory");
+        bf16x8 iw[4];
+        {
+            int ln = lane;
+            asm volatile("" : "+v"(ln));
+            mx_identity_operand(iw, ln);
+        }
+#pragma unroll
+        for (int k = b; k < e; ++k) {
+            const char* t = slot(k % NBUF);
+            bf16x8 x[4];
+            int xbk = xb;
+            asm volatile("" : "+v"(xbk));
+#pragma unroll
+            for (int f = 0; f < 4; ++f) x[f] = *(const bf16x8*)(t + (xbk ^ (f << 5)));
+            if (r96 && h) {
+                x[2] = __builtin_bit_cast(bf16x8, u32x4{0u, 0u, 0u, 0u});
+                x[3] = x[2];
+            }
+            acc[k / MT][k % MT] = mfma_mx6(acc[k / MT][k % MT], iw, x);
+            asm volatile("" : "+v"(acc[k / MT][k % MT]));
+            __builtin_amdgcn_sched_barrier(0);
+        }
+        if (g + 1 < NG && !(PRE && NBUF > 1 && g == 0)) {
+            asm volatile("s_waitcnt lgkmcnt(0)" ::: "memory");
+#pragma unroll
+            for (int k = e; k < tail_group_begin<NBUF, PRE>(g + 2); ++k) rdma(k);
+        }
+        if (late_k >= 0) finish(late_k);
+        late_k = g + 1 < NG && !(PRE && NBUF > 1 && g == 0) ? e - 1 : -1;
+#pragma unroll
+        for (int k = b; k < e; ++k)
+            if (k != late_k) finish(k);
     }
 }
 
diff --git a/wsi_segmentation_pipeline_amd/native.py b/wsi_segmentation_pipeline_amd/native.py
--- a/wsi_segmentation_pipeline_amd/native.py
+++ b/wsi_segmentation_pipeline_amd/native.py
@@ -175,6 +175,7 @@
     S2_NT2 = 32768
     UNET_CONCAT_PASS = 65536
     WIDE_NO_D8 = 131072
+    TAIL_BATCHED = 262144
     L1_PERSISTENT = 1048576
     UNET_NO_TAIL = 2097152
     UNET_TAIL_FORM1 = 4194304
```

New measurement: 119,300 patches/s, median of 2. Within noise of the previous version (+0.1%).
